# lucagem29/mcmc_clv_model

Hardware: AMD Instinct MI355X
Metric: MCMC sweeps/sec x N_customers (customer-sweeps/s) (higher is better)
Workload: dtype f64

## Files before the change

include/clvmcmc.h:

```cpp
#ifndef CLVMCMC_H
#define CLVMCMC_H

#include <stdint.h>

#ifdef __cplusplus
extern "C" {
#endif

#define CLV_ABI_VERSION 2

#define CLV_BLOCK 256
#define CLV_MAX_K 9
#define CLV_MAX_D 3

enum { CLV_OK = 0, CLV_EINVAL = -1, CLV_EHIP = -2, CLV_ESTATE = -3, CLV_ENOMEM = -4 };
enum { CLV_RNG_PHILOX = 0, CLV_RNG_REPLAY = 1 };
enum { CLV_SINK_FULL = 0, CLV_SINK_SUMMARY = 1, CLV_SINK_NONE = 2, CLV_SINK_SUMMARY_PCT = 3 };

#define CLV_SUMMARY_MU_CAP 0.05
enum {
  CLV_SUM_LAMBDA = 0, CLV_SUM_MU, CLV_SUM_Z, CLV_SUM_LOG_LAMBDA, CLV_SUM_LOG_MU,
  CLV_SUM_LAMBDA2, CLV_SUM_MU2, CLV_SUM_ETA, CLV_SUM_LOG_ETA, CLV_SUM_MU_CAPPED, CLV_SUM_TAU,
  CLV_N_SUM_STATS
};

typedef struct clv_config {
  int32_t abi_version;
  int32_t D;
  int32_t K;
  int32_t n_mh_steps;
  int32_t burnin, mcmc, thin;
  int32_t n_chains;
  int32_t chain_first;
  int32_t rng_mode;
  int32_t draw_sink;
  int32_t device;
  uint64_t seed;
  int64_t n_global;
  int64_t shard_begin;
  int32_t world_size;
  int32_t rank;
  int32_t blocks_per_rank;
  int32_t blocks_per_unit;
  uint64_t stream;
} clv_config;

typedef struct clv_data {
  int64_t n;
  const int32_t* x;
  const double* t_x;
  const double* T_cal;
  const double* covariates;
  const double* log_s;
} clv_data;

typedef struct clv_prior {
  double lam_init;
  double V[CLV_MAX_K * CLV_MAX_K];
  double chol_V[CLV_MAX_K * CLV_MAX_K];
  double A0B0[CLV_MAX_K * CLV_MAX_D];
  double S0_B0A0B0[CLV_MAX_D * CLV_MAX_D];
  double nu_n;
  double beta_init[CLV_MAX_K * CLV_MAX_D];
  double sigma_init[CLV_MAX_D * CLV_MAX_D];
  double omega2;
} clv_prior;

typedef struct clv_sampler clv_sampler;

int32_t clv_abi_version(void);
int32_t clv_default_blocks_per_unit(int64_t n_global);
int64_t clv_sizeof(int32_t which);
const char* clv_last_error(void);
int clv_device_count(int32_t* count);

int clv_create(const clv_config* cfg, const clv_data* data, const clv_prior* prior,
               clv_sampler** out);
void clv_destroy(clv_sampler* s);

int clv_set_replay_tape(clv_sampler* s, const double* tape, int64_t n_sweeps);
int64_t clv_replay_sweep_stride(const clv_sampler* s);

int clv_run(clv_sampler* s, int64_t n_sweeps);
int clv_rollback(clv_sampler* s);

int clv_sweep(clv_sampler* s);
int clv_hyper(clv_sampler* s, const double* gathered_device_ptr);
int clv_partials(clv_sampler* s, double** device_ptr, int64_t* n_doubles, int32_t* stride);
int clv_copy_partials(clv_sampler* s, void* dst_device_ptr);
int clv_synchronize(clv_sampler* s);
int64_t clv_sweeps_done(const clv_sampler* s);

int clv_clock_ghz(clv_sampler* s, double* ghz);
int clv_clock_probe(clv_sampler* s, double us, double* ghz);
int clv_launch_info(const clv_sampler* s, int64_t* out);
int clv_split_relay_steps(const clv_sampler* s, int32_t* out);
#define CLV_IPC_HANDLE_BYTES 64
int clv_p2p_info(const clv_sampler* s, int64_t* out);
int clv_p2p_export(clv_sampler* s, void* handle);
int clv_p2p_connect(clv_sampler* s, const void* handles, const uint64_t* ptrs);
int clv_p2p_disconnect(clv_sampler* s);
int clv_p2p_set_persistent(clv_sampler* s, int32_t on);
int clv_set_wait_timeout(clv_sampler* s, double ms);
int clv_set_stream(clv_sampler* s, uint64_t stream);
int clv_note_sweeps(clv_sampler* s, int64_t n);

int clv_read_draws(clv_sampler* s, double* level1, double* level2, double* loglik);
int clv_stream_draws(clv_sampler* s, double* level1);
int clv_read_summary(clv_sampler* s, double* sums, int64_t* n_stored);

int clv_get_state(clv_sampler* s, double* lambdas, double* mus, double* hyper);
int clv_set_state(clv_sampler* s, const double* lambdas, const double* mus, const double* hyper,
                  int64_t sweeps_done);

int clv_set_timing(clv_sampler* s, int32_t enable);
int clv_kernel_time(clv_sampler* s, double* sweep_kernel_ms_total, int64_t* sweep_launches,
                    double* hyper_kernel_ms_total, int64_t* hyper_launches);

int clv_debug_host_times(const clv_sampler* s, int64_t* out);
int clv_debug_philox(uint32_t k0, uint32_t k1, const uint32_t* ctr, int64_t n, uint32_t* out);
int clv_debug_variates(uint64_t seed, int32_t chain, uint32_t sweep, int64_t n, int32_t n_steps,
                       float* t_l, float* t_m, float* u_acc, double* u_z, double* u_tau,
                       double* e_alive, double* eta_z, float* log2_u_acc);
int clv_debug_log2u_scan(uint64_t w_begin, uint64_t w_end, double* out);
int clv_debug_t3(const uint32_t* words, int64_t n, int32_t packed, float* t_l, float* t_m);
int clv_debug_level2(int32_t D, int32_t K, const clv_prior* prior, const double* xty,
                     const double* yty, const double* iw_normal, const double* iw_chi2,
                     const double* z, double* beta, double* sigma);
int clv_debug_stamps(clv_sampler* s, uint64_t* out);
int clv_debug_wg_stamps(clv_sampler* s, uint64_t* out);
int clv_debug_hyper_variates(uint64_t seed, int32_t chain, uint32_t sweep, double df, int64_t n,
                             double* chi2, double* normals);
int clv_debug_exp(const double* x, int64_t n, double* out);
int clv_debug_log(const double* x, int64_t n, double* out);
int clv_debug_mh_step(int64_t n, const int32_t* x, const uint8_t* z, const double* T_cal, const double* tau,
                      const double* mean, const double* prec3, const double* cur_pt, const float* t3,
                      const double* scale2, const float* log_u, double* out);
int clv_debug_wg_map(int32_t n_chains, int32_t nb, int32_t n_cu, int32_t* out);
int clv_debug_persist_fits(int64_t grid_wgs, int32_t blocks_per_cu, int32_t n_cu);
int clv_debug_persist_choice(int32_t D, int32_t K, int32_t n_chains, int64_t grid_wgs, int32_t blocks_per_cu,
                             int32_t n_cu);
int clv_debug_split_fits(int32_t n_chains, int32_t nb, int32_t blocks_per_cu, int32_t n_cu);
int clv_debug_split_choice(int32_t n_chains, int32_t nb, int32_t blocks_per_cu, int32_t n_cu);
int clv_debug_split_layout(int32_t n_chains, int32_t nb, int32_t* out);
int clv_debug_split_relay_plan(int32_t S, int32_t R, int32_t* out);
int clv_debug_split_draw_plan(int32_t R, int32_t share, int32_t* out);
int clv_debug_split_stamps(clv_sampler* s, uint64_t* out);
int clv_debug_sweep_plan(const int64_t* in, int32_t* out);

enum { CLV_EXCHANGE_AUTO = 0, CLV_EXCHANGE_P2P = 1, CLV_EXCHANGE_COPY = 2 };
typedef struct clv_group clv_group;
int clv_group_create(clv_sampler* const* shards, int32_t n, int32_t exchange, clv_group** out);
int clv_group_run(clv_group* g, int64_t n_sweeps);
int32_t clv_group_exchange(const clv_group* g);
void clv_group_destroy(clv_group* g);

enum {
  CLV_L1_MEAN_LAMBDA = 0, CLV_L1_LAMBDA_P025, CLV_L1_LAMBDA_P975, CLV_L1_MEAN_MU, CLV_L1_MEAN_MU_CAPPED,
  CLV_L1_MU_P025, CLV_L1_MU_P975, CLV_L1_MEAN_Z, CLV_L1_MEAN_TAU, CLV_L1_MEAN_ETA, CLV_N_L1_STATS
};
int clv_predict(int32_t device, const double* level1, int64_t n_draws, int64_t n, int32_t width,
                const double* T_cal, double T_star, uint64_t seed, int32_t simulate_spend, double sigma_s,
                int64_t* x_future, double* spend_future);
int clv_predict_sampler(clv_sampler* s, double T_star, uint64_t seed, int32_t simulate_spend,
                        double sigma_s, int64_t* x_future, double* spend_future);
int clv_track(int32_t device, const double* level1, int64_t n_draws, int64_t n, int32_t width,
              const double* birth_week, const double* times, int32_t n_times, uint64_t seed,
              double* inc_weekly);
int clv_track_sampler(clv_sampler* s, const double* birth_week, const double* times, int32_t n_times,
                      uint64_t seed, double* inc_weekly);
int clv_level1_summary(int32_t device, const double* level1, int64_t n_draws, int64_t n, int32_t width,
                       double mu_cap, double* out);
int clv_level1_summary_sampler(clv_sampler* s, double mu_cap, double* out);
int clv_chain_total_loglik(int32_t device, const double* level1, int64_t n_draws, int64_t n, int32_t width,
                           const int32_t* x, const double* T_cal, double* mean_total);
int clv_chain_total_loglik_sampler(clv_sampler* s, double* mean_total);

enum {
  CLV_LTV_VALUE_MEAN = 0, CLV_LTV_VALUE_SD, CLV_LTV_VALUE_P025, CLV_LTV_VALUE_P50, CLV_LTV_VALUE_P975,
  CLV_LTV_RESIDUAL_MEAN, CLV_LTV_RESIDUAL_SD, CLV_LTV_RESIDUAL_P025, CLV_LTV_RESIDUAL_P50, CLV_LTV_RESIDUAL_P975,
  CLV_LTV_P_ALIVE, CLV_LTV_LIFETIME_YRS, CLV_LTV_SURVIVAL_1YR, CLV_N_LTV_STATS
};
enum {
  CLV_LTV_DRAW_EQUITY = 0, CLV_LTV_DRAW_VALUE_TOTAL, CLV_LTV_DRAW_N_ALIVE, CLV_LTV_DRAW_MU_SHARE,
  CLV_N_LTV_DRAW_STATS
};
int clv_lifetime_value(int32_t device, const double* level1, int64_t n_draws, int64_t n, int32_t width,
                       const double* monetary , double delta, double horizon ,
                       double value_scale, double periods_per_year, double* out_customers, double* out_draws);
int clv_lifetime_value_sampler(clv_sampler* s, const double* monetary, double delta, double horizon,
                               double value_scale, double periods_per_year, double* out_customers,
                               double* out_draws);
int clv_ltv_info(int64_t* out);

enum {
  CLV_IC_LPPD = 0, CLV_IC_P_WAIC, CLV_IC_ELPD_WAIC, CLV_IC_ELPD_LOO, CLV_IC_P_LOO, CLV_IC_PARETO_K,
  CLV_IC_TAIL_LEN, CLV_N_IC_STATS
};
int clv_pointwise_loglik(int32_t device, const double* level1, int64_t n_draws, int64_t n, int32_t width,
                         const int32_t* x, const double* t_x, const double* T_cal,
                         const double* log_s , double omega2, double* out);
int clv_psis_loo(int32_t device, const double* loglik, int64_t n_draws, int64_t n, double reff, double* out);
int clv_information_criteria(int32_t device, const double* level1, int64_t n_draws, int64_t n, int32_t width,
                             const int32_t* x, const double* t_x, const double* T_cal, const double* log_s,
                             double omega2, double reff, double* out);
int clv_information_criteria_sampler(clv_sampler* s, int32_t spend, double omega2, double reff, double* out);
int clv_ic_info(int64_t* out);
int clv_debug_information_criteria(int32_t device, const double* level1, int64_t n_draws, int64_t n, int32_t width,
                                   const int32_t* x, const double* t_x, const double* T_cal, const double* log_s,
                                   double omega2, double reff, int64_t batch_keys, int32_t grid, double* out);

int clv_score_customers(int32_t device, int32_t D, int32_t K, int32_t n_chains, int64_t n_draws,
                        const double* level2, int64_t n, const int32_t* x, const double* t_x,
                        const double* T_cal, const double* cov, const double* log_s, double omega2,
                        int32_t n_mh_steps, int32_t warmup, int32_t inner_sweeps, uint64_t seed,
                        int32_t chain_first, int64_t customer_offset, int64_t sweep_first,
                        const double* init_lam, const double* init_mu, int32_t sink, double* level1_out,
                        double* sums_out, double* state_lam_out, double* state_mu_out);
int clv_score_customers_sampler(clv_sampler* s, int64_t n, const int32_t* x, const double* t_x,
                                const double* T_cal, const double* cov, const double* log_s,
                                int32_t n_mh_steps, int32_t warmup, int32_t inner_sweeps, uint64_t seed,
                                int64_t customer_offset, int64_t sweep_first, const double* init_lam,
                                const double* init_mu, int32_t sink, double* level1_out, double* sums_out,
                                double* state_lam_out, double* state_mu_out);
int clv_score_info(int64_t* out);
int clv_debug_score_hyper(int32_t device, int32_t D, int32_t K, int64_t n_rec, const double* level2,
                          double omega2, double* out);

enum {
  CLV_FC_XSTAR_MEAN = 0, CLV_FC_P_ALIVE, CLV_FC_P_ZERO, CLV_FC_Q05, CLV_FC_Q50, CLV_FC_Q95, CLV_FC_TAIL_MASS,
  CLV_FC_LOG_SCORE, CLV_FC_PIT_LO, CLV_FC_PIT_HI, CLV_FC_RPS, CLV_N_FC_STATS
// ... 150 lines not shown
```

mcmc_clv_model_amd/_lib.py:

```python
from __future__ import annotations

import ctypes
import os
from ctypes import c_uint8, POINTER, c_char_p, c_double, c_float, c_int32, c_int64, c_uint32, c_uint64, c_void_p

try:
    import torch
except Exception:
    torch = None

LIB_NAME = "libclvmcmc.so"
LIB_PATH = os.environ.get("CLV_LIB_PATH") or os.path.join(os.path.dirname(os.path.abspath(__file__)), LIB_NAME)

ABI_VERSION = 2
BLOCK = 256
MAX_K = 9
MAX_D = 3
RNG_PHILOX, RNG_REPLAY = 0, 1
SINK_FULL, SINK_SUMMARY, SINK_NONE, SINK_SUMMARY_PCT = 0, 1, 2, 3
EXCHANGE_AUTO, EXCHANGE_P2P, EXCHANGE_COPY = 0, 1, 2
SUM_STATS = ("lambda", "mu", "z", "log_lambda", "log_mu", "lambda2", "mu2", "eta", "log_eta", "mu_capped", "tau")
SUMMARY_MU_CAP = 0.05
N_SUM_STATS = len(SUM_STATS)
TAPE_HYPER = 40


class ClvConfig(ctypes.Structure):
    _fields_ = [
        ("abi_version", c_int32), ("D", c_int32), ("K", c_int32), ("n_mh_steps", c_int32),
        ("burnin", c_int32), ("mcmc", c_int32), ("thin", c_int32), ("n_chains", c_int32),
        ("chain_first", c_int32), ("rng_mode", c_int32), ("draw_sink", c_int32), ("device", c_int32),
        ("seed", c_uint64), ("n_global", c_int64), ("shard_begin", c_int64),
        ("world_size", c_int32), ("rank", c_int32), ("blocks_per_rank", c_int32),
        ("blocks_per_unit", c_int32), ("stream", c_uint64),
    ]


class ClvData(ctypes.Structure):
    _fields_ = [
        ("n", c_int64), ("x", c_void_p), ("t_x", c_void_p), ("T_cal", c_void_p),
        ("covariates", c_void_p), ("log_s", c_void_p),
    ]


class ClvPrior(ctypes.Structure):
    _fields_ = [
        ("lam_init", c_double), ("V", c_double * 81), ("chol_V", c_double * 81), ("A0B0", c_double * 27),
        ("S0_B0A0B0", c_double * 9), ("nu_n", c_double), ("beta_init", c_double * 27),
        ("sigma_init", c_double * 9), ("omega2", c_double),
    ]


class ClvBatchItem(ctypes.Structure):
    _fields_ = [
        ("n", c_int64), ("seed", c_uint64), ("x", c_void_p), ("t_x", c_void_p), ("T_cal", c_void_p),
        ("covariates", c_void_p), ("log_s", c_void_p), ("prior", POINTER(ClvPrior)),
        ("level1", c_void_p), ("level2", c_void_p), ("loglik", c_void_p), ("sums", c_void_p),
        ("state_lam", c_void_p), ("state_mu", c_void_p),
    ]


_lib = None


class ClvError(RuntimeError):
    pass


def lib() -> ctypes.CDLL:
    global _lib
    if _lib is not None:
        return _lib
    if not os.path.exists(LIB_PATH):
        raise ClvError(
            f"{LIB_NAME} is not built ({LIB_PATH}); run `make -C mcmc_clv_model_amd/csrc` "
            "or `python -c 'import __graft_entry__ as g; g.build()'`")
    L = ctypes.CDLL(LIB_PATH, mode=ctypes.RTLD_GLOBAL)
    sp = c_void_p
    dp = POINTER(c_double)
    sigs = {
        "clv_abi_version": (c_int32, []),
        "clv_default_blocks_per_unit": (c_int32, [c_int64]),
        "clv_sizeof": (c_int64, [c_int32]),
        "clv_last_error": (c_char_p, []),
        "clv_device_count": (c_int32, [POINTER(c_int32)]),
        "clv_create": (c_int32, [POINTER(ClvConfig), POINTER(ClvData), POINTER(ClvPrior), POINTER(sp)]),
        "clv_destroy": (None, [sp]),
        "clv_set_replay_tape": (c_int32, [sp, dp, c_int64]),
        "clv_replay_sweep_stride": (c_int64, [sp]),
        "clv_run": (c_int32, [sp, c_int64]),
        "clv_rollback": (c_int32, [sp]),
        "clv_sweep": (c_int32, [sp]),
        "clv_hyper": (c_int32, [sp, c_void_p]),
        "clv_partials": (c_int32, [sp, POINTER(c_void_p), POINTER(c_int64), POINTER(c_int32)]),
        "clv_copy_partials": (c_int32, [sp, c_void_p]),
        "clv_synchronize": (c_int32, [sp]),
        "clv_sweeps_done": (c_int64, [sp]),
        "clv_clock_ghz": (c_int32, [sp, POINTER(c_double)]),
        "clv_clock_probe": (c_int32, [sp, c_double, POINTER(c_double)]),
        "clv_launch_info": (c_int32, [sp, POINTER(c_int64)]),
        "clv_split_relay_steps": (c_int32, [sp, POINTER(c_int32)]),
        "clv_p2p_info": (c_int32, [sp, POINTER(c_int64)]),
        "clv_p2p_export": (c_int32, [sp, c_void_p]),
        "clv_p2p_connect": (c_int32, [sp, c_void_p, POINTER(c_uint64)]),
        "clv_p2p_disconnect": (c_int32, [sp]),
        "clv_p2p_set_persistent": (c_int32, [sp, c_int32]),
        "clv_set_wait_timeout": (c_int32, [sp, c_double]),
        "clv_set_stream": (c_int32, [sp, c_uint64]),
        "clv_note_sweeps": (c_int32, [sp, c_int64]),
        "clv_read_draws": (c_int32, [sp, dp, dp, dp]),
        "clv_stream_draws": (c_int32, [sp, dp]),
        "clv_read_summary": (c_int32, [sp, dp, POINTER(c_int64)]),
        "clv_get_state": (c_int32, [sp, dp, dp, dp]),
        "clv_set_state": (c_int32, [sp, dp, dp, dp, c_int64]),
        "clv_set_timing": (c_int32, [sp, c_int32]),
        "clv_kernel_time": (c_int32, [sp, dp, POINTER(c_int64), dp, POINTER(c_int64)]),
        "clv_debug_philox": (c_int32, [c_uint32, c_uint32, POINTER(c_uint32), c_int64, POINTER(c_uint32)]),
        "clv_debug_variates": (c_int32, [c_uint64, c_int32, c_uint32, c_int64, c_int32, POINTER(c_float),
                                         POINTER(c_float), POINTER(c_float), dp, dp, dp, dp, POINTER(c_float)]),
        "clv_debug_log2u_scan": (c_int32, [c_uint64, c_uint64, dp]),
        "clv_debug_host_times": (c_int32, [sp, POINTER(c_int64)]),
        "clv_debug_t3": (c_int32, [POINTER(c_uint32), c_int64, c_int32, POINTER(c_float), POINTER(c_float)]),
        "clv_debug_level2": (c_int32, [c_int32, c_int32, POINTER(ClvPrior), dp, dp, dp, dp, dp, dp, dp]),
        "clv_debug_hyper_variates": (c_int32, [c_uint64, c_int32, c_uint32, c_double, c_int64, dp, dp]),
        "clv_debug_stamps": (c_int32, [sp, POINTER(c_uint64)]),
        "clv_debug_wg_stamps": (c_int32, [sp, POINTER(c_uint64)]),
        "clv_debug_split_stamps": (c_int32, [sp, POINTER(c_uint64)]),
        "clv_debug_split_relay_plan": (c_int32, [c_int32, c_int32, POINTER(c_int32)]),
        "clv_debug_split_draw_plan": (c_int32, [c_int32, c_int32, POINTER(c_int32)]),
        "clv_debug_exp": (c_int32, [dp, c_int64, dp]),
        "clv_debug_log": (c_int32, [dp, c_int64, dp]),
        "clv_debug_mh_step": (c_int32, [c_int64, POINTER(c_int32), POINTER(c_uint8), dp, dp, dp, dp, dp,
                                        POINTER(c_float), dp, POINTER(c_float), dp]),
        "clv_debug_wg_map": (c_int32, [c_int32, c_int32, c_int32, POINTER(c_int32)]),
        "clv_debug_sweep_plan": (c_int32, [POINTER(c_int64), POINTER(c_int32)]),
        "clv_debug_persist_choice": (c_int32, [c_int32, c_int32, c_int32, c_int64, c_int32, c_int32]),
        "clv_debug_persist_fits": (c_int32, [c_int64, c_int32, c_int32]),
        "clv_group_create": (c_int32, [POINTER(sp), c_int32, c_int32, POINTER(sp)]),
        "clv_group_run": (c_int32, [sp, c_int64]),
        "clv_group_exchange": (c_int32, [sp]),
        "clv_group_destroy": (None, [sp]),
        "clv_predict": (c_int32, [c_int32, dp, c_int64, c_int64, c_int32, dp, c_double, c_uint64, c_int32, c_double,
                                  POINTER(c_int64), dp]),
        "clv_predict_sampler": (c_int32, [sp, c_double, c_uint64, c_int32, c_double, POINTER(c_int64), dp]),
        "clv_track": (c_int32, [c_int32, dp, c_int64, c_int64, c_int32, dp, dp, c_int32, c_uint64, dp]),
        "clv_track_sampler": (c_int32, [sp, dp, dp, c_int32, c_uint64, dp]),
        "clv_level1_summary": (c_int32, [c_int32, dp, c_int64, c_int64, c_int32, c_double, dp]),
        "clv_level1_summary_sampler": (c_int32, [sp, c_double, dp]),
        "clv_chain_total_loglik": (c_int32, [c_int32, dp, c_int64, c_int64, c_int32, POINTER(c_int32), dp, dp]),
        "clv_chain_total_loglik_sampler": (c_int32, [sp, dp]),
        "clv_lifetime_value": (c_int32, [c_int32, dp, c_int64, c_int64, c_int32, dp, c_double, c_double, c_double,
                                         c_double, dp, dp]),
        "clv_lifetime_value_sampler": (c_int32, [sp, dp, c_double, c_double, c_double, c_double, dp, dp]),
        "clv_ltv_info": (c_int32, [POINTER(c_int64)]),
        "clv_pointwise_loglik": (c_int32, [c_int32, dp, c_int64, c_int64, c_int32, POINTER(c_int32), dp, dp, dp,
                                           c_double, dp]),
        "clv_psis_loo": (c_int32, [c_int32, dp, c_int64, c_int64, c_double, dp]),
        "clv_information_criteria": (c_int32, [c_int32, dp, c_int64, c_int64, c_int32, POINTER(c_int32), dp, dp, dp,
                                               c_double, c_double, dp]),
        "clv_information_criteria_sampler": (c_int32, [sp, c_int32, c_double, c_double, dp]),
        "clv_ic_info": (c_int32, [POINTER(c_int64)]),
        "clv_debug_information_criteria": (c_int32, [c_int32, dp, c_int64, c_int64, c_int32, POINTER(c_int32), dp,
                                                     dp, dp, c_double, c_double, c_int64, c_int32, dp]),
        "clv_score_customers": (c_int32, [c_int32, c_int32, c_int32, c_int32, c_int64, dp, c_int64, POINTER(c_int32), dp,
                                          dp, dp, dp, c_double, c_int32, c_int32, c_int32, c_uint64, c_int32, c_int64,
                                          c_int64, dp, dp, c_int32, dp, dp, dp, dp]),
        "clv_score_customers_sampler": (c_int32, [sp, c_int64, POINTER(c_int32), dp, dp, dp, dp, c_int32, c_int32,
                                                  c_int32, c_uint64, c_int64, c_int64, dp, dp, c_int32, dp, dp, dp, dp]),
        "clv_score_info": (c_int32, [POINTER(c_int64)]),
        "clv_debug_score_hyper": (c_int32, [c_int32, c_int32, c_int32, c_int64, dp, c_double, dp]),
        "clv_forecast": (c_int32, [c_int32, dp, c_int64, c_int64, c_int32, POINTER(c_int32), dp, dp, c_double, c_int32,
                                   POINTER(c_int32), dp, dp]),
        "clv_forecast_sampler": (c_int32, [sp, c_double, c_int32, POINTER(c_int32), dp, dp]),
        "clv_forecast_info": (c_int32, [POINTER(c_int64)]),
        "clv_debug_forecast": (c_int32, [c_int32, dp, c_int64, c_int64, c_int32, POINTER(c_int32), dp, dp, c_double,
                                         c_int32, POINTER(c_int32), c_int64, c_int32, dp, dp]),
        "clv_ppc": (c_int32, [c_int32, c_int32, dp, c_int32, dp, c_int32, c_int32, dp, c_int64, c_int64,
                              POINTER(c_int32), dp, dp, c_int32, c_uint64, c_int64, dp, POINTER(c_int64), dp,
                              POINTER(c_int64), dp]),
        "clv_ppc_sampler": (c_int32, [sp, c_int32, c_int32, c_uint64, dp, POINTER(c_int64), dp, POINTER(c_int64), dp]),
        "clv_ppc_info": (c_int32, [POINTER(c_int64)]),
        "clv_debug_ppc": (c_int32, [c_int32, c_int32, dp, c_int32, dp, c_int32, c_int32, dp, c_int64, c_int64,
                                    POINTER(c_int32), dp, dp, c_int32, c_uint64, c_int64, dp, POINTER(c_int64), dp,
                                    POINTER(c_int64), dp, c_int64, c_int32]),
        "clv_marginal_loglik": (c_int32, [c_int32, dp, c_int32, c_int32, dp, c_int64, c_int64, POINTER(c_int32), dp,
                                          dp, dp, c_double, c_int32, dp]),
        "clv_marginal_information_criteria": (c_int32, [c_int32, dp, c_int32, c_int32, dp, c_int64, c_int64,
                                                        POINTER(c_int32), dp, dp, dp, c_double, c_int32, c_double, dp]),
        "clv_marginal_information_criteria_sampler": (c_int32, [sp, c_int32, c_double, c_double, c_int32, dp]),
        "clv_marginal_info": (c_int32, [POINTER(c_int64)]),
        "clv_debug_marginal_loglik": (c_int32, [c_int32, dp, c_int32, c_int32, dp, c_int64, c_int64, POINTER(c_int32),
                                                dp, dp, dp, c_double, c_int32, c_int64, c_int32, dp, dp]),
        "clv_mml_create": (c_int32, [c_int32, c_int64, POINTER(c_int32), dp, dp, dp, c_int32, dp, POINTER(sp)]),
        "clv_mml_destroy": (None, [sp]),
        "clv_mml_eval": (c_int32, [sp, dp, c_int32, dp, POINTER(c_int64)]),
        "clv_mml_customers": (c_int32, [sp, dp, c_int32, c_double, dp]),
        "clv_debug_mml_eval": (c_int32, [sp, dp, c_int32, c_int32, dp, POINTER(c_int64)]),
        "clv_mml_info": (c_int32, [POINTER(c_int64)]),
        "clv_diagnostics": (c_int32, [c_int32, dp, c_int32, c_int64, c_int64, c_int32, c_uint32, dp]),
        "clv_diagnostics_sampler": (c_int32, [sp, c_uint32, dp, dp]),
        "clv_autocorr": (c_int32, [c_int32, dp, c_int32, c_int64, c_int64, c_int32, dp]),
        "clv_rank_diagnostics": (c_int32, [c_int32, dp, c_int32, c_int64, c_int64, c_int32, c_uint32, c_double, dp]),
        "clv_rank_diagnostics_sampler": (c_int32, [sp, c_uint32, c_double, dp, dp]),
        "clv_debug_zscale": (c_int32, [c_int32, dp, c_int32, c_int64, c_int64, c_int32, dp, dp]),
        "clv_elog2cbs": (c_int32, [c_int32, c_int64, POINTER(c_int64), POINTER(c_int64), dp, c_int64, c_int64, c_int64,
                                   POINTER(c_int64), POINTER(c_int64), POINTER(c_int64), dp, dp, dp, dp,
                                   POINTER(c_int64), dp, dp, POINTER(c_int64), dp]),
        "clv_generate_pareto_abe": (c_int32, [c_int32, c_int64, c_int32, dp, dp, dp, dp, c_int32, dp, c_uint64,
                                              POINTER(c_int64), dp, dp, dp, dp, POINTER(c_uint8), POINTER(c_int64), dp,
                                              POINTER(c_int64), POINTER(c_int64), c_int64, POINTER(c_int64), dp]),
        "clv_pnbd_create": (c_int32, [c_int32, c_int64, POINTER(c_int32), dp, dp, dp, POINTER(sp)]),
        "clv_pnbd_destroy": (None, [sp]),
        "clv_pnbd_eval": (c_int32, [sp, dp, dp, POINTER(c_int64)]),
        "clv_pnbd_customers": (c_int32, [sp, dp, c_double, dp]),
        "clv_pnbd_track": (c_int32, [c_int32, c_int64, dp, dp, c_int32, dp, dp]),
        "clv_pnbd_set_covariates": (c_int32, [sp, c_int32, dp, c_int32, dp]),
        "clv_pnbd_eval_cov": (c_int32, [sp, dp, dp, POINTER(c_int64)]),
        "clv_pnbd_customers_cov": (c_int32, [sp, dp, c_double, dp]),
# ... 153 lines not shown
```

mcmc_clv_model_amd/csrc/capi.hip:

```cpp
#include <hip/hip_runtime.h>

#include <algorithm>
#include <chrono>
#include <cstdlib>
#include <cstdio>
#include <cstring>
#include <string>
#include <vector>

#include "internal.h"
#include "kernels.h"
#include "philox.h"

using namespace clv;

namespace {

thread_local std::string g_err;

constexpr int PRIOR_V = 0, PRIOR_CHOLV = 81, PRIOR_A0B0 = 162, PRIOR_S0B = 189, PRIOR_DOUBLES = 198;
constexpr int GRAPH_CHUNK = 64;
constexpr int TIMING_EVENTS = 256;

}
// ... 214 lines not shown
  if ((d[1] == WAIT_P2P_MAIL || d[1] == WAIT_FX_MAIL) && g.units_per_rank > 0 && unit >= 0)
    m += "unit " + std::to_string(unit) + " (rank " + std::to_string(unit / g.units_per_rank) + ", local unit " +
         std::to_string(unit % g.units_per_rank) + ")";
  else
    m += (d[1] == WAIT_HYPER ? "of block " : "") + std::to_string(unit);
  if (d[1] == WAIT_RELAY) m += " (statistic: the wave row, bits: the flag's tag)";
  char bits[32];
  std::snprintf(bits, sizeof(bits), "%016llx", d[7]);
  m += " statistic " + std::to_string((long long)d[6]) + " still empty (bits " + bits + ") after " +
       std::to_string(d[8]) + " polls, " + std::to_string(d[9] / 100000.0) + " ms; " + std::to_string(d[10]) +
       " lanes of the wave missing";
  if (d[1] == WAIT_P2P_MAIL || d[1] == WAIT_FX_MAIL) {
    m += "; progress (sweep each rank's level-2 side last polled for):";
    for (int q = 0; q < std::min(g.world_size, 5); ++q)
      m += " " + std::to_string(q) + ":" + (d[11 + q] == ~0ull ? std::string("none") : std::to_string((long long)d[11 + q]));
  }
  return m + "]";
}

bool parse_wait_ms(const char* txt, double* ms) {
  for (const char* c = txt; *c; ++c)
    if (*c == 'x' || *c == 'X' || *c == 'n' || *c == 'N' || *c == 'i' || *c == 'I') return false;
  char* end = nullptr;
  const double v = std::strtod(txt, &end);
  if (end == txt) return false;
  while (*end == ' ' || *end == '\t' || *end == '\n') ++end;
  if (*end || !(v == v) || v > 1e300 || v < -1e300) return false;
  *ms = std::min(3.6e6, std::max(1.0, v));
  return true;
}

}

extern "C" {

int32_t clv_abi_version(void) { return CLV_ABI_VERSION; }

int32_t clv_default_blocks_per_unit(int64_t n_global) {
  const int64_t nb = (n_global + BLOCK - 1) / BLOCK;
  int32_t g = 1;
  while ((nb + g - 1) / g > 512) g *= 2;
  return g;
}

const char* clv_last_error(void) { return g_err.c_str(); }

int64_t clv_sizeof(int32_t which) {
  switch (which) {
    case 0: return (int64_t)sizeof(clv_config);
    case 1: return (int64_t)sizeof(clv_data);
    case 2: return (int64_t)sizeof(clv_prior);
    default: return -1;
  }
}

int clv_device_count(int32_t* count) {
  int n = 0;
  CLV_HIP(hipGetDeviceCount(&n));
  *count = n;
  return CLV_OK;
}

int64_t clv_replay_sweep_stride(const clv_sampler* s) {
  const int64_t n = s->g.n;
  return n * (2 + 3 * (int64_t)s->g.S + (s->g.D == 3 ? 1 : 0)) + TAPE_HYPER;
}

}

bool clv::persist_grid_fits(int64_t grid_wgs, int blocks_per_cu, int n_cu) {
  constexpr int SGPR_MAX = 102;
  const int sgpr_term = 800 / (((SGPR_MAX + 15) / 16) * 16 + 16);
  const int64_t per_cu = std::min({blocks_per_cu, 8, sgpr_term});
  const int64_t slots = per_cu * n_cu;
  const int64_t margin = std::max(1, n_cu / 32);
  return grid_wgs > 0 && slots > 0 && grid_wgs <= slots - margin;
}

constexpr size_t PERSIST_SCRATCH_MAX = 64;
#ifndef CLV_SPLIT_RELAY_DEFAULT
#define CLV_SPLIT_RELAY_DEFAULT 1
#endif
constexpr bool SPLIT_RELAY_DEFAULT = CLV_SPLIT_RELAY_DEFAULT != 0;

namespace {

bool persist_worth(int D, int K, int n_chains, int64_t grid_wgs, int n_cu) {
  (void)D, (void)K, (void)n_chains;
  return n_cu > 0 && grid_wgs > 0;
}

bool persist_split_fits(int n_chains, int nb, int blocks_per_cu, int n_cu) {
  if (n_chains < 1 || nb < 1 || nb > SPLIT_MAX_NB || blocks_per_cu < 1 || n_cu < 1) return false;
  const int64_t grid = (int64_t)n_chains * (split_wgs(nb) + 1);
  const int64_t margin = std::max(1, n_cu / 64);
  return grid <= n_cu - margin;
}

bool persist_split_pays(int n_chains, int nb, int n_cu) { return (int64_t)n_chains * (nb + 1) > n_cu; }

std::vector<int32_t> persist_split_layout(int n_chains, int nb) {
  const int per = split_wgs(nb) + 1;
  std::vector<int32_t> map((size_t)n_chains * per);
  for (int c = 0; c < n_chains; ++c)
    for (int p = 0; p < per; ++p) map[(size_t)c * per + p] = (c << 16) | p;
  return map;
}

#ifndef CLV_L2_ALONE_MIN_NB
#define CLV_L2_ALONE_MIN_NB 256
#endif
std::vector<int32_t> persist_wg_map(int C, int nb, int n_cu) {
  const int per = nb + 1;
  const int T = C * per;
  std::vector<int32_t> map(T);
  for (int c = 0; c < C; ++c)
    for (int b = 0; b < per; ++b) map[c * per + b] = (c << 16) | b;
  const int P = T - n_cu;
  if (P <= 0 || T > 2 * n_cu) return map;
  std::vector<std::vector<int>> todo(C);
  for (int c = 0; c < C; ++c)
    for (int b = nb - 1; b >= 0; --b) todo[c].push_back(b);
  std::vector<int32_t> first, second, single;
  int p = 0;
  const bool l2_alone = nb >= CLV_L2_ALONE_MIN_NB;
  for (int c = 0; !l2_alone && c < C && p < P; ++c, ++p) {
    first.push_back((c << 16) | nb);
    if (todo[c].empty()) return map;
    second.push_back((c << 16) | todo[c].back());
    todo[c].pop_back();
  }
  const int n_l2_paired = (int)first.size();
  const bool l2_paired = n_l2_paired == C;
  for (int c = 0; p < P; c = (c + 1) % C) {
    bool any = false;
    for (int k = 0; k < C && !any; ++k) any = todo[(c + k) % C].size() >= 2;
    if (!any) return map;
    if (todo[c].size() < 2) continue;
    first.push_back((c << 16) | todo[c].back());
    todo[c].pop_back();
    second.push_back((c << 16) | todo[c].back());
    todo[c].pop_back();
    ++p;
  }
  for (int c = 0; c < C; ++c) {
    if (!l2_paired && c >= n_l2_paired) single.push_back((c << 16) | nb);
    while (!todo[c].empty()) {
      single.push_back((c << 16) | todo[c].back());
      todo[c].pop_back();
    }
  }
  std::vector<int32_t> sorted_single;
  for (size_t k = 0; sorted_single.size() < single.size(); ++k)
    for (int c = 0; c < C; ++c) {
      size_t seen = 0;
      for (int32_t v : single)
        if ((v >> 16) == c && seen++ == k) sorted_single.push_back(v);
    }
  if ((int)first.size() != P || (int)sorted_single.size() != n_cu - P) return map;
  for (int i = 0; i < P; ++i) {
    map[i] = first[i];
    map[n_cu + i] = second[i];
  }
  for (int i = 0; i < n_cu - P; ++i) map[P + i] = sorted_single[i];
  return map;
}


struct SweepEnv {
  int persistent = -1;
  int layout = 0;
  int relay = -1;
  bool defer = true;
  int mail_first = 0;
  double wait_ms = 0.0;
};

SweepEnv read_sweep_env() {
  const auto is = [](const char* v, const char* text) { return v && !std::strcmp(v, text); };
  SweepEnv e;
  const char* v = std::getenv("CLV_PERSISTENT");
  e.persistent = is(v, "0") ? 0 : is(v, "1") ? 1 : -1;
  v = std::getenv("CLV_PERSIST_LAYOUT");
  e.layout = !v ? 0 : is(v, "block") ? LAYOUT_BLOCK : is(v, "split") ? LAYOUT_SPLIT : -1;
  v = std::getenv("CLV_SPLIT_RELAY");
  e.relay = !v ? -1 : is(v, "0") ? 0 : is(v, "1") ? 1 : 2;
  e.defer = !is(std::getenv("CLV_DEFER"), "0");
  v = std::getenv("CLV_MAIL_ALLOC");
  e.mail_first = is(v, "fine") ? 1 : is(v, "default") ? 2 : 0;
  v = std::getenv("CLV_WAIT_TIMEOUT_MS");
  if (v && !parse_wait_ms(v, &e.wait_ms)) e.wait_ms = -1.0;
  return e;
}

constexpr int64_t NOT_QUERIED = -2, QUERY_FAILED = -1;
struct Instance { int bpc = 0; int64_t scratch = NOT_QUERIED; };
struct SweepResources {
  int n_cu = 0;
  Instance block, split, relay;
};
struct SweepPlan {
  bool persistent = false, split = false, p2p_capable = false, p2p_persist_fits = false, fx_capable = false, defer = false;
  int relay_steps = 0;
  bool need_split = false, need_relay = false;
  const char* error = nullptr;
};

bool persist_shape(const Geometry& g, bool replay) {
  if (replay || g.nb_local <= 0 || g.nb_local > 2 * BLOCK) return false;
  if (g.world_size == 1) return g.blocks_per_unit == 1;
  const int bpu = g.blocks_per_unit;
  return g.world_size <= MAX_WORLD && g.n_units_global <= 2 * BLOCK && bpu <= 64 &&
         (int64_t)g.stride * ((g.nb_local + bpu - 1) / bpu) <= UMAIL;
}

bool persist_grid_chosen(int D, int K, int n_chains, int64_t grid_wgs, int blocks_per_cu, int n_cu, bool force) {
  return persist_grid_fits(grid_wgs, blocks_per_cu, n_cu) && (force || persist_worth(D, K, n_chains, grid_wgs, n_cu));
}
bool split_chosen(int n_chains, int nb, int blocks_per_cu, int n_cu, bool force) {
  return persist_split_fits(n_chains, nb, blocks_per_cu, n_cu) && (force || persist_split_pays(n_chains, nb, n_cu));
}

SweepPlan plan_sweep(const Geometry& g, bool replay, const SweepResources& r, const SweepEnv& e) {
  SweepPlan p;
  const int C = g.n_chains, nb = g.nb_local;
  const bool force = e.persistent == 1;
  const bool resident = persist_shape(g, replay) && e.persistent != 0 &&
                        (force || (r.block.scratch >= 0 && r.block.scratch <= (int64_t)PERSIST_SCRATCH_MAX)) &&
                        persist_grid_chosen(g.D, g.K, C, (int64_t)(nb + 1) * C, r.block.bpc, r.n_cu, force);
  if (g.world_size == 1) p.persistent = resident;
  else p.p2p_capable = p.p2p_persist_fits = resident;
  p.fx_capable = !replay && g.world_size > 1 && g.world_size <= MAX_WORLD && g.n_units_global <= 2 * BLOCK;
  p.defer = p.persistent && e.defer;
  if (!(p.persistent && g.D == 2 && g.S <= PRE_STEPS && nb <= SPLIT_MAX_NB)) return p;
  if (e.layout < 0) p.error = "CLV_PERSIST_LAYOUT must be block or split";
  else if (e.relay > 1) p.error = "CLV_SPLIT_RELAY must be 0 or 1";
  if (p.error || e.layout == LAYOUT_BLOCK) return p;
  if (r.split.scratch == NOT_QUERIED) {
    p.need_split = true;
    return p;
  }
  p.split = r.split.scratch == 0 && split_chosen(C, nb, r.split.bpc, r.n_cu, e.layout == LAYOUT_SPLIT);
  if (p.split && SPLIT_RELAY_STEPS > 0 && g.S > SPLIT_RELAY_STEPS && (e.relay < 0 ? SPLIT_RELAY_DEFAULT : e.relay == 1)) {
    if (r.relay.scratch == NOT_QUERIED) p.need_relay = true;
    else if (r.relay.scratch == 0 && persist_split_fits(C, nb, r.relay.bpc, r.n_cu)) p.relay_steps = SPLIT_RELAY_STEPS;
  }
  return p;
}


int validate_and_derive(const clv_config* cfg, const clv_data* data, const clv_prior* prior, clv_sampler** out) {
  if (cfg->abi_version != CLV_ABI_VERSION) return fail(CLV_EINVAL, "ABI version mismatch");
  if (cfg->D != 2 && cfg->D != 3) return fail(CLV_EINVAL, "D must be 2 or 3");
  if (cfg->K < 1 || cfg->K > CLV_MAX_K) return fail(CLV_EINVAL, "K must be in 1..9");
  if (cfg->n_mh_steps < 0) return fail(CLV_EINVAL, "n_mh_steps must be >= 0");
  if (cfg->thin < 1) return fail(CLV_EINVAL, "thin must be >= 1");
  if (cfg->burnin < 0 || cfg->mcmc < 0) return fail(CLV_EINVAL, "burnin/mcmc must be >= 0");
  if (cfg->n_chains < 1) return fail(CLV_EINVAL, "n_chains must be >= 1");
  if (cfg->rng_mode != CLV_RNG_PHILOX && cfg->rng_mode != CLV_RNG_REPLAY) return fail(CLV_EINVAL, "bad rng_mode");
  if (cfg->draw_sink < CLV_SINK_FULL || cfg->draw_sink > CLV_SINK_SUMMARY_PCT) return fail(CLV_EINVAL, "bad draw_sink");
  if (data->n < 0) return fail(CLV_EINVAL, "n must be >= 0");
  if (cfg->n_global > 0xffffffffLL) return fail(CLV_EINVAL, "n_global must fit the 32-bit Philox customer counter");
  if (cfg->n_global < data->n || cfg->n_global < 1) return fail(CLV_EINVAL, "n_global must be >= n >= 0 and > 0");
  if (cfg->world_size < 1 || cfg->rank < 0 || cfg->rank >= cfg->world_size) return fail(CLV_EINVAL, "bad rank/world_size");
  if (cfg->D == 3 && data->n > 0 && !data->log_s) return fail(CLV_EINVAL, "D == 3 needs log_s");
  if (cfg->K > 1 && data->n > 0 && !data->covariates) return fail(CLV_EINVAL, "K > 1 needs covariates");
  if (data->n > 0 && (!data->x || !data->t_x || !data->T_cal)) return fail(CLV_EINVAL, "missing CBS column");
  if (cfg->rng_mode == CLV_RNG_REPLAY && cfg->world_size != 1) return fail(CLV_EINVAL, "replay needs world_size 1");

  const int32_t bpu = cfg->blocks_per_unit ? cfg->blocks_per_unit : clv_default_blocks_per_unit(cfg->n_global);
  if (!is_pow2(bpu)) return fail(CLV_EINVAL, "blocks_per_unit must be a power of two");
  const int nb_local = (int)((data->n + BLOCK - 1) / BLOCK);
  int32_t bpr = cfg->blocks_per_rank;
  if (bpr == 0) {
    if (cfg->world_size != 1) return fail(CLV_EINVAL, "blocks_per_rank required when sharded");
    bpr = ((std::max(nb_local, 1) + bpu - 1) / bpu) * bpu;
  }
  if (bpr % bpu) return fail(CLV_EINVAL, "blocks_per_rank must be a multiple of blocks_per_unit");
  if (nb_local > bpr) return fail(CLV_EINVAL, "shard larger than blocks_per_rank * CLV_BLOCK");
  if (cfg->shard_begin != (int64_t)cfg->rank * bpr * BLOCK) return fail(CLV_EINVAL, "shard_begin != rank * blocks_per_rank * CLV_BLOCK");
  const int64_t nb_global = (cfg->n_global + BLOCK - 1) / BLOCK;
  if ((int64_t)bpr * cfg->world_size < nb_global) return fail(CLV_EINVAL, "shards do not cover n_global");

  auto* s = new clv_sampler();
  s->cfg = *cfg;
  s->cfg.blocks_per_rank = bpr;
  s->cfg.blocks_per_unit = bpu;
  s->prior = *prior;
  s->replay = cfg->rng_mode == CLV_RNG_REPLAY;

  Geometry& g = s->g;
  g.D = cfg->D;
  g.K = cfg->K;
  g.S = cfg->n_mh_steps;
  g.n_chains = cfg->n_chains;
  g.n = data->n;
  g.n_global = cfg->n_global;
  g.shard_begin = cfg->shard_begin;
  g.nb_local = nb_local;
  g.blocks_per_rank = bpr;
  g.blocks_per_unit = bpu;
  g.units_per_rank = bpr / bpu;
  g.n_units_global = (nb_global + bpu - 1) / bpu;
  g.world_size = cfg->world_size;
  g.stride = cfg->K * cfg->D + cfg->D * (cfg->D + 1) / 2 + 1;
  g.burnin = cfg->burnin;
  g.mcmc = cfg->mcmc;
  g.thin = cfg->thin;
  g.n_draws = cfg->mcmc >= 1 ? (cfg->mcmc - 1) / cfg->thin + 1 : 0;
  g.l2w = cfg->D * cfg->K + cfg->D * (cfg->D + 1) / 2;
  *out = s;
  return CLV_OK;
}

int open_device_and_stream(clv_sampler* s) {
  if (s->cfg.device >= 0) CLV_HIP(hipSetDevice(s->cfg.device));
  CLV_HIP(hipGetDevice(&s->device));
  if (s->cfg.stream) {
    s->stream = (hipStream_t)(uintptr_t)s->cfg.stream;
  } else {
    CLV_HIP(hipStreamCreateWithFlags(&s->own, hipStreamNonBlocking));
    s->stream = s->own;
  }
  return CLV_OK;
}

Instance query_split_instance(const Geometry& g, bool relay) {
  Instance in;
  size_t scratch = 0;
  const bool ok = persist_split_resources(g.D, g.K, &in.bpc, &scratch, relay) == hipSuccess;
  if (!ok) (void)hipGetLastError();
  in.scratch = ok ? (int64_t)scratch : QUERY_FAILED;
  return in;
}

int decide_sweep_path(clv_sampler* s, const SweepEnv& env) {
  const Geometry& g = s->g;
  SweepResources r;
  if (persist_shape(g, s->replay)) {
    hipDeviceProp_t prop{};
    size_t scratch = 0;
    r.block.scratch = QUERY_FAILED;
    if (persist_occupancy(g.D, g.K, g.world_size > 1, &r.block.bpc) == hipSuccess &&
        persist_scratch_bytes(g.D, g.K, g.world_size > 1, &scratch) == hipSuccess &&
        hipGetDeviceProperties(&prop, s->device) == hipSuccess) {
      r.block.scratch = (int64_t)scratch;
      r.n_cu = prop.multiProcessorCount;
    }
    s->persist_bpc = r.block.bpc;
    s->n_cu = r.n_cu;
  }
  SweepPlan p = plan_sweep(g, s->replay, r, env);
  if (p.need_split) {
    r.split = query_split_instance(g, false);
    p = plan_sweep(g, s->replay, r, env);
  }
  if (p.need_relay) {
    r.relay = query_split_instance(g, true);
    p = plan_sweep(g, s->replay, r, env);
  }
  if (p.error) return fail(CLV_EINVAL, p.error);
  s->persistent = p.persistent;
  s->split = p.split;
  s->relay_steps = p.relay_steps;
  s->p2p_capable = p.p2p_capable;
  s->p2p_persist_fits = p.p2p_persist_fits;
  s->fx_capable = p.fx_capable;
  s->defer = p.defer;
  if (s->persistent || s->p2p_capable || s->fx_capable) {
    if (env.wait_ms < 0) return fail(CLV_EINVAL, "CLV_WAIT_TIMEOUT_MS must be a finite decimal number of ms");
    const double ms = env.wait_ms > 0 ? env.wait_ms : g.world_size > 1 ? 10000.0 : 2000.0;
    s->wait_ticks = (uint64_t)(ms * 1e5);
  }
  return CLV_OK;
}

void forget_peers(clv_sampler* s) {
  s->p2p_ready = false;
  for (void* p : s->ipc_opened) (void)hipIpcCloseMemHandle(p);
  s->ipc_opened.clear();
}

hipError_t fill_mail(clv_sampler* s) {
  return hipMemsetAsync(s->d_mail, 0xFF, sizeof(double) * mail_count(s->g), s->stream);
}

int allocate_and_clear(clv_sampler* s, const SweepEnv& env) {
  const Geometry& g = s->g;
  const hipStream_t st = s->stream;
  const size_t C = g.n_chains, n1 = std::max<int64_t>(g.n, 1);
  const bool summary = (s->cfg.draw_sink == CLV_SINK_SUMMARY || s->cfg.draw_sink == CLV_SINK_SUMMARY_PCT) && g.n > 0;
  CLV_HIP(s->d_x.alloc(n1));
  for (auto* b : {&s->d_tx, &s->d_T}) CLV_HIP(b->alloc(n1));
  if (g.K > 1) CLV_HIP(s->d_cov.alloc((g.K - 1) * n1));
  if (g.D == 3) CLV_HIP(s->d_logs.alloc(n1));
  CLV_HIP(s->d_clk.alloc(2 * CLK_RING, 0, st));
  for (auto* b : {&s->d_lam, &s->d_mu}) CLV_HIP(b->alloc(state_count(g)));
  CLV_HIP(s->d_hyper.alloc(hyper_count(g), 0, st));
  CLV_HIP(s->d_block.alloc(C * g.blocks_per_rank * g.stride, 0, st));
  if (g.blocks_per_unit > 1) CLV_HIP(s->d_unit_own.alloc(unit_count(g), 0, st));
  s->d_unit = g.blocks_per_unit > 1 ? s->d_unit_own : s->d_block;
  CLV_HIP(s->d_prior.alloc(PRIOR_DOUBLES));
  CLV_HIP(s->d_ctrl.alloc(1, 0, st));
  CLV_HIP(s->d_arrive.alloc(arrive_count(g), 0, st));
  CLV_HIP(s->d_hvar.alloc(2 * C * HV, 0, st));
  CLV_HIP(s->d_hyp2.alloc(handoff_count(g)));
  if (s->p2p_capable || s->fx_capable) {
    const unsigned flags[3] = {hipDeviceMallocUncached, hipDeviceMallocFinegrained, hipDeviceMallocDefault};
    for (int k = env.mail_first; k < 3 && !s->d_mail; ++k) {
      void* p = nullptr;
      if (hipExtMallocWithFlags(&p, sizeof(double) * mail_count(g), flags[k]) == hipSuccess && p) {
        s->d_mail.reset((double*)p);
        s->mail_kind = k;
      } else {
        (void)hipGetLastError();
      }
    }
    if (!s->d_mail) return fail(CLV_ENOMEM, "peer mail buffer");
    CLV_HIP(fill_mail(s));
    CLV_HIP(s->d_peers.alloc(g.world_size));
  }
  if (s->persistent || s->p2p_capable || s->fx_capable) {
    CLV_HIP(s->d_pblock.alloc(pblock_count(g)));
    if (s->defer) CLV_HIP(s->d_pend.alloc(2 * C * g.stride));
    for (auto* b : {&s->d_lam_alt, &s->d_mu_alt}) CLV_HIP(b->alloc(state_count(g)));
    CLV_HIP(s->d_hyper_alt.alloc(hyper_count(g)));
    if (summary) CLV_HIP(s->d_sums_prev.alloc(sums_count(g)));
    CLV_HIP(s->d_diag.alloc(DIAG_WORDS, 0, st));
    CLV_HIP(hipHostMalloc((void**)&s->h_abort, sizeof(uint32_t), hipHostMallocMapped));
    *s->h_abort = 0;
    CLV_HIP(hipHostGetDevicePointer((void**)&s->d_h_abort, s->h_abort, 0));
  }
  if ((s->persistent || s->p2p_capable) && s->n_cu > 0) {
    const std::vector<int32_t> map = persist_wg_map((int)C, g.nb_local, s->n_cu);
    CLV_HIP(s->d_wgmap.upload(map.data(), map.size()));
    if (s->split) {
      const std::vector<int32_t> smap = persist_split_layout((int)C, g.nb_local);
      CLV_HIP(s->d_wgmap_split.upload(smap.data(), smap.size()));
    }
  }
#ifdef CLV_STAMPS
  {
    std::vector<unsigned long long> stamps(1024 * 8 + (12 + 16) * C * (std::max(g.nb_local, 1) + 1), 0ull);
    for (int i = 0; i < 1024; ++i) stamps[i * 8 + 0] = stamps[i * 8 + 4] = ~0ull;
    CLV_HIP(s->d_stamps.upload(stamps.data(), stamps.size()));
  }
#endif
// ... 132 lines not shown
  if (s->pending_init_hyper) return fail(CLV_ESTATE, "bivariate: call clv_hyper once before the first sweep");
  CLV_HIP(hipSetDevice(s->device));
  int rc = persist_flush(s);
  if (rc) return rc;
  rc = check_replay_range(s, 1);
  if (rc) return rc;
  hipEvent_t e0 = nullptr, e1 = nullptr;
  if (s->timing) {
    rc = ensure_events(s);
    if (rc) return rc;
    e0 = s->ev[4 * s->ev_used];
    e1 = s->ev[4 * s->ev_used + 1];
  }
  rc = enqueue_sweep(s, e0, e1);
  if (rc) return rc;
  if (s->timing && ++s->ev_used == TIMING_EVENTS) {
    rc = harvest_timing(s);
    if (rc) return rc;
  }
  s->sweeps_done++;
  return CLV_OK;
}

int clv_partials(clv_sampler* s, double** ptr, int64_t* n_doubles, int32_t* stride) {
  if (!s) return fail(CLV_EINVAL, "null sampler");
  if (ptr) *ptr = s->d_unit;
  if (n_doubles) *n_doubles = (int64_t)unit_count(s->g);
  if (stride) *stride = s->g.stride;
  return CLV_OK;
}

int clv_copy_partials(clv_sampler* s, void* dst) {
  if (!s || !dst) return fail(CLV_EINVAL, "null argument");
  CLV_HIP(hipSetDevice(s->device));
  CLV_HIP(hipMemcpyAsync(dst, s->d_unit, sizeof(double) * unit_count(s->g), hipMemcpyDeviceToDevice, s->stream));
  return CLV_OK;
}

int clv_synchronize(clv_sampler* s) {
  if (!s) return fail(CLV_EINVAL, "null sampler");
  CLV_HIP(hipSetDevice(s->device));
  CLV_HIP(hipStreamSynchronize(s->stream));
  return CLV_OK;
}

int64_t clv_sweeps_done(const clv_sampler* s) { return s ? s->sweeps_done : -1; }

int clv_clock_ghz(clv_sampler* s, double* ghz) {
  if (!s || !ghz) return fail(CLV_EINVAL, "null argument");
  *ghz = 0.0;
  const int64_t end = s->sweeps_done - 1;
  const int64_t first = std::max<int64_t>(s->clk_first, end - (CLK_RING - 1));
  if (!s->d_clk || s->clk_first < 1 || end < first) return CLV_OK;
  CLV_HIP(hipSetDevice(s->device));
  CLV_HIP(hipStreamSynchronize(s->stream));
  std::vector<unsigned long long> ring(2 * CLK_RING);
  CLV_HIP(hipMemcpy(ring.data(), s->d_clk, sizeof(unsigned long long) * ring.size(), hipMemcpyDeviceToHost));
  double dm = 0.0, dr = 0.0;
  for (int64_t q = first; q <= end; ++q) {
    dm += (double)ring[2 * (q % CLK_RING)];
    dr += (double)ring[2 * (q % CLK_RING) + 1];
  }
  if (dr > 0.0) *ghz = 0.1 * dm / dr;
  return CLV_OK;
}

int clv_launch_info(const clv_sampler* s, int64_t* out) {
  if (!s || !out) return fail(CLV_EINVAL, "null argument");
  out[0] = s->persistent ? 1 : 0;
  out[1] = s->persist_bpc;
  out[2] = s->n_cu;
  out[3] = (int64_t)(s->g.nb_local + (s->persistent ? 1 : 0)) * s->g.n_chains;
  out[4] = s->split ? (int64_t)(split_wgs(s->g.nb_local) + 1) * s->g.n_chains : out[3];
  out[5] = !s->persistent ? LAYOUT_NONE : s->split ? LAYOUT_SPLIT : s->split_reverted ? -LAYOUT_BLOCK : LAYOUT_BLOCK;
  return CLV_OK;
}

int clv_split_relay_steps(const clv_sampler* s, int32_t* out) {
  if (!s || !out) return fail(CLV_EINVAL, "null argument");
  *out = s->split ? s->relay_steps : 0;
  return CLV_OK;
}

int clv_p2p_info(const clv_sampler* s, int64_t* out) {
  if (!s || !out) return fail(CLV_EINVAL, "null argument");
  out[0] = (s->p2p_capable || s->fx_capable) ? 1 : 0;
  out[4] = s->p2p_capable ? 1 : 0;
  out[1] = s->p2p_ready ? 1 : 0;
  out[2] = s->d_mail ? (int64_t)sizeof(double) * 2 * s->g.world_size * s->g.n_chains * s->g.stride * s->g.units_per_rank : 0;
  out[3] = (int64_t)(uintptr_t)s->d_mail.p;
  out[5] = s->d_mail ? s->mail_kind : -1;
  return CLV_OK;
}

int clv_p2p_export(clv_sampler* s, void* handle) {
  if (!s || !handle) return fail(CLV_EINVAL, "null argument");
  if (!s->p2p_capable && !s->fx_capable) return fail(CLV_ESTATE, "no peer exchange for this sampler (world size 1 or replay mode)");
  CLV_HIP(hipSetDevice(s->device));
  hipIpcMemHandle_t h;
  CLV_HIP(hipIpcGetMemHandle(&h, s->d_mail));
  std::memcpy(handle, &h, sizeof(h));
  return CLV_OK;
}

int clv_p2p_connect(clv_sampler* s, const void* handles, const uint64_t* ptrs) {
  if (!s || (!handles && !ptrs)) return fail(CLV_EINVAL, "null argument");
  if (!s->p2p_capable && !s->fx_capable) return fail(CLV_ESTATE, "no peer exchange for this sampler (world size 1 or replay mode)");
  CLV_HIP(hipSetDevice(s->device));
  CLV_HIP(hipStreamSynchronize(s->stream));
  forget_peers(s);
  CLV_HIP(fill_mail(s));
  const int W = s->g.world_size, r = s->cfg.rank;
  std::vector<double*> peers(W, nullptr);
  for (int q = 0; q < W; ++q) {
    if (q == r) {
      peers[q] = s->d_mail;
    } else if (handles) {
      hipIpcMemHandle_t h;
      std::memcpy(&h, (const char*)handles + (size_t)q * sizeof(h), sizeof(h));
      void* p = nullptr;
      CLV_HIP(hipIpcOpenMemHandle(&p, h, hipIpcMemLazyEnablePeerAccess));
      s->ipc_opened.push_back(p);
      peers[q] = (double*)p;
    } else {
      peers[q] = (double*)(uintptr_t)ptrs[q];
    }
    if (!peers[q]) return fail(CLV_EINVAL, "null peer mail pointer");
  }
  CLV_HIP(hipMemcpy(s->d_peers, peers.data(), sizeof(double*) * W, hipMemcpyHostToDevice));
  CLV_HIP(hipStreamSynchronize(s->stream));
  s->p2p_ready = true;
  return CLV_OK;
}

int clv_p2p_set_persistent(clv_sampler* s, int32_t on) {
  if (!s) return fail(CLV_EINVAL, "null sampler");
  if (on && !s->p2p_persist_fits) return fail(CLV_ESTATE, "the persistent peer exchange does not fit this shard's grid");
  if (!on && !s->fx_capable) return fail(CLV_ESTATE, "no fused peer exchange for this sampler");
  CLV_HIP(hipSetDevice(s->device));
  CLV_HIP(hipStreamSynchronize(s->stream));
  s->p2p_capable = on != 0;
  s->last_persist_n = 0;
  return CLV_OK;
}

int clv_p2p_disconnect(clv_sampler* s) {
  if (!s) return fail(CLV_EINVAL, "null sampler");
  CLV_HIP(hipSetDevice(s->device));
  CLV_HIP(hipStreamSynchronize(s->stream));
  forget_peers(s);
  if (s->d_peers) CLV_HIP(hipMemset(s->d_peers, 0, sizeof(double*) * s->g.world_size));
  return CLV_OK;
}

int clv_set_wait_timeout(clv_sampler* s, double ms) {
  if (!s || !(ms >= 1.0) || ms > 3.6e6) return fail(CLV_EINVAL, "wait timeout must be in [1 ms, 1 h]");
  s->wait_ticks = (uint64_t)(ms * 1e5);
  return drop_graph(s);
}

int clv_set_stream(clv_sampler* s, uint64_t stream) {
  if (!s || !stream) return fail(CLV_EINVAL, "bad arguments");
  if (int rc = drop_graph(s)) return rc;
  s->stream = (hipStream_t)(uintptr_t)stream;
  return CLV_OK;
}

int clv_note_sweeps(clv_sampler* s, int64_t n) {
  if (!s || s->sweeps_done + n < 0) return fail(CLV_EINVAL, "bad arguments");
  s->sweeps_done += n;
  s->last_persist_n = 0;
  return CLV_OK;
}

}

static int rewind_ctrl_and_sums(clv_sampler* s) {
  Ctrl c{};
  c.cur = s->sweeps_done;
  CLV_HIP(hipMemcpy(s->d_ctrl, &c, sizeof(Ctrl), hipMemcpyHostToDevice));
  if (s->d_sums_prev)
    CLV_HIP(hipMemcpy(s->d_sums, s->d_sums_prev, sizeof(double) * sums_count(s->g), hipMemcpyDeviceToDevice));
  return CLV_OK;
}

static inline int64_t host_now_ns() {
  return std::chrono::duration_cast<std::chrono::nanoseconds>(std::chrono::steady_clock::now().time_since_epoch())
      .count();
}

int clv::persist_launch(clv_sampler* s, int64_t n_sweeps) {
  const Geometry& g = s->g;
  s->last_persist_n = 0;
  s->inflight_n = 0;
  if (n_sweeps == 0) return CLV_OK;
  if (s->slots_dirty) {
    CLV_HIP(hipMemsetAsync(s->d_hyp2, 0xFF, sizeof(double) * handoff_count(g), s->stream));
    CLV_HIP(hipMemsetAsync(s->d_pblock, 0xFF, sizeof(double) * pblock_count(g), s->stream));
    s->slots_dirty = false;
  }
  if (s->d_sums_prev)
    CLV_HIP(hipMemcpyAsync(s->d_sums_prev, s->d_sums, sizeof(double) * sums_count(g), hipMemcpyDeviceToDevice, s->stream));
  SweepArgs a = sweep_args(s, 0, 1);
  const int64_t stride_c = (int64_t)g.n_chains * g.stride;
  a.pend_in = s->pend ? s->d_pend + s->pend_buf * stride_c : nullptr;
  a.pend_out = s->defer ? s->d_pend + (s->pend_buf ^ 1) * stride_c : nullptr;
  hipEvent_t e0 = nullptr, e1 = nullptr;
  if (s->timing) {
    int rc = ensure_events(s);
    if (rc) return rc;
    e0 = s->ev[4 * s->ev_used];
    e1 = s->ev[4 * s->ev_used + 1];
    if (s->ev_sweeps.size() < TIMING_EVENTS) s->ev_sweeps.assign(TIMING_EVENTS, 1);
    s->ev_sweeps[s->ev_used] = n_sweeps;
  }
  if (e0) CLV_HIP(hipEventRecord(e0, s->stream));
  s->host_ns[2] = host_now_ns();
  if (s->split) {
    a.wg_map = s->d_wgmap_split;
    CLV_HIP(launch_persist_split(a, s->sweeps_done + 1, n_sweeps, s->stream, s->relay_steps > 0));
  } else {
    CLV_HIP(launch_persist(a, s->sweeps_done + 1, n_sweeps, s->stream, nullptr, nullptr));
  }
  s->host_ns[3] = host_now_ns();
  if (e1) CLV_HIP(hipEventRecord(e1, s->stream));
  s->inflight_done = e1;
  if (s->timing) {
    if (++s->ev_used == TIMING_EVENTS) {
      int rc = harvest_timing(s);
      if (rc) return rc;
    }
  } else {
    if (!s->done_ev) CLV_HIP(hipEventCreateWithFlags(&s->done_ev, hipEventDisableTiming));
    CLV_HIP(hipEventRecord(s->done_ev, s->stream));
    s->inflight_done = s->done_ev;
  }
  s->inflight_n = n_sweeps;
  s->host_ns[4] = host_now_ns();
  return CLV_OK;
}

int clv::persist_wait(clv_sampler* s) {
  const int64_t n_sweeps = s->inflight_n;
  if (n_sweeps == 0) return CLV_OK;
  s->inflight_n = 0;
  const Geometry& g = s->g;
  const hipEvent_t done = s->inflight_done;
  if (!done) {
    CLV_HIP(hipStreamSynchronize(s->stream));
  } else {
    hipError_t q;
    while ((q = hipEventQuery(done)) == hipErrorNotReady) {
    }
    CLV_HIP(q);
  }
  s->host_ns[5] = host_now_ns();
  if (__atomic_load_n(s->h_abort, __ATOMIC_ACQUIRE)) {
    *s->h_abort = 0;
    if (int rc = rewind_ctrl_and_sums(s)) return rc;
    s->slots_dirty = true;
    if (g.world_size > 1) s->p2p_ready = false;
    std::string diag = take_wait_diag(s);
    if (s->split) {
      s->split = false;
      s->relay_steps = 0;
      s->split_reverted = true;
      diag += "; the split layout's launch aborted: this handle uses the block layout from now on";
    }
    return fail(CLV_EHIP, std::string(g.world_size > 1
                                          ? "persistent sweep kernel: a wait timed out (a peer rank not running, or not all "
                                            "resident?); state unchanged"
                                          : "persistent sweep kernel: a workgroup timed out waiting for its chain (not all "
                                            "resident?); state unchanged") + diag);
  }
  s->d_lam.swap(s->d_lam_alt);
  s->d_mu.swap(s->d_mu_alt);
  s->rb_pend = s->pend;
  s->rb_pend_buf = s->pend_buf;
  s->rb_hyper_swaps = 0;
  if (s->defer) {
    s->pend = true;
    s->pend_buf ^= 1;
  } else {
    s->d_hyper.swap(s->d_hyper_alt);
    s->rb_hyper_swaps = 1;
    s->pend = false;
  }
  if (int rc = drop_graph(s)) return rc;
  s->sweeps_done += n_sweeps;
  s->last_persist_n = n_sweeps;
  return CLV_OK;
}

int clv::persist_flush(clv_sampler* s) {
  if (!s->pend) return CLV_OK;
  CLV_HIP(hipSetDevice(s->device));
  SweepArgs a = sweep_args(s, 0, 1);
  a.pend_in = s->d_pend + s->pend_buf * (int64_t)s->g.n_chains * s->g.stride;
  a.pend_out = nullptr;
  CLV_HIP(launch_persist_flush(a, s->sweeps_done + 1, s->stream));
  CLV_HIP(hipStreamSynchronize(s->stream));
  s->d_hyper.swap(s->d_hyper_alt);
  s->rb_hyper_swaps++;
  s->pend = false;
  return drop_graph(s);
}

namespace {
int run_persistent(clv_sampler* s, int64_t n_sweeps) {
  int rc = persist_launch(s, n_sweeps);
  if (rc) return rc;
  return persist_wait(s);
}

int enqueue_fused_sweeps(clv_sampler* s, int64_t n_sweeps) {
  int rc = CLV_OK;
  int64_t left = n_sweeps;
  if (s->timing) {
    rc = ensure_events(s);
    if (rc) return rc;
    while (left > 0) {
      const int k = s->ev_used;
      rc = enqueue_fused(s, s->ev[4 * k], s->ev[4 * k + 1]);
      if (rc) return rc;
      s->ev_used++;
      s->sweeps_done++;
      left--;
      if (s->ev_used == TIMING_EVENTS) {
        rc = harvest_timing(s);
        if (rc) return rc;
      }
    }
    return harvest_timing(s);
  }
  if (left >= GRAPH_CHUNK) {
    rc = build_graph(s, GRAPH_CHUNK);
    if (rc) return rc;
    while (left >= GRAPH_CHUNK) {
      CLV_HIP(hipGraphLaunch(s->graph_exec, s->stream));
      s->sweeps_done += GRAPH_CHUNK;
      left -= GRAPH_CHUNK;
    }
  }
  while (left > 0) {
    rc = enqueue_fused(s, nullptr, nullptr);
    if (rc) return rc;
    s->sweeps_done++;
    left--;
// ... 337 lines not shown
  CLV_HIP(dres.alloc(r.size()));
  CLV_HIP(launch_debug_log2u_scan(w_begin, w_end, NB, dres, nullptr));
  CLV_HIP(dres.download(r.data(), r.size()));
  double mu = 0.0, ma = 0.0, wu = 0.0, mu_far = 0.0;
  for (int b = 0; b < NB; ++b) {
    if (r[4 * b] > mu) {
      mu = r[4 * b];
      wu = r[4 * b + 2];
    }
    ma = std::max(ma, r[4 * b + 1]);
    mu_far = std::max(mu_far, r[4 * b + 3]);
  }
  out[0] = mu;
  out[1] = ma;
  out[2] = wu;
  out[3] = mu_far;
  return CLV_OK;
}

int clv_debug_t3(const uint32_t* words, int64_t n, int32_t packed, float* tl, float* tm) {
  if (!words || !tl || !tm || n < 1 || (packed != 0 && packed != 1)) return fail(CLV_EINVAL, "bad arguments");
  DevPtr<uint32_t> dw;
  DevPtr<float> dl, dm;
  CLV_HIP(dw.upload(words, 3 * n));
  CLV_HIP(dl.alloc(n));
  CLV_HIP(dm.alloc(n));
  CLV_HIP(launch_debug_t3(dw, n, packed, dl, dm, nullptr));
  CLV_HIP(dl.download(tl, n));
  CLV_HIP(dm.download(tm, n));
  return CLV_OK;
}

int clv_debug_level2(int32_t D, int32_t K, const clv_prior* prior, const double* xty, const double* yty,
                     const double* iwn, const double* chi2, const double* z, double* beta, double* sigma) {
  if ((D != 2 && D != 3) || K < 1 || K > CLV_MAX_K || !prior) return fail(CLV_EINVAL, "bad arguments");
  const std::vector<double> pr = pack_prior(prior, D, K);
  std::vector<double> in(K * D + D * D + 6 + D * K, 0.0);
  for (int i = 0; i < K * D; ++i) in[i] = xty[i];
  for (int i = 0; i < D * D; ++i) in[K * D + i] = yty[i];
  for (int i = 0; i < D * (D - 1) / 2; ++i) in[K * D + D * D + i] = iwn[i];
  for (int i = 0; i < D; ++i) in[K * D + D * D + 3 + i] = chi2[i];
  for (int i = 0; i < D * K; ++i) in[K * D + D * D + 6 + i] = z[i];
  std::vector<double> o(K * D + D * D);
  DevPtr<double> dpr, din, dout;
  CLV_HIP(dpr.upload(pr.data(), pr.size()));
  CLV_HIP(din.upload(in.data(), in.size()));
  CLV_HIP(dout.alloc(o.size()));
  CLV_HIP(launch_debug_level2(D, K, dpr, din, dout, nullptr));
  CLV_HIP(dout.download(o.data(), o.size()));
  for (int i = 0; i < K * D; ++i) beta[i] = o[i];
  for (int i = 0; i < D * D; ++i) sigma[i] = o[K * D + i];
  return CLV_OK;
}

int clv_debug_hyper_variates(uint64_t seed, int32_t chain, uint32_t sweep, double df, int64_t n, double* chi2,
                             double* normals) {
  if (n < 1 || df < 2.0) return fail(CLV_EINVAL, "bad arguments");
  DevPtr<double> dc, dn;
  CLV_HIP(dc.alloc(n));
  CLV_HIP(dn.alloc(n));
  CLV_HIP(launch_debug_hyper_variates(seed, chain, sweep, df, n, dc, dn, nullptr));
  CLV_HIP(dc.download(chi2, n));
  CLV_HIP(dn.download(normals, n));
  return CLV_OK;
}

int clv_debug_persist_choice(int32_t D, int32_t K, int32_t n_chains, int64_t grid_wgs, int32_t blocks_per_cu,
                             int32_t n_cu) {
  return persist_grid_chosen(D, K, n_chains, grid_wgs, blocks_per_cu, n_cu, false) ? 1 : 0;
}

int clv_debug_persist_fits(int64_t grid_wgs, int32_t blocks_per_cu, int32_t n_cu) {
  return persist_grid_fits(grid_wgs, blocks_per_cu, n_cu) ? 1 : 0;
}

int clv_debug_split_fits(int32_t n_chains, int32_t nb, int32_t blocks_per_cu, int32_t n_cu) {
  return persist_split_fits(n_chains, nb, blocks_per_cu, n_cu) ? 1 : 0;
}

int clv_debug_split_choice(int32_t n_chains, int32_t nb, int32_t blocks_per_cu, int32_t n_cu) {
  return split_chosen(n_chains, nb, blocks_per_cu, n_cu, false) ? 1 : 0;
}

int clv_debug_sweep_plan(const int64_t* in, int32_t* out) {
  if (!in || !out) return fail(CLV_EINVAL, "null argument");
  Geometry g{};
  g.D = (int)in[0];
  g.K = (int)in[1];
  g.S = (int)in[2];
  g.n_chains = (int)in[3];
  g.nb_local = (int)in[4];
  g.blocks_per_unit = (int)in[5];
  g.n_units_global = in[6];
  g.world_size = (int)in[7];
  g.stride = g.K * g.D + g.D * (g.D + 1) / 2 + 1;
  SweepResources r;
  r.n_cu = (int)in[9];
  r.block = Instance{(int)in[10], in[11]};
  r.split = Instance{(int)in[12], in[13]};
  r.relay = Instance{(int)in[14], in[15]};
  SweepEnv e;
  e.persistent = (int)in[16];
  e.layout = (int)in[17];
  e.relay = (int)in[18];
  e.defer = in[19] != 0;
  const SweepPlan p = plan_sweep(g, in[8] != 0, r, e);
  const int32_t o[8] = {p.persistent, p.split, p.relay_steps, p.p2p_capable, p.p2p_persist_fits, p.fx_capable,
                        p.defer, (p.need_split ? 1 : 0) | (p.need_relay ? 2 : 0)};
  std::copy(o, o + 8, out);
  return p.error ? fail(CLV_EINVAL, p.error) : CLV_OK;
}

int clv_debug_split_relay_plan(int32_t S, int32_t R, int32_t* out) {
  if (!out || S < 0 || S > PRE_STEPS || !(R == 0 || R == 8 || R == 12)) return fail(CLV_EINVAL, "bad arguments");
  const SplitRelayPlan pl = split_relay_plan(S, R);
  const int32_t o[8] = {pl.own_begin, pl.own_end, pl.relay_begin, pl.relay_end,
                        pl.own_begin, pl.own_end, pl.relay_begin, pl.relay_end};
  std::copy(o, o + 8, out);
  return CLV_OK;
}

int clv_debug_split_draw_plan(int32_t R, int32_t share, int32_t* out) {
  if (!out || !(R == 8 || R == 12) || share < -1 || share >= SPLIT_DRAW_SHARES) return fail(CLV_EINVAL, "bad arguments");
  if (share < 0) {
    out[0] = SPLIT_RELAY_DRAW;
    return CLV_OK;
  }
  constexpr int NQ = PRE_STEPS / 4;
  for (int row = 0; row < SPLIT_CW; ++row) {
    for (int q = 0; q < NQ; ++q) {
      const SplitDrawSlot d = split_draw_plan(R, share, row, q);
      const int32_t o[4] = {d.wave, d.slot, d.staged, d.reader};
      std::copy(o, o + 4, out + (row * NQ + q) * 4);
    }
  }
  return CLV_OK;
}

int clv_debug_split_layout(int32_t n_chains, int32_t nb, int32_t* out) {
  if (!out || n_chains < 1 || nb < 1 || nb > SPLIT_MAX_NB || n_chains >= (1 << 15)) return fail(CLV_EINVAL, "bad arguments");
  const std::vector<int32_t> m = persist_split_layout(n_chains, nb);
  const int nwg = split_wgs(nb);
  for (size_t i = 0; i < m.size(); ++i) {
    int32_t* o = out + 8 * i;
    const int p = m[i] & 0xFFFF;
    o[0] = m[i] >> 16;
    for (int k = 1; k < 8; ++k) o[k] = -1;
    if (p == nwg) continue;
    const int r0 = SPLIT_CW * p;
    o[1] = r0;
    o[2] = std::min(SPLIT_CW, 4 * nb - r0);
    const int b0 = (p & 1) ? (r0 - 2) / 4 : r0 / 4, b1 = (p & 1) ? (r0 + 2) / 4 : r0 / 4 + 1;
    o[3] = (p & 1) ? 3 : 1;
    o[4] = b0;
    if (b1 < nb) {
      o[5] = (p & 1) ? 1 : 2;
      o[6] = b1;
    }
    o[7] = (p & 1) ? nb + 2 * (b0 / 3) : -1;
  }
  return CLV_OK;
}

int clv_debug_wg_map(int32_t n_chains, int32_t nb, int32_t n_cu, int32_t* out) {
  if (!out || n_chains < 1 || nb < 0 || n_cu < 1 || n_chains >= (1 << 15) || nb >= (1 << 16))
    return fail(CLV_EINVAL, "bad arguments");
  const std::vector<int32_t> m = persist_wg_map(n_chains, nb, n_cu);
  std::copy(m.begin(), m.end(), out);
  return CLV_OK;
}

int clv_debug_mh_step(int64_t n, const int32_t* x, const uint8_t* z, const double* T_cal, const double* tau,
                      const double* mean, const double* prec3, const double* cur_pt, const float* t3,
                      const double* scale2, const float* log_u, double* out) {
  if (!x || !z || !T_cal || !tau || !mean || !prec3 || !cur_pt || !t3 || !scale2 || !log_u || !out || n < 1)
    return fail(CLV_EINVAL, "bad arguments");
  DevPtr<int32_t> dx;
  DevPtr<uint8_t> dz;
  DevPtr<double> dT, dtau, dm, dp, dc, ds, dout;
  DevPtr<float> dt3, dlu;
  CLV_HIP(dx.upload(x, n));
  CLV_HIP(dz.upload(z, n));
  CLV_HIP(dT.upload(T_cal, n));
  CLV_HIP(dtau.upload(tau, n));
  CLV_HIP(dm.upload(mean, 2 * n));
  CLV_HIP(dp.upload(prec3, 3));
  CLV_HIP(dc.upload(cur_pt, 2 * n));
  CLV_HIP(ds.upload(scale2, 2));
  CLV_HIP(dt3.upload(t3, 2 * n));
  CLV_HIP(dlu.upload(log_u, n));
  CLV_HIP(dout.alloc(7 * n));
  CLV_HIP(launch_debug_mh(dx, dz, dT, dtau, dm, dp, dc, dt3, ds, dlu, n, dout, nullptr));
  CLV_HIP(dout.download(out, 7 * n));
// ... 20 lines not shown
```

mcmc_clv_model_amd/csrc/internal.h:

```cpp
#pragma once
#include <hip/hip_runtime.h>

#include <algorithm>
#include <atomic>
#include <condition_variable>
#include <mutex>
#include <string>
#include <vector>

#include "kernels.h"

namespace clv {

int fail(int code, const std::string& msg);

int persist_launch(clv_sampler* s, int64_t n_sweeps);
int persist_wait(clv_sampler* s);
int persist_flush(clv_sampler* s);
bool persist_grid_fits(int64_t grid_wgs, int blocks_per_cu, int n_cu);

struct DrawStreamState {
  std::mutex m;
  std::condition_variable cv;
  int64_t pending = 0;
// ... 40 lines not shown
    const hipError_t e = alloc(count);
    return e != hipSuccess || !count ? e : hipMemsetAsync(p, byte, count * sizeof(T), st);
  }
  hipError_t upload(const T* host, size_t count) {
    const hipError_t e = alloc(count);
    return e != hipSuccess || !count ? e : hipMemcpy(p, host, count * sizeof(T), hipMemcpyHostToDevice);
  }
  hipError_t download(T* host, size_t count) const { return hipMemcpy(host, p, count * sizeof(T), hipMemcpyDeviceToHost); }
};
using DevBuf = DevPtr<void>;

struct DeviceScope {
  int prev = -1;
  explicit DeviceScope(int dev) {
    (void)hipGetDevice(&prev);
    if (dev >= 0) (void)hipSetDevice(dev);
  }
  ~DeviceScope() {
    if (prev >= 0) (void)hipSetDevice(prev);
  }
};

}

#define CLV_HIP(expr)                                                                           \
  do {                                                                                          \
    hipError_t e_ = (expr);                                                                     \
    if (e_ != hipSuccess)                                                                       \
      return ::clv::fail(CLV_EHIP, std::string(#expr) + ": " + hipGetErrorString(e_));          \
  } while (0)

namespace clv {

template <class T>
int upload(DevBuf& buf, const T* host, size_t count, hipStream_t st) {
  if (!host) return CLV_OK;
  CLV_HIP(hipMalloc(&buf.p, sizeof(T) * count));
  CLV_HIP(hipMemcpyAsync(buf.p, host, sizeof(T) * count, hipMemcpyHostToDevice, st));
  return CLV_OK;
}

}

struct clv_sampler {
  clv_config cfg{};
  clv_prior prior{};
  clv::Geometry g{};
  bool replay = false;
  int device = 0;
  hipStream_t stream = nullptr;
  hipStream_t own = nullptr;

  clv::DevPtr<int32_t> d_x;
  clv::DevPtr<double> d_tx, d_T, d_cov, d_logs;
  clv::DevPtr<double> d_lam, d_mu, d_hyper;
  clv::DevPtr<double> d_block, d_unit_own;
  double* d_unit = nullptr;
  clv::DevPtr<double> d_prior;
  clv::DevPtr<clv::Ctrl> d_ctrl;
  clv::DevPtr<uint32_t> d_arrive;
  clv::DevPtr<double> d_hyp2;
  clv::DevPtr<double> d_pblock;
  clv::DevPtr<double> d_lam_alt, d_mu_alt, d_hyper_alt;
  clv::DevPtr<double> d_sums_prev;
  uint32_t* h_abort = nullptr;
  uint32_t* d_h_abort = nullptr;
  clv::DevPtr<unsigned long long> d_diag;
  clv::DevPtr<unsigned long long> d_clk;
  int64_t clk_first = 0;
  uint64_t wait_ticks = 0;
  bool slots_dirty = true;
  int64_t last_persist_n = 0;
  bool defer = false;
  bool pend = false;
  int pend_buf = 0;
  clv::DevPtr<double> d_pend;
  bool rb_pend = false;
  int rb_pend_buf = 0;
  int rb_hyper_swaps = 0;
  bool persistent = false;
  int persist_bpc = 0, n_cu = 0;
  bool split = false;
  int relay_steps = 0;
  bool split_reverted = false;
  clv::DevPtr<int32_t> d_wgmap_split;
  bool p2p_capable = false;
  bool p2p_persist_fits = false;
  bool fx_capable = false;
  bool p2p_ready = false;
  clv::DevPtr<double> d_mail;
  int mail_kind = -1;
  clv::DevPtr<double*> d_peers;
  clv::DevPtr<int32_t> d_wgmap;
  std::vector<void*> ipc_opened;
  clv::DevPtr<double> d_hvar;
  clv::DevPtr<unsigned long long> d_stamps;
  clv::DevPtr<double> d_level1, d_level2, d_loglik, d_sums;
  clv::DevPtr<float2> d_qstore;
  clv::DevPtr<double> d_tape;
  clv::DevPtr<double> d_bs;
  int64_t tape_sweeps = 0;

  bool pending_init_hyper = false;
  int64_t sweeps_done = 0;

  hipGraphExec_t graph_exec = nullptr;
  int graph_sweeps = 0;

  hipEvent_t done_ev = nullptr;
  int64_t inflight_n = 0;
  hipEvent_t inflight_done = nullptr;

  int64_t host_ns[8] = {0, 0, 0, 0, 0, 0, 0, 0};

  clv::DrawStreamState* ds = nullptr;
  double* ds_dest = nullptr;
  int64_t ds_next = 0;

  bool timing = false;
  std::vector<hipEvent_t> ev;
  std::vector<int64_t> ev_sweeps;
  int ev_used = 0;
  double t_sweep_ms = 0.0, t_hyper_ms = 0.0;
  int64_t n_sweep_timed = 0, n_hyper_timed = 0;
};

namespace clv {

inline size_t state_count(const Geometry& g) { return (size_t)g.n_chains * std::max<int64_t>(g.n, 1); }
inline size_t hyper_count(const Geometry& g) { return (size_t)g.n_chains * HS; }
inline size_t sums_count(const Geometry& g) { return (size_t)g.n_chains * CLV_N_SUM_STATS * g.n; }
inline size_t arrive_count(const Geometry& g) { return (size_t)g.n_chains * (1 + g.units_per_rank); }
inline size_t handoff_count(const Geometry& g) { return 2 * hyper_count(g); }
inline size_t pblock_count(const Geometry& g) { return (size_t)g.n_chains * split_records(std::max(g.nb_local, 1)) * g.stride; }
inline size_t unit_count(const Geometry& g) { return (size_t)g.n_chains * g.units_per_rank * g.stride; }
inline size_t mail_count(const Geometry& g) { return mail_slots(g.world_size, g.n_chains, g.stride, g.units_per_rank) + MAIL_TAIL; }
inline size_t loglik_count(const Geometry& g) { return (size_t)g.n_chains * g.n_draws; }
inline size_t level1_count(const Geometry& g) { return loglik_count(g) * g.n * (g.D + 2); }

inline int64_t stored_draws(const clv_sampler* s) {
  if (s->sweeps_done <= s->g.burnin) return 0;
  const int64_t k = (s->sweeps_done - 1 - s->g.burnin) / s->g.thin + 1;
  return k < s->g.n_draws ? k : (int64_t)s->g.n_draws;
}

}
```

mcmc_clv_model_amd/csrc/kernels.h:

```cpp
#pragma once
#include <hip/hip_runtime.h>
#include <stdint.h>

#include "../../include/clvmcmc.h"

namespace clv {

constexpr int BLOCK = CLV_BLOCK;
constexpr int HS = 64;
constexpr int H_TAG = 63;
constexpr int TAPE_HYPER = 40;
constexpr int MAX_WORLD = 64;
constexpr int UMAIL = 2048;
constexpr int HV = 40;
constexpr int MAIL_TAIL = MAX_WORLD;
constexpr int CLK_RING = 1024;
constexpr int DIAG_WORDS = 16;
constexpr int PRE_STEPS = 20;
constexpr int SPLIT_CW = 6;
constexpr int SPLIT_NT = 512;
constexpr int SPLIT_MAX_NB = 256;
enum : int { LAYOUT_NONE = 0, LAYOUT_BLOCK = 1, LAYOUT_SPLIT = 2 };
__host__ __device__ inline int split_wgs(int nb) { return (2 * nb + 2) / 3; }
__host__ __device__ inline int split_records(int nb) { return nb + 2 * ((nb + 1) / 3); }
enum : int { WAIT_HYPER = 1, WAIT_BLOCKS = 2, WAIT_P2P_MAIL = 3, WAIT_FX_MAIL = 4, WAIT_RELAY = 5 };
#ifndef CLV_SPLIT_RELAY_STEPS
#define CLV_SPLIT_RELAY_STEPS 8
#endif
constexpr int SPLIT_RELAY_STEPS = CLV_SPLIT_RELAY_STEPS;
static_assert(SPLIT_RELAY_STEPS == 0 || SPLIT_RELAY_STEPS == 8 || SPLIT_RELAY_STEPS == 12, "relay point: 8 or 12 steps");
struct SplitRelayPlan {
  int own_begin, own_end, relay_begin, relay_end;
};
__host__ __device__ constexpr SplitRelayPlan split_relay_plan(int S, int R) {
  return SplitRelayPlan{0, (R > 0 && S > R) ? R : S, (R > 0 && S > R) ? R : S, S};
}
#ifndef CLV_SPLIT_RELAY_DRAW
#define CLV_SPLIT_RELAY_DRAW 4
#endif
#ifndef CLV_SPLIT_RELAY_GAP2_CHUNKS
#define CLV_SPLIT_RELAY_GAP2_CHUNKS 3
#endif
#ifndef CLV_SPLIT_RELAY_GAP2_STOP
#define CLV_SPLIT_RELAY_GAP2_STOP 6
#endif
constexpr int SPLIT_RELAY_DRAW = CLV_SPLIT_RELAY_DRAW;
constexpr int SPLIT_RELAY_GAP2_CHUNKS = CLV_SPLIT_RELAY_GAP2_CHUNKS;
constexpr int SPLIT_RELAY_GAP2_STOP = CLV_SPLIT_RELAY_GAP2_STOP;
constexpr int SPLIT_DRAW_SHARES = 6;
static_assert(SPLIT_RELAY_DRAW >= 0 && SPLIT_RELAY_DRAW < SPLIT_DRAW_SHARES, "draw share: 0..5");
static_assert(SPLIT_RELAY_GAP2_CHUNKS >= 1 && SPLIT_RELAY_GAP2_STOP >= 1 && SPLIT_RELAY_GAP2_STOP <= SPLIT_CW, "gap 2 limits");
enum : int { DRAW_WINDOW = 0, DRAW_GAP1 = 1, DRAW_GAP2 = 2 };
struct SplitDrawSlot {
  int wave;
  int slot;
  int staged;
  int reader;
};
__host__ __device__ constexpr int split_draw_gap1_chunks(int share) { return share >= 4 ? share - 3 : share >= 2 ? share - 1 : 0; }
__host__ __device__ constexpr SplitDrawSlot split_draw_plan(int R, int share, int row, int chunk) {
  const int qr = R / 4;
  const int reader = (row >= 4 && chunk >= qr) ? row + 2 : row;
  if (share >= 1 && share <= 3 && row >= 4 && chunk >= qr && chunk < qr + SPLIT_RELAY_GAP2_CHUNKS)
    return SplitDrawSlot{row + 2, DRAW_GAP2, 0, reader};
  if ((row & 3) < 2 && chunk < split_draw_gap1_chunks(share) && chunk < qr)
    return SplitDrawSlot{6 + (row & 1), DRAW_GAP1, 1, reader};
  return SplitDrawSlot{reader, DRAW_WINDOW, 0, reader};
}

__host__ __device__ inline int64_t mail_slots(int world, int chains, int stride, int units_per_rank) {
  return 2LL * world * chains * stride * units_per_rank;
}

enum : int {
  H_BETA = 0,
  H_SIGMA = 27,
  H_P00 = 36, H_P01 = 37, H_P11 = 38,
  H_S00 = 39, H_S11 = 40,
  H_S22 = 41, H_POSTVAR = 42, H_SQRT_POSTVAR = 43, H_OMEGA2 = 44,
  H_INV_OMEGA2 = 45, H_INV_S22 = 46,
};

struct Ctrl {
  int64_t cur;
  uint32_t arrive;
  uint32_t abort;
};

struct Geometry {
  int D, K, S;
  int n_chains;
  int64_t n;
  int64_t n_global;
  int64_t shard_begin;
  int nb_local;
  int blocks_per_rank;
  int blocks_per_unit;
  int units_per_rank;
  int64_t n_units_global;
  int world_size;
  int stride;
  int burnin, mcmc, thin, n_draws;
  int l2w;
};

struct Rng {
  uint64_t seed;
// ... 11 lines not shown
  Ctrl* ctrl;
  double* level2;
  double* loglik;
  const double* V;
  const double* cholV;
  const double* A0B0;
  const double* S0B;
  double nu_n;
  double omega2;
  int mode;
  const double* hvar;
  unsigned long long* stamps;
};

struct SweepArgs {
  Geometry g;
  Rng r;
  const int32_t* x;
  const double* tx;
  const double* T;
  const double* cov;
  const double* log_s;
  double* lam;
  double* mu;
  const double* hyper;
  double* blockpart;
  double* pblock;
  const Ctrl* ctrl;
  Ctrl* ctrl_rw;
  double* hyp2;
  double* level1;
  double* sums;
  float2* qstore;
  int64_t* n_stored;
  double lam_init;
  int init;
  int fuse;
  uint32_t* chain_arrive;
  uint32_t* unit_arrive;
  double* unitpart;
  double* hvar_out;
  double* mail;
  double* const* peers;
  int rank;
  const int32_t* wg_map;
  double* lam_out;
  double* mu_out;
  double* hyper_out;
  const double* pend_in;
  double* pend_out;
  uint64_t wait_ticks;
  uint32_t* abort_host;
  unsigned long long* diag;
  unsigned long long* clk;
  HyperArgs h;
  unsigned long long* stamps;
};

struct ScoreArgs {
  const double* hyper;
  int64_t n_draws;
  int64_t s_first;
  int warmup;
  int inner;
  double* level1;
  double* sums;
  double* lam_out;
  double* mu_out;
};

struct GroupArgs {
  Geometry g;
  const double* blockpart;
  double* unitpart;
};


hipError_t launch_sweep(const SweepArgs& a, bool replay, hipStream_t st, hipEvent_t e0 = nullptr,
                        hipEvent_t e1 = nullptr);
hipError_t launch_group(const GroupArgs& a, hipStream_t st);
hipError_t launch_persist(const SweepArgs& a, int64_t s_first, int64_t n_sweeps, hipStream_t st,
                          hipEvent_t e0 = nullptr, hipEvent_t e1 = nullptr);
hipError_t launch_persist_split(const SweepArgs& a, int64_t s_first, int64_t n_sweeps, hipStream_t st,
                                bool relay = false);
hipError_t persist_split_resources(int D, int K, int* blocks_per_cu, size_t* scratch_bytes, bool relay = false);
hipError_t persist_occupancy(int D, int K, bool p2p, int* blocks_per_cu);
hipError_t persist_scratch_bytes(int D, int K, bool p2p, size_t* bytes);
hipError_t launch_persist_flush(const SweepArgs& a, int64_t s_first, hipStream_t st);
hipError_t launch_hyper(const HyperArgs& a, bool replay, hipStream_t st);
hipError_t launch_set_hyper(int D, int K, int n_chains, double* hyper, const double* beta_sigma,
                            double omega2, bool replay, hipStream_t st);
hipError_t launch_debug_philox(uint32_t k0, uint32_t k1, const uint32_t* ctr, int64_t n, uint32_t* out,
                               hipStream_t st);
hipError_t launch_debug_variates(uint64_t seed, int chain, uint32_t sweep, int64_t n, int S, float* tl,
                                 float* tm, float* ua, float* l2u, double* uz, double* ut, double* ea, double* ez,
                                 hipStream_t st);
hipError_t launch_debug_log2u_scan(uint64_t w_begin, uint64_t w_end, int n_blocks, double* out, hipStream_t st);
hipError_t launch_debug_t3(const uint32_t* w, int64_t n, int packed, float* tl, float* tm, hipStream_t st);
hipError_t launch_debug_level2(int D, int K, const double* prior_dev, const double* in, double* out,
                               hipStream_t st);
hipError_t launch_debug_hyper_variates(uint64_t seed, int chain, uint32_t sweep, double df, int64_t n,
                                       double* chi2, double* normals, hipStream_t st);
hipError_t launch_debug_exp(const double* x, int64_t n, double* out, hipStream_t st, bool log_fn = false);
hipError_t launch_debug_mh(const int32_t* x, const uint8_t* z, const double* T, const double* tau, const double* m,
                           const double* prec, const double* cur_pt, const float* t3, const double* scale,
                           const float* log_u, int64_t n, double* out, hipStream_t st);

}
```

mcmc_clv_model_amd/csrc/kernels.hip:

```cpp
#include <hip/hip_ext.h>

#include "fastmath.h"
#include "internal.h"
#include "kernels.h"
#include "philox.h"

#ifndef SWEEP_MH_PIPELINE
#define SWEEP_MH_PIPELINE 1
#endif
#ifndef CLV_OPAQUE_GI
#define CLV_OPAQUE_GI(D) ((D) == 3)
#endif
#ifndef CLV_L2_OPAQUE
#define CLV_L2_OPAQUE(P) (P)
#endif
#ifndef CLV_L2_LANE0_MAX
#define CLV_L2_LANE0_MAX 6
#endif
#ifndef PERSIST_REDUCE_GEN
#define PERSIST_REDUCE_GEN 1
#endif
#ifndef SWEEP_REDUCE_CHUNK
#define SWEEP_REDUCE_CHUNK 8
#endif
// ... 1816 lines not shown
          const uint64_t t0 = __builtin_amdgcn_s_memrealtime();
          for (uint32_t poll = 0; !timed_out; ++poll) {
            bool ok = true;
#pragma unroll
            for (int q = 0; q < FXC; ++q) {
              if (j0 + q < NS) {
                v0[q] = ld_sys(q0 + j0 + q);
                v1[q] = ld_sys(q1 + j0 + q);
                ok = ok & (!h0 | slot_full(v0[q])) & (!h1 | slot_full(v1[q]));
              }
            }
            if (__all(ok)) break;
            const int ws = wait_state(a, t0, poll, a.wait_ticks);
            if (ws == WAIT_OBSERVED) {
              timed_out = true;
            } else if (ws == WAIT_EXPIRED) {
              timed_out = true;
              int64_t mu_ = -1;
              int mj = -1;
              uint64_t mb = 0;
#pragma unroll
              for (int q = FXC - 1; q >= 0; --q) {
                if (j0 + q < NS) {
                  if (h1 && !slot_full(v1[q])) { mu_ = u1; mj = j0 + q; mb = dbits(v1[q]); }
                  if (h0 && !slot_full(v0[q])) { mu_ = u0; mj = j0 + q; mb = dbits(v0[q]); }
                }
              }
              report_wait(a, WAIT_FX_MAIL, s, c, ok, mu_, mj, mb, poll, t0);
              raise_abort(a);
            } else {
              __builtin_amdgcn_s_sleep(1);
            }
          }
#pragma unroll
          for (int q = 0; q < FXC; ++q) {
            if (j0 + q < NS) {
              acc[j0 + q] = 0.0;
              if (h0) acc[j0 + q] += v0[q];
              if (h1) acc[j0 + q] += v1[q];
            }
          }
        }
        if (timed_out) s_fx_abort = 1;
        __syncthreads();
        if (!s_fx_abort) {
          const int nrun = g.units_per_rank * NS;
          hyper_finish<D, K, REPLAY, NS, NT>(a.h, c, s, 0, acc, red, tot, var_iw, var_chi, var_noise, &l2, [&] {
            for (int e = (int)threadIdx.x - 64; e >= 0 && e < g.world_size * nrun; e += NT - 64) {
              const int q = e / nrun;
              st_sys((double*)mb + (int64_t)q * mail_rank + (e - q * nrun), slot_empty());
            }
          });
        }
      }
      if (threadIdx.x == 0) CLV_STAMP(a.stamps, s, 3, false);
    }
  }
}


template <int D, int K, bool REPLAY, bool FX>
__global__ __launch_bounds__(BLOCK) void sweep_kernel(SweepArgs a) {
  sweep_body<D, K, REPLAY, FX>(a);
}
template <int D, int K, bool REPLAY, bool FX>
__global__ __launch_bounds__(BLOCK, 4) void sweep_kernel_occ4(SweepArgs a) {
  sweep_body<D, K, REPLAY, FX>(a);
}

template <int D, int K, bool REPLAY, bool FX>
hipError_t launch_sweep_t(const SweepArgs& a, hipStream_t st, hipEvent_t e0, hipEvent_t e1) {
  const dim3 grid(a.g.nb_local, a.g.n_chains);
  const dim3 block(BLOCK);
  if constexpr (SweepOcc<D, K>::value >= 4) {
    if (e0) hipExtLaunchKernelGGL((sweep_kernel_occ4<D, K, REPLAY, FX>), grid, block, 0, st, e0, e1, 0, a);
    else hipLaunchKernelGGL((sweep_kernel_occ4<D, K, REPLAY, FX>), grid, block, 0, st, a);
  } else {
    if (e0) hipExtLaunchKernelGGL((sweep_kernel<D, K, REPLAY, FX>), grid, block, 0, st, e0, e1, 0, a);
    else hipLaunchKernelGGL((sweep_kernel<D, K, REPLAY, FX>), grid, block, 0, st, a);
  }
  return hipGetLastError();
}

template <int D, int K, bool P2P, bool SPLIT = false>
__device__ __forceinline__ void persist_level2(const SweepArgs& a, int64_t s_first, int64_t n_sweeps, int c, uint32_t k0,
                                            uint32_t k1, int64_t wgi, int64_t it_stamp, double* pool) {
  constexpr int NT = BLOCK;
  constexpr int NXY = K * D;
  constexpr int NYY = D * (D + 1) / 2;
  constexpr int NS = NXY + NYY + 1;
  constexpr int NTRIL = D * (D - 1) / 2;
  (void)NXY;
  __shared__ double red[BLOCK / 64][NS];
  __shared__ double tot[NS];
  __shared__ double Hs[HS];
  __shared__ uint32_t s_abort;
  __shared__ double var_iw[4], var_chi[4], var_noise[32];
  __shared__ L2Scratch l2;
  __shared__ double* s_peers[P2P ? MAX_WORLD : 1];
  const Geometry& g = a.g;
  const int tid0 = threadIdx.x;
  (void)wgi;
  static_assert(!(SPLIT && P2P), "the split layout is world size 1 only");
  double* parts0 = a.pblock + (int64_t)c * (SPLIT ? split_records(g.nb_local) : g.nb_local) * NS;
  if (tid0 == 0) s_abort = 0;
  if constexpr (P2P) {
    if (tid0 < g.world_size) s_peers[tid0] = a.peers[tid0];
  }
  __syncthreads();
  __builtin_amdgcn_s_setprio(3);
  stage_prior(a.h.V, &l2);
  const double* pin = P2P ? nullptr : a.pend_in;
  double* pout = P2P ? nullptr : a.pend_out;
  ClockMark clk_prev = CLV_CLOCK_RECORD && a.clk && c == 0 ? ClockMark::now() : ClockMark{0, 0};
  for (int64_t it = pin ? -1 : 0; it < n_sweeps; ++it) {
    int tid = tid0;
    double* parts = parts0;
    if constexpr (CLV_L2_OPAQUE(P2P)) {
      asm volatile("" : "+v"(tid));
      asm volatile("" : "+s"(parts));
    }
    const int64_t s = s_first + it;
    const bool stp = tid == 0 && it == it_stamp;
    (void)stp;
    const int64_t hs = (D == 2) ? s + 1 : s;
    const bool from_pend = it < 0;
    const bool defer_now = pout && it == n_sweeps - 1;
    CLV_P_STAMP(a.stamps, wgi, 0, stp);
    if (!defer_now) {
      if (tid < NTRIL) var_iw[tid] = hyper_normal(k0, k1, HSLOT_NORMAL0 + tid, (uint32_t)hs);
      if (tid >= 32 && tid < 32 + D * K) var_noise[tid - 32] = hyper_normal(k0, k1, HSLOT_BETA_NORMAL0 + (tid - 32), (uint32_t)hs);
      if (tid >= 64 && tid < 64 + D) var_chi[tid - 64] = chi2_draw(k0, k1, (uint32_t)hs, tid - 64, a.h.nu_n - D + 1 + (tid - 64));
    }
    if (from_pend && tid < NS) tot[tid] = pin[(int64_t)c * NS + tid];
    __syncthreads();
    if (!defer_now && tid == 0) bartlett_inverse<D>(var_iw, var_chi, l2.Ai);
    CLV_P_STAMP(a.stamps, wgi, 1, stp);
    if (!from_pend) {
    double v0[NS], v1[NS];
    int eb = -1, er = 0, src = tid & 63;
    if constexpr (SPLIT) {
      const int bm = tid - 1, bp = tid + 1;
      if (tid % 3 == 1 && tid < g.nb_local) {
        eb = tid;
        src = (tid & 63) != 63 ? src + 1 : src - 1;
      } else if (bm >= 0 && bm % 3 == 1 && (bm & 63) != 63 && bm < g.nb_local) {
        eb = bm;
        er = 1;
      } else if (bp % 3 == 1 && (bp & 63) == 63 && bp < g.nb_local) {
        eb = bp;
        er = 1;
      }
    }
    const bool own_split = SPLIT && eb == tid;
    const int b0 = tid, b1 = SPLIT ? eb : tid + NT;
    const bool hb0 = b0 < g.nb_local, hb1 = SPLIT ? eb >= 0 : b1 < g.nb_local;
    double* pb0 = parts + (int64_t)b0 * NS;
    double* pb1 = parts + (int64_t)(SPLIT ? g.nb_local + 2 * (eb / 3) + er : b1) * NS;
    const double* qb0 = hb0 ? pb0 : parts;
    const double* qb1 = hb1 ? pb1 : parts;
    const int64_t per_rank = (int64_t)g.n_chains * NS * g.units_per_rank;
    const double* mb = a.mail + (int64_t)(s & 1) * g.world_size * per_rank + (int64_t)c * NS * g.units_per_rank;
    const int64_t u0 = tid, u1 = tid + NT;
    const int r0 = (int)(u0 / g.units_per_rank), r1 = (int)(u1 / g.units_per_rank);
    const int l0 = (int)(u0 % g.units_per_rank), l1 = (int)(u1 % g.units_per_rank);
    const double* p0 = mb + r0 * per_rank + (int64_t)l0 * NS;
    const double* p1 = mb + r1 * per_rank + (int64_t)l1 * NS;
    const bool h0 = u0 < g.n_units_global, h1 = u1 < g.n_units_global;
    const bool m0 = P2P && h0 && r0 != a.rank, m1 = P2P && h1 && r1 != a.rank;
    const double* q0 = m0 ? p0 : mb;
    const double* q1 = m1 ? p1 : mb;
    double w0[NS], w1[NS];
    bool mdone = !(m0 || m1);
    if constexpr (P2P) {
      if (tid == 0) post_progress(a, s_peers, s);
    }
    const uint64_t t0 = __builtin_amdgcn_s_memrealtime();
    {
      bool done = false;
      for (uint32_t poll = 0;; ++poll) {
        if (!done) {
          bool ok = true;
#pragma unroll
          for (int j = 0; j < NS; ++j) {
            v0[j] = ld_wt(qb0 + j);
            v1[j] = ld_wt(qb1 + j);
          }
#pragma unroll
          for (int j = 0; j < NS; ++j) ok = ok & (!hb0 | slot_full(v0[j])) & (!hb1 | slot_full(v1[j]));
          done = ok;
        }
        if constexpr (P2P) {
          if (!mdone) {
            bool ok = true;
#pragma unroll
            for (int j = 0; j < NS; ++j) {
              w0[j] = ld_sys(q0 + j);
              w1[j] = ld_sys(q1 + j);
            }
#pragma unroll
            for (int j = 0; j < NS; ++j) ok = ok & (!m0 | slot_full(w0[j])) & (!m1 | slot_full(w1[j]));
            mdone = ok;
          }
        }
        if (__all(done)) break;
        const int ws = wait_state(a, t0, poll, a.wait_ticks);
        if (ws == WAIT_OBSERVED) {
          s_abort = 1;
          break;
        }
        if (ws == WAIT_EXPIRED) {
          int64_t mb_ = -1;
          int mj = -1;
          uint64_t mbits = 0;
#pragma unroll
          for (int j = NS - 1; j >= 0; --j) {
            if (hb1 && !slot_full(v1[j])) { mb_ = b1; mj = j; mbits = dbits(v1[j]); }
            if (hb0 && !slot_full(v0[j])) { mb_ = b0; mj = j; mbits = dbits(v0[j]); }
          }
          report_wait(a, WAIT_BLOCKS, s, c, done, mb_, mj, mbits, poll, t0);
          raise_abort(a);
// ... 41 lines not shown
          for (int j = 0; j < NS; ++j) t[j] = v[j];
        } else {
#pragma unroll
          for (int j = 0; j < NS; ++j) t[j] = 0.0 + v[j];
          for (int k = 1; k < bpu; ++k) {
#pragma unroll
            for (int j = 0; j < NS; ++j) t[j] += __shfl(v[j], lane + k, 64);
          }
        }
        if (tid % bpu == 0 && ub < ul) {
#pragma unroll
          for (int j = 0; j < NS; ++j) umail[ub * NS + j] = t[j];
        }
      }
      lds_barrier();
      CLV_P_STAMP(a.stamps, wgi, 10, stp);
      const int64_t dst = ((int64_t)(s & 1) * g.world_size + a.rank) * per_rank + (int64_t)c * NS * g.units_per_rank;
      for (int e = tid; e < NS * ul; e += NT) {
        const double v = umail[e];
        for (int q = 0; q < g.world_size; ++q)
          if (q != a.rank) st_sys(s_peers[q] + dst + e, v);
      }
      const uint64_t tw = t0;
      for (uint32_t poll = 0; !__all(mdone); ++poll) {
        if (!mdone) {
          bool ok = true;
#pragma unroll
          for (int j = 0; j < NS; ++j) {
            w0[j] = ld_sys(q0 + j);
            w1[j] = ld_sys(q1 + j);
          }
#pragma unroll
          for (int j = 0; j < NS; ++j) ok = ok & (!m0 | slot_full(w0[j])) & (!m1 | slot_full(w1[j]));
          mdone = ok;
        }
        if (__all(mdone)) break;
        const int ws = wait_state(a, tw, poll, a.wait_ticks);
        if (ws == WAIT_OBSERVED) {
          s_abort = 1;
          break;
        }
        if (ws == WAIT_EXPIRED) {
          int64_t mu_ = -1;
          int mj = -1;
          uint64_t mbits = 0;
#pragma unroll
          for (int j = NS - 1; j >= 0; --j) {
            if (m1 && !slot_full(w1[j])) { mu_ = u1; mj = j; mbits = dbits(w1[j]); }
            if (m0 && !slot_full(w0[j])) { mu_ = u0; mj = j; mbits = dbits(w0[j]); }
          }
          report_wait(a, WAIT_P2P_MAIL, s, c, mdone, mu_, mj, mbits, poll, tw);
          raise_abort(a);
          s_abort = 1;
          break;
        }
        __builtin_amdgcn_s_sleep(1);
      }
      CLV_P_STAMP(a.stamps, wgi, 11, stp);
      lds_barrier();
      if (s_abort) return;
#pragma unroll
      for (int j = 0; j < NS; ++j) {
        const double x0 = m0 ? w0[j] : (h0 ? umail[l0 * NS + j] : 0.0);
        const double x1 = m1 ? w1[j] : (h1 ? umail[l1 * NS + j] : 0.0);
        acc[j] = 0.0;
        if (h0) acc[j] += x0;
        if (h1) acc[j] += x1;
      }
    }
    block_reduce<NS, NT, P2P>(acc, red, tot);
    CLV_P_STAMP(a.stamps, wgi, 6, stp);
    const int rt = tid - 64;
    if (rt >= 0) {
      const int nrec = (SPLIT ? split_records(g.nb_local) : g.nb_local) * NS;
      for (int e = rt; e < nrec; e += NT - 64) st_wt(parts + e, slot_empty());
      if ((it > 0 || pin) && rt < HS) st_wt(a.hyp2 + ((int64_t)(s & 1) * g.n_chains + c) * HS + rt, slot_empty());
    }
    if constexpr (P2P) {
      const int nrun = g.units_per_rank * NS;
      for (int e = rt; rt >= 0 && e < g.world_size * nrun; e += NT - 64) {
        const int q = e / nrun;
        if (q != a.rank) st_sys((double*)mb + (int64_t)q * per_rank + (e - q * nrun), slot_empty());
      }
    }
    }
    if (defer_now) {
      if (tid < NS) pout[(int64_t)c * NS + tid] = tot[tid];
      if (tid == 0) {
        if (is_stored(s, g)) a.h.loglik[(int64_t)c * g.n_draws + draw_index(s, g)] = tot[NS - 1] / (double)g.n_global;
        a.ctrl_rw->cur = s;
      }
      return;
    }
    if (tid < HS) Hs[tid] = 0.0;
    level2_draw<D, K, P2P ? 6 : CLV_L2_LANE0_MAX>(tot, var_iw, var_chi, var_noise, false, &l2, l2.Ai);
    CLV_P_STAMP(a.stamps, wgi, 7, stp);
    if (tid == 0) {
      double Sig[D][D];
#pragma unroll
      for (int p = 0; p < D; ++p)
#pragma unroll
        for (int q = 0; q < D; ++q) Sig[p][q] = l2.Sig[p * D + q];
      finalize_hyper<D, K, true, CLV_L2_NR != 0>(l2.beta, Sig, a.h.omega2, Hs);
    }
    CLV_P_STAMP(a.stamps, wgi, 3, stp);
    asm volatile("s_waitcnt vmcnt(0)" ::: "memory");
    __syncthreads();
    const bool last = it == n_sweeps - 1;
    if (tid < HS) {
      if (last) a.hyper_out[(int64_t)c * HS + tid] = Hs[tid];
      else st_wt(a.hyp2 + ((int64_t)((s + 1) & 1) * g.n_chains + c) * HS + tid, Hs[tid]);
    }
    CLV_P_STAMP(a.stamps, wgi, 4, stp);
    CLV_P_STAMP(a.stamps, wgi, 5, tid == 0 && it + 1 == it_stamp);
    if (CLV_CLOCK_RECORD && a.clk && c == 0 && tid == 0) clk_prev = clock_mark(a.clk, s, clk_prev);
#ifdef CLV_STAMPS
    if (tid == 0 && a.stamps && c < 8 && it % 4 == 0 && it / 4 < 1024)
      a.stamps[(it / 4) * 8 + c] = __builtin_amdgcn_s_memrealtime();
#endif
    const bool store_l2 = hs >= 1 && is_stored(hs, g);
    double* o = store_l2 ? a.h.level2 + ((int64_t)c * g.n_draws + draw_index(hs, g)) * g.l2w : nullptr;
    if (tid < K * D && store_l2) o[(tid % D) * K + tid / D] = l2.beta[tid];
    if (tid == 0) {
      if (store_l2) {
        int q = K * D;
#pragma unroll
        for (int p = 0; p < D; ++p)
#pragma unroll
          for (int r = p; r < D; ++r) o[q++] = l2.Sig[p * D + r];
      }
      if (!from_pend && is_stored(s, g)) a.h.loglik[(int64_t)c * g.n_draws + draw_index(s, g)] = tot[NS - 1] / (double)g.n_global;
      if (last) a.ctrl_rw->cur = s;
    }
    __syncthreads();
  }
  return;
}

__device__ __forceinline__ const SweepArgs& kernargs_fresh() {
  auto p4 = (const __attribute__((address_space(4))) SweepArgs*)__builtin_amdgcn_kernarg_segment_ptr();
  asm volatile("" : "+s"(p4));
  return *(const SweepArgs*)p4;
}

#ifndef CLV_PERSIST_FRESH_ARGS
#define CLV_PERSIST_FRESH_ARGS 1
#endif
template <bool FRESH>
__device__ __forceinline__ const SweepArgs& loop_args(const SweepArgs& a) {
  if constexpr (FRESH) return kernargs_fresh();
  else return a;
}

template <int D, int K, bool P2P>
__global__ __launch_bounds__(BLOCK, 2) void persist_kernel(SweepArgs a, int64_t s_first, int64_t n_sweeps) {
  constexpr int NXY = K * D;
  constexpr int NYY = D * (D + 1) / 2;
  constexpr int NS = NXY + NYY + 1;
  __shared__ double red[BLOCK / 64][NS];
  __shared__ double tot[NS];
  __shared__ __attribute__((aligned(16))) double exp_tab[D == 3 ? FAST_TAB_N3 : FAST_TAB_N];
  __shared__ double Hs[HS];
  __shared__ uint32_t s_abort;
  __shared__ __attribute__((aligned(16))) char pool[PRE_LDS_BYTES];
  static_assert(UMAIL * sizeof(double) <= PRE_LDS_BYTES, "the level-2 unit partials share the variates' LDS");
  __shared__ double zeta_lds[D == 3 ? BLOCK : 1];
// ... 58 lines not shown
          if (__all(slot_full(v))) {
            Hs[tid] = v;
            break;
          }
          const int ws = wait_state(a, t0, poll, hyper_wait_ticks(a));
          if (ws != WAIT_GOING) {
            if (ws == WAIT_EXPIRED) {
              report_wait(a, WAIT_HYPER, s, c, slot_full(v), b, tid, dbits(v), poll, t0);
              raise_abort(a);
            }
            if (tid == 0) s_abort = 1;
            break;
          }
          __builtin_amdgcn_s_sleep(1);
        }
      }
      __syncthreads();
      if (s_abort) return;
    }
    CLV_P_STAMP(a.stamps, wgi, 1, stp);
    StatGen<D, K> st{};
    CustOut<D> out{};
    __builtin_amdgcn_s_setprio(2);
    if (cu.active) {
      cust_coeffs<D, K, false>(cu, Hs, exp_tab);
      CLV_P_STAMP(a.stamps, wgi, 2, stp);
      const double s00 = Hs[H_S00];
      const double s11 = Hs[H_S11];
      if (pre) mh_run_pre(cu, pv, s00, s11, g.S, exp_tab);
      else mh_run(cu, SlotPhilox(k0, k1, cu.gi, (uint32_t)s), s00, s11, g.S, exp_tab);
      CLV_P_STAMP(a.stamps, wgi, 3, stp);
      if constexpr (D == 3) {
        if (!pre) zeta_lds[tid] = eta_normal(k0, k1, cu.gi, s, exp_tab);
      }
      out = cust_finish<D, K, false>(cu, a, s, stored, Hs, k0, k1, nullptr, exp_tab, st,
                                     D == 3 ? &zeta_lds[tid] : nullptr);
    }
    CLV_P_STAMP(a.stamps, wgi, 4, stp);
#if PERSIST_REDUCE_GEN
    block_reduce_gen<NS, SWEEP_REDUCE_CHUNK>(st, red, tot);
#else
    {
      double acc[NS];
#pragma unroll
      for (int j = 0; j < NS; ++j) acc[j] = st(j);
      block_reduce<NS>(acc, red, tot);
    }
#endif
    if (tid < NS) st_wt(parts + (int64_t)b * NS + tid, tot[tid]);
    __builtin_amdgcn_s_setprio(0);
    CLV_P_STAMP(a.stamps, wgi, 5, stp);
    CLV_P_STAMP(a.stamps, wgi, 8, stp);
    CLV_P_STAMP(a.stamps, wgi, 9, stp);
#ifdef CLV_STAMPS
    if (stp && a.stamps) a.stamps[1024 * 8 + wgi * 12 + 11] = blockIdx.y * gridDim.x + blockIdx.x;
#endif
    if (cu.active) {
      cust_store<D, K>(cu, out, a, c, s, stored, false);
      if (it + 1 < n_sweeps) {
        cust_ztau<D, K, false>(cu, a, s + 1, k0, k1, nullptr, exp_tab);
        if (pre) mh_pre_variates(SlotPhilox(k0, k1, cu.gi, (uint32_t)(s + 1)), g.S, pv);
        if constexpr (D == 3) {
          if (pre) zeta_lds[tid] = eta_normal(k0, k1, cu.gi, s + 1, exp_tab);
        }
      }
    }
    CLV_P_STAMP(a.stamps, wgi, 6, stp);
  }
  if (cu.active) {
    const int64_t ci = (int64_t)c * g.n + cu.i;
    a.lam_out[ci] = cu.lam;
    a.mu_out[ci] = cu.mu;
  }
}

#ifndef CLV_SPLIT_HELP_CHUNKS
#define CLV_SPLIT_HELP_CHUNKS 2
#endif
constexpr int SPLIT_NC = SPLIT_CW * 64;
constexpr int SPLIT_PRE_LDS_BYTES = PRE_STEPS * SPLIT_NC * 12;

constexpr int RELAY_REC = 11;

template <int D, int K, int R>
__device__ __forceinline__ void split_relay_sweeps(const SweepArgs& a_launch, int64_t s_first, int64_t n_sweeps, int c,
                                                   int p, uint32_t k0, uint32_t k1, int64_t wgi, int64_t it_stamp,
                                                   double* parts, char* pool, double (*red)[K * D + D * (D + 1) / 2 + 1],
                                                   const double* exp_tab, double* Hs, uint32_t* s_abort) {
  constexpr int NS = K * D + D * (D + 1) / 2 + 1;
  constexpr int MC = MH_CHUNK_STEPS;
  constexpr int NQ = PRE_STEPS / MC;
  static_assert(R > 0 && R % MC == 0 && R < PRE_STEPS, "relay point: whole chunks, inside the pool");
  constexpr SplitRelayPlan PLAN = split_relay_plan(PRE_STEPS, R);
  static_assert(PLAN.own_begin == 0 && PLAN.own_end == PLAN.relay_begin && PLAN.own_end % MC == 0 && PLAN.relay_end == PRE_STEPS,
                "the relay plan cuts between chunks");
  static_assert(split_relay_plan(R + 1, R).own_end == PLAN.own_end, "one cut for every relayed S");
  constexpr int QR = PLAN.relay_begin / MC;
  __shared__ double relay_rec[RELAY_REC][128];
  __shared__ double relay_ret[4][128];
  __shared__ uint32_t relay_flag[2];
  __shared__ uint32_t relay_abort;
  (void)wgi;
  (void)it_stamp;
  const int tid = threadIdx.x;
  const int wave = __builtin_amdgcn_readfirstlane(tid >> 6);
  const bool first_wait = a_launch.pend_in != nullptr;
  if (tid < 2) relay_flag[tid] = 0;
  if (tid == 2) relay_abort = 0;
  constexpr int DRAW = SPLIT_RELAY_DRAW;
  constexpr int HC1 = split_draw_gap1_chunks(DRAW);
  constexpr bool GAP2 = split_draw_plan(R, DRAW, 4, QR).slot == DRAW_GAP2;
  static_assert(HC1 <= QR, "gap 1 draws owner chunks only");
  static_assert(HC1 == 0 || (split_draw_plan(R, DRAW, 0, HC1 - 1).wave == SPLIT_CW && split_draw_plan(R, DRAW, 4, HC1 - 1).wave == SPLIT_CW &&
                             split_draw_plan(R, DRAW, 1, HC1 - 1).wave == SPLIT_CW + 1 && split_draw_plan(R, DRAW, 5, HC1 - 1).wave == SPLIT_CW + 1 &&
                             split_draw_plan(R, DRAW, 0, HC1).slot == DRAW_WINDOW && split_draw_plan(R, DRAW, 2, 0).slot == DRAW_WINDOW),
                "gap 1: the first HC1 chunks of rows 0 and 4 by wavefront 6, of rows 1 and 5 by wavefront 7");
  static_assert(GAP2 == (split_draw_plan(R, DRAW, 5, QR).slot == DRAW_GAP2) && split_draw_plan(R, DRAW, 4, QR - 1).slot != DRAW_GAP2,
                "gap 2: the relay wavefront's own chunks, the same of rows 4 and 5");
  constexpr int STAGE_STEPS = (HC1 > 0 ? HC1 : 1) * MC;
  float2* stage_t = nullptr;
  float* stage_u = nullptr;
  uint32_t* relay_drawn = nullptr;
  uint32_t* relay_arrive = nullptr;
  if constexpr (HC1 > 0) {
    __shared__ __attribute__((aligned(16))) char stage[4 * STAGE_STEPS * 64 * 12];
    __shared__ uint32_t drawn[4];
    stage_t = (float2*)stage;
    stage_u = (float*)(stage + 4 * STAGE_STEPS * 64 * 8);
    relay_drawn = drawn;
  }
  if constexpr (GAP2) {
    __shared__ uint32_t arrive;
    relay_arrive = &arrive;
    if (tid == 3) arrive = 0;
  }

  if (wave >= SPLIT_CW) {
    const int rw = wave - SPLIT_CW;
    const int rl = tid - SPLIT_CW * 64;
    const PreVariates pv{(float2*)pool, (float*)(pool + PRE_STEPS * SPLIT_NC * 8), tid - 128};
    Cust<D, K> cu;
    {
      const Geometry& g = a_launch.g;
      const int64_t i = (int64_t)p * SPLIT_NC + (tid - 128);
      cu.active = i < g.n;
      cu.i = cu.active ? i : (g.n > 0 ? g.n - 1 : 0);
      cu.xr_[0] = 1.0;
#pragma unroll
      for (int k = 1; k < K; ++k) cu.xr_[k] = a_launch.cov[(int64_t)(k - 1) * g.n + cu.i];
      cu.gi = (uint32_t)(g.shard_begin + cu.i);
      cu.xm = 0.0;
      cu.lc.omz = 0.0;
      if (cu.active) mh_pre_variates_range<QR, NQ, SPLIT_NC>(SlotPhilox(k0, k1, cu.gi, (uint32_t)s_first), g.S, pv);
    }
    __syncthreads();
    for (int64_t it = 0; it < n_sweeps; ++it) {
      const SweepArgs& a = loop_args<CLV_PERSIST_FRESH_ARGS != 0>(a_launch);
      const Geometry& g = a.g;
      if (it > 0 || first_wait) {
        __syncthreads();
        if (*s_abort) return;
      }
      const int64_t s = uniform64(s_first + it);
      const bool stored = is_stored(s, g);
      const uint32_t tag = (uint32_t)it + 1u;
      const bool ahead = it + 1 < n_sweeps;
      if constexpr (HC1 > 0) {
        if (ahead) {
          const int S = opaque_uniform(g.S);
          uint32_t have[2] = {0u, 0u};
          bool go = true;
#pragma unroll
          for (int q = 0; q < HC1; ++q) {
#pragma unroll
            for (int t = 0; t < 2; ++t) {
              if (q * MC < S) {
                if (go)
                  go = (uint32_t)__builtin_amdgcn_readfirstlane(
                           (int)__hip_atomic_load(&relay_flag[rw], __ATOMIC_RELAXED, __HIP_MEMORY_SCOPE_WORKGROUP)) != tag;
                if (go) {
                  const int64_t i = (int64_t)p * SPLIT_NC + (rw + 4 * t) * 64 + (tid & 63);
                  if (i < g.n) {
                    const SlotPhilox ph(k0, k1, (uint32_t)(g.shard_begin + i), (uint32_t)(s + 1));
                    float tl[MC], tm[MC], lu[MC];
                    mh_chunk_variates(ph, (uint32_t)q, tl, tm, lu);
                    const int col = ((2 * t + rw) * STAGE_STEPS + q * MC) * 64 + (tid & 63);
#pragma unroll
                    for (int st = 0; st < MC; ++st) {
                      stage_t[col + st * 64] = make_float2(tl[st], tm[st]);
                      stage_u[col + st * 64] = q * MC + st < S ? lu[st] : __builtin_inff();
                    }
                  }
                  have[t] |= 1u << q;
                }
              }
            }
          }
          if ((tid & 63) == 0) {
            relay_drawn[rw] = have[0];
            relay_drawn[2 + rw] = have[1];
          }
        }
        CLV_R_STAMP(a, wgi, 12 + rw, it == it_stamp);
      }
      bool seen = true;
      {
        const uint64_t t0 = __builtin_amdgcn_s_memrealtime();
        for (uint32_t poll = 0;; ++poll) {
          const uint32_t f = (uint32_t)__builtin_amdgcn_readfirstlane(
              (int)__hip_atomic_load(&relay_flag[rw], __ATOMIC_RELAXED, __HIP_MEMORY_SCOPE_WORKGROUP));
          if (f == tag) break;
          const int ws = wait_state(a, t0, poll, a.wait_ticks);
          if (ws != WAIT_GOING) {
            if (ws == WAIT_EXPIRED) {
              report_wait(a, WAIT_RELAY, s, c, false, p, 4 + rw, f, poll, t0);
              raise_abort(a);
            }
            if ((tid & 63) == 0) relay_abort = 1;
            seen = false;
            break;
          }
          __builtin_amdgcn_s_sleep(1);
        }
      }
      __builtin_amdgcn_fence(__ATOMIC_ACQUIRE, "workgroup", "local");
      CLV_R_STAMP(a, wgi, 2 * rw, it == it_stamp);
      StatGen<D, K> st{};
      __builtin_amdgcn_s_setprio(3);
      if (seen && cu.active) {
        cu.fc.A = relay_rec[0][rl];
        cu.fc.B = relay_rec[1][rl];
        cu.fc.C = relay_rec[2][rl];
        cu.fc.Dl = relay_rec[3][rl];
        cu.fc.El = relay_rec[4][rl];
        cu.fc.w = relay_rec[5][rl];
        cu.ll = relay_rec[6][rl];
        cu.lm = relay_rec[7][rl];
        cu.cur = relay_rec[8][rl];
        cu.lc.w = cu.fc.w;
        if (stored) {
          cu.xm = relay_rec[9][rl];
          cu.lc.omz = relay_rec[10][rl];
        }
        mh_run_pre_range<QR, NQ, SPLIT_NC>(cu, pv, Hs[H_S00], Hs[H_S11], g.S, exp_tab);
        const CustOut<D> out = cust_finish<D, K, false>(cu, a, s, stored, Hs, k0, k1, nullptr, exp_tab, st, nullptr);
        relay_ret[0][rl] = out.lam;
        relay_ret[1][rl] = out.mu;
        relay_ret[2][rl] = cu.ll;
        relay_ret[3][rl] = cu.lm;
      }
      wave_reduce_gen_row<NS, SWEEP_REDUCE_CHUNK>(st, red[4 + rw]);
      CLV_R_STAMP(a, wgi, 2 * rw + 1, it == it_stamp);
      if constexpr (GAP2) {
        uint32_t have = 0u;
        if (ahead) {
          __builtin_amdgcn_s_setprio(0);
          const int S = opaque_uniform(g.S);
          const SlotPhilox ph(k0, k1, cu.gi, (uint32_t)(s + 1));
          bool go = true;
#pragma unroll
          for (int q = QR; q < NQ; ++q) {
            if (split_draw_plan(R, DRAW, 4, q).slot == DRAW_GAP2 && q * MC < S) {
              if (go)
                go = (int32_t)((uint32_t)__builtin_amdgcn_readfirstlane(
                                   (int)__hip_atomic_load(relay_arrive, __ATOMIC_RELAXED, __HIP_MEMORY_SCOPE_WORKGROUP)) -
                               ((tag - 1u) * (uint32_t)SPLIT_CW + (uint32_t)SPLIT_RELAY_GAP2_STOP)) < 0;
              if (go) {
                if (cu.active) {
                  float tl[MC], tm[MC], lu[MC];
                  mh_chunk_variates(ph, (uint32_t)q, tl, tm, lu);
#pragma unroll
                  for (int st = 0; st < MC; ++st) {
                    const int k = q * MC + st;
                    pv.t[k * SPLIT_NC + pv.lane] = make_float2(tl[st], tm[st]);
                    pv.u[k * SPLIT_NC + pv.lane] = k < S ? lu[st] : __builtin_inff();
                  }
                }
                have |= 1u << q;
              }
            }
          }
        }
        CLV_R_STAMP(a, wgi, 14 + rw, it == it_stamp);
        __syncthreads();
        __builtin_amdgcn_s_setprio(0);
        if (relay_abort) return;
        if (cu.active && ahead)
          mh_pre_variates_window<QR, NQ, SPLIT_NC, SPLIT_NC, false>(SlotPhilox(k0, k1, cu.gi, (uint32_t)(s + 1)), g.S, pv, pv, have);
      } else {
        __syncthreads();
        __builtin_amdgcn_s_setprio(0);
        if (relay_abort) return;
        if (cu.active && ahead)
          mh_pre_variates_range<QR, NQ, SPLIT_NC>(SlotPhilox(k0, k1, cu.gi, (uint32_t)(s + 1)), g.S, pv);
      }
    }
    return;
  }

  const bool relayed = wave >= 4;
  const int rl = tid - 4 * 64;
  const PreVariates pv{(float2*)pool, (float*)(pool + PRE_STEPS * SPLIT_NC * 8), tid};
  CLV_P_STAMP(a_launch.stamps, wgi, 7, tid == 0);
  Cust<D, K> cu;
  {
    const int64_t i = (int64_t)p * SPLIT_NC + tid;
    cu.active = i < a_launch.g.n;
    cu.i = cu.active ? i : (a_launch.g.n > 0 ? a_launch.g.n - 1 : 0);
  }
  cust_load(cu, a_launch, c);
  __syncthreads();
  if (cu.active) {
    cust_ztau<D, K, false>(cu, a_launch, s_first, k0, k1, nullptr, exp_tab);
    const SlotPhilox ph(k0, k1, cu.gi, (uint32_t)s_first);
    mh_pre_variates_range<0, QR, SPLIT_NC>(ph, a_launch.g.S, pv);
    if (!relayed) mh_pre_variates_range<QR, NQ, SPLIT_NC>(ph, a_launch.g.S, pv);
  }
  CLV_P_STAMP(a_launch.stamps, wgi, 10, tid == 0);
  for (int64_t it = 0; it < n_sweeps; ++it) {
    const SweepArgs& a = loop_args<CLV_PERSIST_FRESH_ARGS != 0>(a_launch);
    const Geometry& g = a.g;
    const double* hyp_c = a.hyp2 + (int64_t)c * HS;
    const int64_t s = uniform64(s_first + it);
    const bool stored = is_stored(s, g);
    const bool stp = tid == 0 && it == it_stamp;
    (void)stp;
    CLV_P_STAMP(a.stamps, wgi, 0, stp);
    if (it > 0 || first_wait) {
      if (tid < 64) {
        const double* src = hyp_c + (int64_t)(s & 1) * g.n_chains * HS;
        const uint64_t t0 = __builtin_amdgcn_s_memrealtime();
        for (uint32_t poll = 0;; ++poll) {
          const double v = ld_wt(src + tid);
          if (__all(slot_full(v))) {
            Hs[tid] = v;
            break;
          }
          const int ws = wait_state(a, t0, poll, hyper_wait_ticks(a));
          if (ws != WAIT_GOING) {
            if (ws == WAIT_EXPIRED) {
              report_wait(a, WAIT_HYPER, s, c, slot_full(v), p, tid, dbits(v), poll, t0);
              raise_abort(a);
            }
            if (tid == 0) *s_abort = 1;
            break;
          }
          __builtin_amdgcn_s_sleep(1);
        }
      }
      __syncthreads();
      if (*s_abort) return;
    }
    CLV_P_STAMP(a.stamps, wgi, 1, stp);
    StatGen<D, K> st{};
    CustOut<D> out{};
    if (relayed) {
      __builtin_amdgcn_s_setprio(3);
      if (cu.active) {
        cust_coeffs<D, K, false>(cu, Hs, exp_tab);
        mh_run_pre_range<0, QR, SPLIT_NC>(cu, pv, Hs[H_S00], Hs[H_S11], g.S, exp_tab);
        relay_rec[0][rl] = cu.fc.A;
        relay_rec[1][rl] = cu.fc.B;
        relay_rec[2][rl] = cu.fc.C;
        relay_rec[3][rl] = cu.fc.Dl;
        relay_rec[4][rl] = cu.fc.El;
        relay_rec[5][rl] = cu.fc.w;
        relay_rec[6][rl] = cu.ll;
        relay_rec[7][rl] = cu.lm;
        relay_rec[8][rl] = cu.cur;
        if (stored) {
          relay_rec[9][rl] = cu.xm;
          relay_rec[10][rl] = cu.lc.omz;
        }
      }
      __builtin_amdgcn_fence(__ATOMIC_RELEASE, "workgroup", "local");
      if ((tid & 63) == 0)
        __hip_atomic_store(&relay_flag[wave - 4], (uint32_t)it + 1u, __ATOMIC_RELAXED, __HIP_MEMORY_SCOPE_WORKGROUP);
    } else {
      __builtin_amdgcn_s_setprio(2);
      if (cu.active) {
        cust_coeffs<D, K, false>(cu, Hs, exp_tab);
        CLV_P_STAMP(a.stamps, wgi, 2, stp);
        mh_run_pre_range<0, QR, SPLIT_NC>(cu, pv, Hs[H_S00], Hs[H_S11], g.S, exp_tab);
        mh_run_pre_range<QR, NQ, SPLIT_NC>(cu, pv, Hs[H_S00], Hs[H_S11], g.S, exp_tab);
        CLV_P_STAMP(a.stamps, wgi, 3, stp);
        out = cust_finish<D, K, false>(cu, a, s, stored, Hs, k0, k1, nullptr, exp_tab, st, nullptr);
      }
      CLV_P_STAMP(a.stamps, wgi, 4, stp);
      wave_reduce_gen<NS, SWEEP_REDUCE_CHUNK>(st, red);
    }
    if constexpr (GAP2) {
      if ((tid & 63) == 0) __hip_atomic_fetch_add(relay_arrive, 1u, __ATOMIC_RELAXED, __HIP_MEMORY_SCOPE_WORKGROUP);
    }
    __syncthreads();
    if (relay_abort) return;
    {
      const int j = tid & 63;
      const int r0 = SPLIT_CW * p;
      if (j < NS && tid < 128) {
        if ((p & 1) == 0) {
          if (tid < 64) {
            st_wt(parts + (int64_t)(r0 / 4) * NS + j, ((red[0][j] + red[1][j]) + red[2][j]) + red[3][j]);
          } else {
            const int b = r0 / 4 + 1;
            if (b < g.nb_local) st_wt(parts + (int64_t)b * NS + j, red[4][j] + red[5][j]);
          }
        } else {
          if (tid < 64) {
            const int b = (r0 - 2) / 4;
            double* ext = parts + (int64_t)(g.nb_local + 2 * (b / 3)) * NS;
            st_wt(ext + j, red[0][j]);
            st_wt(ext + NS + j, red[1][j]);
          } else {
            const int b = (r0 + 2) / 4;
            if (b < g.nb_local) st_wt(parts + (int64_t)b * NS + j, ((red[2][j] + red[3][j]) + red[4][j]) + red[5][j]);
          }
        }
      }
    }
    __builtin_amdgcn_s_setprio(0);
    CLV_P_STAMP(a.stamps, wgi, 5, stp);
    CLV_P_STAMP(a.stamps, wgi, 8, stp);
    CLV_P_STAMP(a.stamps, wgi, 9, stp);
#ifdef CLV_STAMPS
    if (stp && a.stamps) a.stamps[1024 * 8 + wgi * 12 + 11] = blockIdx.y * gridDim.x + blockIdx.x;
#endif
    if (cu.active) {
      if (relayed) {
        cu.lam = relay_ret[0][rl];
        cu.mu = relay_ret[1][rl];
        out = CustOut<D>{cu.lam, cu.mu, 1.0, relay_ret[2][rl], relay_ret[3][rl], 0.0};
      }
      cust_store<D, K>(cu, out, a, c, s, stored, false);
      if (it + 1 < n_sweeps) {
        cust_ztau<D, K, false>(cu, a, s + 1, k0, k1, nullptr, exp_tab);
        const SlotPhilox ph(k0, k1, cu.gi, (uint32_t)(s + 1));
        if constexpr (HC1 > 0) {
          const int w = __builtin_amdgcn_readfirstlane(tid >> 6);
          const int sr = 2 * (w >> 2) + (w & 1);
          const uint32_t have = (w & 3) < 2 ? relay_drawn[sr] : 0u;
          const PreVariates sv{stage_t + sr * STAGE_STEPS * 64, stage_u + sr * STAGE_STEPS * 64, tid & 63};
          mh_pre_variates_window<0, HC1, SPLIT_NC, 64, true>(ph, g.S, pv, sv, have);
          mh_pre_variates_range<HC1, QR, SPLIT_NC>(ph, g.S, pv);
        } else {
          mh_pre_variates_range<0, QR, SPLIT_NC>(ph, g.S, pv);
        }
        if (!relayed) mh_pre_variates_range<QR, NQ, SPLIT_NC>(ph, g.S, pv);
      }
    }
    CLV_P_STAMP(a.stamps, wgi, 6, stp);
  }
  if (cu.active) {
    const int64_t ci = (int64_t)c * a_launch.g.n + cu.i;
    a_launch.lam_out[ci] = cu.lam;
    a_launch.mu_out[ci] = cu.mu;
  }
}

template <int D, int K, int HC, int R = 0>
__global__ __launch_bounds__(SPLIT_NT, 1) void persist_kernel_split(SweepArgs a, int64_t s_first, int64_t n_sweeps) {
  static_assert(D == 2, "the split layout is bivariate");
  constexpr int NXY = K * D;
  constexpr int NYY = D * (D + 1) / 2;
  constexpr int NS = NXY + NYY + 1;
  constexpr int MC = MH_CHUNK_STEPS;
  constexpr int NQ = PRE_STEPS / MC;
  static_assert(HC >= 0 && HC <= NQ, "helper share");
  __shared__ double red[SPLIT_CW][NS];
  __shared__ __attribute__((aligned(16))) double exp_tab[FAST_TAB_N];
  __shared__ double Hs[HS];
  __shared__ uint32_t s_abort;
  __shared__ __attribute__((aligned(16))) char pool[SPLIT_PRE_LDS_BYTES];
  const Geometry& g = a.g;
  const int nwg = split_wgs(g.nb_local);
  int c = blockIdx.y, p = blockIdx.x;
  if (a.wg_map) {
    const int32_t m = a.wg_map[blockIdx.y * gridDim.x + blockIdx.x];
    c = m >> 16;
    p = m & 0xFFFF;
  }
  const int tid = threadIdx.x;
  const int wave = __builtin_amdgcn_readfirstlane(tid >> 6);
  const int64_t wgi = (int64_t)c * (nwg + 1) + p;
  const int64_t it_stamp = n_sweeps >= 2 ? n_sweeps - 2 : 0;
  (void)wgi;
  (void)it_stamp;
  uint32_t k0, k1;
  chain_key(a.r.seed, (int64_t)a.r.chain_first + c, &k0, &k1);
  double* parts = a.pblock + (int64_t)c * split_records(g.nb_local) * NS;
  if (tid == 0) s_abort = 0;

  if (p == nwg) {
    if (tid >= BLOCK) return;
    persist_level2<D, K, false, true>(a, s_first, n_sweeps, c, k0, k1, wgi, it_stamp, (double*)pool);
    return;
  }

  const PreVariates pv{(float2*)pool, (float*)(pool + PRE_STEPS * SPLIT_NC * 8), tid};
  fast_tab_fill(exp_tab, tid, SPLIT_NT, false);
  if (tid < HS) Hs[tid] = a.hyper[(int64_t)c * HS + tid];
  const bool first_wait = a.pend_in != nullptr;
  CLV_R_STAMP(a, wgi, 4 + wave, true);
  if constexpr (R > 0) {
    split_relay_sweeps<D, K, R>(a, s_first, n_sweeps, c, p, k0, k1, wgi, it_stamp, parts, pool, red, exp_tab, Hs, &s_abort);
    return;
  }

  if (wave >= SPLIT_CW) {
    const int h = wave - SPLIT_CW;
    uint32_t gi[2];
    bool on[2];
    int col[2];
#pragma unroll
    for (int t = 0; t < 2; ++t) {
      col[t] = (h + 4 * t) * 64 + (tid & 63);
      const int64_t i = (int64_t)p * SPLIT_NC + col[t];
      on[t] = i < g.n;
      gi[t] = (uint32_t)(g.shard_begin + i);
    }
    __syncthreads();
    for (int64_t it = 0; it < n_sweeps; ++it) {
      if (it > 0 || first_wait) {
        __syncthreads();
        if (s_abort) return;
      }
      const bool ahead = HC > 0 && it + 1 < n_sweeps;
      const int S = opaque_uniform(loop_args<CLV_PERSIST_FRESH_ARGS != 0>(a).g.S);
      float tl[2][HC > 0 ? HC : 1][MC], tm[2][HC > 0 ? HC : 1][MC], lu[2][HC > 0 ? HC : 1][MC];
      if (ahead) {
#pragma unroll
        for (int t = 0; t < 2; ++t) {
          if (on[t]) {
            const SlotPhilox ph(k0, k1, gi[t], (uint32_t)(s_first + it + 1));
#pragma unroll
            for (int q = 0; q < HC; ++q)
              if (q * MC < S) mh_chunk_variates(ph, (uint32_t)q, tl[t][q], tm[t][q], lu[t][q]);
          }
        }
      }
      __syncthreads();
      if (ahead) {
#pragma unroll
        for (int t = 0; t < 2; ++t) {
          if (on[t]) {
#pragma unroll
            for (int q = 0; q < HC; ++q) {
              if (q * MC < S) {
#pragma unroll
                for (int st = 0; st < MC; ++st) {
                  const int k = q * MC + st;
                  pv.t[k * SPLIT_NC + col[t]] = make_float2(tl[t][q][st], tm[t][q][st]);
                  pv.u[k * SPLIT_NC + col[t]] = k < S ? lu[t][q][st] : __builtin_inff();
                }
              }
            }
          }
        }
      }
    }
    return;
  }

  CLV_P_STAMP(a.stamps, wgi, 7, tid == 0);
  Cust<D, K> cu;
  {
    const int64_t i = (int64_t)p * SPLIT_NC + tid;
    cu.active = i < g.n;
    cu.i = cu.active ? i : (g.n > 0 ? g.n - 1 : 0);
  }
  cust_load(cu, a, c);
  __syncthreads();
  if (cu.active) {
    cust_ztau<D, K, false>(cu, a, s_first, k0, k1, nullptr, exp_tab);
    mh_pre_variates<NQ, SPLIT_NC>(SlotPhilox(k0, k1, cu.gi, (uint32_t)s_first), g.S, pv);
  }
  CLV_P_STAMP(a.stamps, wgi, 10, tid == 0);
  const SweepArgs& a_launch = a;
  for (int64_t it = 0; it < n_sweeps; ++it) {
    const SweepArgs& a = loop_args<CLV_PERSIST_FRESH_ARGS != 0>(a_launch);
    const Geometry& g = a.g;
    const double* hyp_c = a.hyp2 + (int64_t)c * HS;
    const int64_t s = uniform64(s_first + it);
    const bool stored = is_stored(s, g);
    const bool stp = tid == 0 && it == it_stamp;
    (void)stp;
    CLV_P_STAMP(a.stamps, wgi, 0, stp);
    if (it > 0 || first_wait) {
// ... 457 lines not shown
  H[H_P00] = prec[0];
  H[H_P01] = prec[1];
  H[H_P11] = prec[2];
  Cust<2, 1> u;
  u.xr_[0] = 1.0;
  u.xm = (double)x[i];
  u.z = z[i] != 0;
  u.lc.xm = u.xm;
  u.lc.omz = u.z ? 0.0 : 1.0;
  u.lc.w = u.z ? T[i] : tau[i];
  u.ll = cur_pt[2 * i];
  u.lm = cur_pt[2 * i + 1];
  cust_coeffs<2, 1, false>(u, H, tab);
  const double cur0 = u.cur;
  const double pl = clip70_fma(scale[0], (double)t3[2 * i], u.ll);
  const double pm = prop_lm(scale[1], (double)t3[2 * i + 1], u.lm);
  const double plp = log_post_fast(u.fc, pl, pm, tab);
  mh_step(u, scale[0], scale[1], t3[2 * i], t3[2 * i + 1], log_u[i], tab);
  double* o = out + 7 * i;
  o[0] = cur0;
  o[1] = plp;
  o[2] = pl;
  o[3] = pm;
  o[4] = u.ll;
  o[5] = u.lm;
  o[6] = u.cur;
}

#ifdef CLV_ONLY_K
#define CLV_FOR_K(M, D, R) M(D, CLV_ONLY_K, R)
#else
#define CLV_FOR_K(M, D, R) \
  M(D, 1, R) M(D, 2, R) M(D, 3, R) M(D, 4, R) M(D, 5, R) M(D, 6, R) M(D, 7, R) M(D, 8, R) M(D, 9, R)
#endif

hipError_t launch_sweep(const SweepArgs& a, bool replay, hipStream_t st, hipEvent_t e0, hipEvent_t e1) {
  const bool fx = a.fuse && a.g.world_size > 1;
#define CLV_CASE(DD, KK, RR)                                                      \
  if (a.g.D == DD && a.g.K == KK && replay == RR) {                               \
    if constexpr (!RR) {                                                          \
      if (fx) return launch_sweep_t<DD, KK, RR, true>(a, st, e0, e1);             \
    }                                                                             \
    return launch_sweep_t<DD, KK, RR, false>(a, st, e0, e1);                      \
  }
  CLV_FOR_K(CLV_CASE, 2, false)
  CLV_FOR_K(CLV_CASE, 3, false)
  CLV_FOR_K(CLV_CASE, 2, true)
  CLV_FOR_K(CLV_CASE, 3, true)
#undef CLV_CASE
  return hipErrorInvalidValue;
}

hipError_t launch_persist_flush(const SweepArgs& a, int64_t s_first, hipStream_t st) {
  const dim3 grid(1, a.g.n_chains);
#define CLV_CASE(DD, KK, PP)                                                                     \
  if (a.g.D == DD && a.g.K == KK) {                                                              \
    hipLaunchKernelGGL((persist_flush_kernel<DD, KK>), grid, dim3(BLOCK), 0, st, a, s_first);  \
    return hipGetLastError();                                                                  \
  }
  CLV_FOR_K(CLV_CASE, 2, false)
  CLV_FOR_K(CLV_CASE, 3, false)
#undef CLV_CASE
  return hipErrorInvalidValue;
}

hipError_t launch_persist(const SweepArgs& a, int64_t s_first, int64_t n_sweeps, hipStream_t st, hipEvent_t e0,
                          hipEvent_t e1) {
  const dim3 grid(a.g.nb_local + 1, a.g.n_chains);
  const dim3 block(BLOCK);
#define CLV_CASE(DD, KK, PP)                                                                                         \
  if (a.g.D == DD && a.g.K == KK && (a.g.world_size > 1) == PP) {                                                \
    if (e0) hipExtLaunchKernelGGL((persist_kernel<DD, KK, PP>), grid, block, 0, st, e0, e1, 0, a, s_first, n_sweeps); \
    else hipLaunchKernelGGL((persist_kernel<DD, KK, PP>), grid, block, 0, st, a, s_first, n_sweeps);                  \
    return hipGetLastError();                                                                                      \
  }
  CLV_FOR_K(CLV_CASE, 2, false)
  CLV_FOR_K(CLV_CASE, 3, false)
  CLV_FOR_K(CLV_CASE, 2, true)
  CLV_FOR_K(CLV_CASE, 3, true)
#undef CLV_CASE
  return hipErrorInvalidValue;
}

hipError_t launch_persist_split(const SweepArgs& a, int64_t s_first, int64_t n_sweeps, hipStream_t st, bool relay) {
  const dim3 grid(split_wgs(a.g.nb_local) + 1, a.g.n_chains);
  if (relay && !(SPLIT_RELAY_STEPS > 0 && a.g.S > SPLIT_RELAY_STEPS)) return hipErrorInvalidValue;
#define CLV_CASE(DD, KK, PP)                                                                                        \
  if (a.g.D == DD && a.g.K == KK && relay) {                                                                      \
    hipLaunchKernelGGL((persist_kernel_split<DD, KK, CLV_SPLIT_HELP_CHUNKS, SPLIT_RELAY_STEPS>), grid, dim3(SPLIT_NT), 0, st, a, s_first, n_sweeps); \
    return hipGetLastError();                                                                                     \
  }                                                                                                               \
  if (a.g.D == DD && a.g.K == KK) {                                                                               \
    hipLaunchKernelGGL((persist_kernel_split<DD, KK, CLV_SPLIT_HELP_CHUNKS>), grid, dim3(SPLIT_NT), 0, st, a, s_first, n_sweeps); \
    return hipGetLastError();                                                                                     \
  }
  CLV_FOR_K(CLV_CASE, 2, false)
#undef CLV_CASE
  return hipErrorInvalidValue;
}

hipError_t persist_split_resources(int D, int K, int* blocks_per_cu, size_t* scratch_bytes, bool relay) {
  hipFuncAttributes fa{};
  if (relay && SPLIT_RELAY_STEPS <= 0) return hipErrorInvalidValue;
#define CLV_CASE(DD, KK, PP)                                                                                      \
  if (D == DD && K == KK && relay) {                                                                              \
    hipError_t e = hipOccupancyMaxActiveBlocksPerMultiprocessor(blocks_per_cu, persist_kernel_split<DD, KK, CLV_SPLIT_HELP_CHUNKS, SPLIT_RELAY_STEPS>, SPLIT_NT, 0); \
    if (e != hipSuccess) return e;                                                                                \
    e = hipFuncGetAttributes(&fa, reinterpret_cast<const void*>(&persist_kernel_split<DD, KK, CLV_SPLIT_HELP_CHUNKS, SPLIT_RELAY_STEPS>)); \
    *scratch_bytes = fa.localSizeBytes;                                                                           \
    return e;                                                                                                     \
  }                                                                                                               \
  if (D == DD && K == KK) {                                                                                       \
    hipError_t e = hipOccupancyMaxActiveBlocksPerMultiprocessor(blocks_per_cu, persist_kernel_split<DD, KK, CLV_SPLIT_HELP_CHUNKS>, SPLIT_NT, 0); \
    if (e != hipSuccess) return e;                                                                                \
    e = hipFuncGetAttributes(&fa, reinterpret_cast<const void*>(&persist_kernel_split<DD, KK, CLV_SPLIT_HELP_CHUNKS>)); \
    *scratch_bytes = fa.localSizeBytes;                                                                           \
    return e;                                                                                                     \
  }
  CLV_FOR_K(CLV_CASE, 2, false)
#undef CLV_CASE
  return hipErrorInvalidValue;
}

hipError_t persist_occupancy(int D, int K, bool p2p, int* blocks_per_cu) {
#define CLV_CASE(DD, KK, PP) \
  if (D == DD && K == KK && p2p == PP) return hipOccupancyMaxActiveBlocksPerMultiprocessor(blocks_per_cu, persist_kernel<DD, KK, PP>, BLOCK, 0);
  CLV_FOR_K(CLV_CASE, 2, false)
  CLV_FOR_K(CLV_CASE, 3, false)
  CLV_FOR_K(CLV_CASE, 2, true)
  CLV_FOR_K(CLV_CASE, 3, true)
#undef CLV_CASE
  return hipErrorInvalidValue;
}

hipError_t persist_scratch_bytes(int D, int K, bool p2p, size_t* bytes) {
  hipFuncAttributes fa{};
#define CLV_CASE(DD, KK, PP)                                                                     \
  if (D == DD && K == KK && p2p == PP) {                                                         \
    const hipError_t e = hipFuncGetAttributes(&fa, reinterpret_cast<const void*>(&persist_kernel<DD, KK, PP>)); \
    *bytes = fa.localSizeBytes;                                                                  \
    return e;                                                                                    \
  }
  CLV_FOR_K(CLV_CASE, 2, false)
  CLV_FOR_K(CLV_CASE, 3, false)
  CLV_FOR_K(CLV_CASE, 2, true)
  CLV_FOR_K(CLV_CASE, 3, true)
#undef CLV_CASE
  return hipErrorInvalidValue;
}

hipError_t launch_group(const GroupArgs& a, hipStream_t st) {
  const int units_local = (a.g.nb_local + a.g.blocks_per_unit - 1) / a.g.blocks_per_unit;
  hipLaunchKernelGGL(group_kernel, dim3(units_local, a.g.n_chains), dim3(64), 0, st, a);
  return hipGetLastError();
}

hipError_t launch_hyper(const HyperArgs& a, bool replay, hipStream_t st) {
#define CLV_CASE(DD, KK, RR) \
  if (a.g.D == DD && a.g.K == KK && replay == RR) { hipLaunchKernelGGL((hyper_kernel<DD, KK, RR>), dim3(a.g.n_chains), dim3(256), 0, st, a); return hipGetLastError(); }
  CLV_FOR_K(CLV_CASE, 2, false)
  CLV_FOR_K(CLV_CASE, 3, false)
  CLV_FOR_K(CLV_CASE, 2, true)
  CLV_FOR_K(CLV_CASE, 3, true)
#undef CLV_CASE
  return hipErrorInvalidValue;
}

hipError_t launch_set_hyper(int D, int K, int n_chains, double* hyper, const double* bs, double omega2,
                            bool replay, hipStream_t st) {
#define CLV_CASE(DD, KK, RR) \
  if (D == DD && K == KK && replay == RR) { hipLaunchKernelGGL((set_hyper_kernel<DD, KK, !RR && CLV_L2_NR != 0>), dim3(1), dim3(64), 0, st, n_chains, hyper, bs, omega2); return hipGetLastError(); }
  CLV_FOR_K(CLV_CASE, 2, false)
  CLV_FOR_K(CLV_CASE, 3, false)
  CLV_FOR_K(CLV_CASE, 2, true)
  CLV_FOR_K(CLV_CASE, 3, true)
#undef CLV_CASE
  return hipErrorInvalidValue;
}

hipError_t launch_debug_philox(uint32_t k0, uint32_t k1, const uint32_t* ctr, int64_t n, uint32_t* out,
                               hipStream_t st) {
  hipLaunchKernelGGL(debug_philox_kernel, dim3((unsigned)((n + 255) / 256)), dim3(256), 0, st, k0, k1, ctr, n, out);
  return hipGetLastError();
}

hipError_t launch_debug_variates(uint64_t seed, int chain, uint32_t sweep, int64_t n, int S, float* tl,
                                 float* tm, float* ua, float* l2u, double* uz, double* ut, double* ea, double* ez,
// ... 130 lines not shown
```

mcmc_clv_model_amd/sampler.py:

```python
from __future__ import annotations

import ctypes
import weakref
import math
from dataclasses import dataclass, field
from typing import List, Optional, Sequence

import numpy as np

from . import _lib
from ._lib import check, dptr

BLOCK_SIZE = _lib.BLOCK


@dataclass
class Problem:
    D: int
    K: int
    x: np.ndarray
    t_x: np.ndarray
    T_cal: np.ndarray
    cov: np.ndarray
    log_s: Optional[np.ndarray]
# ... 130 lines not shown
        data.T_cal = p.T_cal.ctypes.data if p.N else None
        data.covariates = p.cov.ctypes.data if (p.K > 1 and p.N) else None
        data.log_s = p.log_s.ctypes.data if (p.D == 3 and p.N) else None
        self.prior = prior if prior is not None else make_prior(p, cfg.n_global)
        h = ctypes.c_void_p()
        check(L.clv_create(ctypes.byref(cfg), ctypes.byref(data), ctypes.byref(self.prior), ctypes.byref(h)))
        self.h = h
        self._L = L

    def close(self) -> None:
        for grp in list(getattr(self, "_groups", ())):
            grp.close()
        if getattr(self, "h", None):
            self._L.clv_destroy(self.h)
            self.h = None

    def __del__(self):
        try:
            self.close()
        except Exception:
            pass

    def __enter__(self):
        return self

    def __exit__(self, *exc):
        self.close()

    def run(self, n_sweeps: int) -> None:
        check(self._L.clv_run(self.h, int(n_sweeps)))

    def rollback(self) -> None:
        check(self._L.clv_rollback(self.h))

    def sweep(self) -> None:
        check(self._L.clv_sweep(self.h))

    def hyper(self, gathered_ptr: Optional[int] = None) -> None:
        check(self._L.clv_hyper(self.h, gathered_ptr))

    def partials(self):
        ptr = ctypes.c_void_p()
        nd = ctypes.c_int64()
        st = ctypes.c_int32()
        check(self._L.clv_partials(self.h, ctypes.byref(ptr), ctypes.byref(nd), ctypes.byref(st)))
        return ptr.value, nd.value, st.value

    def set_stream(self, stream: int) -> None:
        check(self._L.clv_set_stream(self.h, int(stream)))

    def note_sweeps(self, n: int) -> None:
        check(self._L.clv_note_sweeps(self.h, int(n)))

    def copy_partials(self, dst_ptr: int) -> None:
        check(self._L.clv_copy_partials(self.h, ctypes.c_void_p(dst_ptr)))

    def synchronize(self) -> None:
        check(self._L.clv_synchronize(self.h))

    def host_times(self) -> dict:
        hn = (ctypes.c_int64 * 8)()
        check(self._L.clv_debug_host_times(self.h, hn))
        h = [x / 1e3 for x in hn]
        if not h[0] or not h[6]:
            return {}
        names = ("set_device", "start_event", "launch_call", "end_event", "wait", "return")
        return {k: round(h[i + 1] - h[i], 3) for i, k in enumerate(names)}

    def clock_ghz(self) -> float:
        v = ctypes.c_double(0.0)
        check(self._L.clv_clock_ghz(self.h, ctypes.byref(v)))
        return float(v.value)

    def clock_probe(self, us: float = 50.0) -> float:
        v = ctypes.c_double(0.0)
        check(self._L.clv_clock_probe(self.h, float(us), ctypes.byref(v)))
        return float(v.value)

    def launch_info(self) -> dict:
        out = (ctypes.c_int64 * 6)()
        check(self._L.clv_launch_info(self.h, out))
        relay = ctypes.c_int32(0)
        check(self._L.clv_split_relay_steps(self.h, ctypes.byref(relay)))
        return dict(persistent=bool(out[0]), persist_blocks_per_cu=int(out[1]), n_cu=int(out[2]),
                    workgroups=int(out[3]), physical_workgroups=int(out[4]),
                    layout={1: "block", 2: "split", -1: "block (split aborted)"}.get(int(out[5])),
                    relay_steps=int(relay.value))

    IPC_HANDLE_BYTES = 64

    def p2p_info(self) -> dict:
        out = (ctypes.c_int64 * 6)()
        check(self._L.clv_p2p_info(self.h, out))
        return dict(capable=bool(out[0]), connected=bool(out[1]), mail_bytes=int(out[2]), mail_ptr=int(out[3]),
                    persistent=bool(out[4]), mail_memory={0: "uncached", 1: "fine-grained", 2: "device"}.get(int(out[5])))

    def p2p_export(self) -> bytes:
        buf = ctypes.create_string_buffer(self.IPC_HANDLE_BYTES)
        check(self._L.clv_p2p_export(self.h, buf))
        return buf.raw

    def p2p_connect(self, handles: Optional[Sequence[bytes]] = None, ptrs: Optional[Sequence[int]] = None) -> None:
        if handles is not None:
            blob = ctypes.create_string_buffer(b"".join(handles), self.IPC_HANDLE_BYTES * len(handles))
            check(self._L.clv_p2p_connect(self.h, blob, None))
        else:
            arr = (ctypes.c_uint64 * len(ptrs))(*[int(p) for p in ptrs])
            check(self._L.clv_p2p_connect(self.h, None, arr))

    def p2p_set_persistent(self, on: bool) -> None:
        check(self._L.clv_p2p_set_persistent(self.h, 1 if on else 0))

    def p2p_disconnect(self) -> None:
        check(self._L.clv_p2p_disconnect(self.h))

    def set_wait_timeout(self, ms: float) -> None:
        check(self._L.clv_set_wait_timeout(self.h, float(ms)))

    @property
    def sweeps_done(self) -> int:
        return int(self._L.clv_sweeps_done(self.h))

    def set_replay_tape(self, tape: np.ndarray, n_sweeps: int) -> None:
        tape = np.ascontiguousarray(tape, dtype=np.float64)
        stride = self.replay_sweep_stride
        if tape.size != self.chains * n_sweeps * stride:
            raise ValueError(f"tape has {tape.size} doubles, expected {self.chains * n_sweeps * stride}")
        check(self._L.clv_set_replay_tape(self.h, dptr(tape), int(n_sweeps)))

    @property
    def replay_sweep_stride(self) -> int:
        return int(self._L.clv_replay_sweep_stride(self.h))

    def level1_buffer(self) -> np.ndarray:
        return np.empty((self.chains, self.n_draws, self.n, self.D + 2))

    def stream_draws(self, level1: Optional[np.ndarray]) -> None:
        if level1 is not None:
            C, nd, n, D = self.chains, self.n_draws, self.n, self.D
            if (level1.shape != (C, nd, n, D + 2) or level1.dtype != np.float64 or not level1.flags.c_contiguous
                    or not level1.flags.writeable):
                raise ValueError("level1 must be a writeable C-contiguous float64 array of shape (chains, n_draws, n, D+2)")
        self._stream_buf = level1
        check(self._L.clv_stream_draws(self.h, dptr(level1)))

    def read_draws(self, level1: bool = True, out: Optional[np.ndarray] = None):
        C, nd, n, D, K = self.chains, self.n_draws, self.n, self.D, self.K
        l1 = None
        if level1 and self.draw_sink == "full":
            l1 = out if out is not None else self.level1_buffer()
        l2 = np.empty((C, nd, D * K + D * (D + 1) // 2))
        ll = np.empty((C, nd))
        check(self._L.clv_read_draws(self.h, dptr(l1), dptr(l2), dptr(ll)))
        return l1, l2, ll

    def flush(self) -> None:
        hyp = np.empty((self.chains, self.K * self.D + self.D * self.D))
        check(self._L.clv_get_state(self.h, None, None, dptr(hyp)))

    def read_summary(self):
        sums = np.empty((self.chains, _lib.N_SUM_STATS, self.n))
        k = ctypes.c_int64()
        check(self._L.clv_read_summary(self.h, dptr(sums), ctypes.byref(k)))
        return sums, int(k.value)

    def get_state(self):
        C, n, D, K = self.chains, self.n, self.D, self.K
        lam, mu = np.empty((C, n)), np.empty((C, n))
        hyp = np.empty((C, K * D + D * D))
        check(self._L.clv_get_state(self.h, dptr(lam), dptr(mu), dptr(hyp)))
# ... 523 lines not shown
```

Measured before the change: 11.49 billion.

## Add row-record partials layout for split relay persistent kernel

```diff
diff --git a/include/clvmcmc.h b/include/clvmcmc.h
--- a/include/clvmcmc.h
+++ b/include/clvmcmc.h
@@ -95,6 +95,7 @@
 int clv_clock_probe(clv_sampler* s, double us, double* ghz);
 int clv_launch_info(const clv_sampler* s, int64_t* out);
 int clv_split_relay_steps(const clv_sampler* s, int32_t* out);
+int clv_split_row_records(const clv_sampler* s, int32_t* out);
 #define CLV_IPC_HANDLE_BYTES 64
 int clv_p2p_info(const clv_sampler* s, int64_t* out);
 int clv_p2p_export(clv_sampler* s, void* handle);
@@ -147,6 +148,8 @@
 int clv_debug_split_draw_plan(int32_t R, int32_t share, int32_t* out);
 int clv_debug_split_stamps(clv_sampler* s, uint64_t* out);
 int clv_debug_sweep_plan(const int64_t* in, int32_t* out);
+int clv_debug_sweep_plan_rows(const int64_t* in, int32_t* out);
+int clv_debug_split_row_layout(int32_t nb, int32_t* out, int64_t* counts);
 
 enum { CLV_EXCHANGE_AUTO = 0, CLV_EXCHANGE_P2P = 1, CLV_EXCHANGE_COPY = 2 };
 typedef struct clv_group clv_group;
diff --git a/mcmc_clv_model_amd/_lib.py b/mcmc_clv_model_amd/_lib.py
--- a/mcmc_clv_model_amd/_lib.py
+++ b/mcmc_clv_model_amd/_lib.py
@@ -100,6 +100,7 @@
         "clv_clock_probe": (c_int32, [sp, c_double, POINTER(c_double)]),
         "clv_launch_info": (c_int32, [sp, POINTER(c_int64)]),
         "clv_split_relay_steps": (c_int32, [sp, POINTER(c_int32)]),
+        "clv_split_row_records": (c_int32, [sp, POINTER(c_int32)]),
         "clv_p2p_info": (c_int32, [sp, POINTER(c_int64)]),
         "clv_p2p_export": (c_int32, [sp, c_void_p]),
         "clv_p2p_connect": (c_int32, [sp, c_void_p, POINTER(c_uint64)]),
@@ -134,6 +135,8 @@
                                         POINTER(c_float), dp, POINTER(c_float), dp]),
         "clv_debug_wg_map": (c_int32, [c_int32, c_int32, c_int32, POINTER(c_int32)]),
         "clv_debug_sweep_plan": (c_int32, [POINTER(c_int64), POINTER(c_int32)]),
+        "clv_debug_sweep_plan_rows": (c_int32, [POINTER(c_int64), POINTER(c_int32)]),
+        "clv_debug_split_row_layout": (c_int32, [c_int32, POINTER(c_int32), POINTER(c_int64)]),
         "clv_debug_persist_choice": (c_int32, [c_int32, c_int32, c_int32, c_int64, c_int32, c_int32]),
         "clv_debug_persist_fits": (c_int32, [c_int64, c_int32, c_int32]),
         "clv_group_create": (c_int32, [POINTER(sp), c_int32, c_int32, POINTER(sp)]),
diff --git a/mcmc_clv_model_amd/csrc/capi.hip b/mcmc_clv_model_amd/csrc/capi.hip
--- a/mcmc_clv_model_amd/csrc/capi.hip
+++ b/mcmc_clv_model_amd/csrc/capi.hip
@@ -320,6 +320,10 @@
 #define CLV_SPLIT_RELAY_DEFAULT 1
 #endif
 constexpr bool SPLIT_RELAY_DEFAULT = CLV_SPLIT_RELAY_DEFAULT != 0;
+#ifndef CLV_SPLIT_ROWS_DEFAULT
+#define CLV_SPLIT_ROWS_DEFAULT 1
+#endif
+constexpr bool SPLIT_ROWS_DEFAULT = CLV_SPLIT_ROWS_DEFAULT != 0;
 
 namespace {
 
@@ -409,6 +413,7 @@
   int persistent = -1;
   int layout = 0;
   int relay = -1;
+  int rows = -1;
   bool defer = true;
   int mail_first = 0;
   double wait_ms = 0.0;
@@ -423,6 +428,8 @@
   e.layout = !v ? 0 : is(v, "block") ? LAYOUT_BLOCK : is(v, "split") ? LAYOUT_SPLIT : -1;
   v = std::getenv("CLV_SPLIT_RELAY");
   e.relay = !v ? -1 : is(v, "0") ? 0 : is(v, "1") ? 1 : 2;
+  v = std::getenv("CLV_SPLIT_ROWS");
+  e.rows = !v ? -1 : is(v, "0") ? 0 : is(v, "1") ? 1 : 2;
   e.defer = !is(std::getenv("CLV_DEFER"), "0");
   v = std::getenv("CLV_MAIL_ALLOC");
   e.mail_first = is(v, "fine") ? 1 : is(v, "default") ? 2 : 0;
@@ -436,11 +443,14 @@
 struct SweepResources {
   int n_cu = 0;
   Instance block, split, relay;
+  Instance rows;
 };
 struct SweepPlan {
   bool persistent = false, split = false, p2p_capable = false, p2p_persist_fits = false, fx_capable = false, defer = false;
   int relay_steps = 0;
+  bool rows = false;
   bool need_split = false, need_relay = false;
+  bool need_rows = false;
   const char* error = nullptr;
 };
 
@@ -473,6 +483,7 @@
   if (!(p.persistent && g.D == 2 && g.S <= PRE_STEPS && nb <= SPLIT_MAX_NB)) return p;
   if (e.layout < 0) p.error = "CLV_PERSIST_LAYOUT must be block or split";
   else if (e.relay > 1) p.error = "CLV_SPLIT_RELAY must be 0 or 1";
+  else if (e.rows > 1) p.error = "CLV_SPLIT_ROWS must be 0 or 1";
   if (p.error || e.layout == LAYOUT_BLOCK) return p;
   if (r.split.scratch == NOT_QUERIED) {
     p.need_split = true;
@@ -482,6 +493,10 @@
   if (p.split && SPLIT_RELAY_STEPS > 0 && g.S > SPLIT_RELAY_STEPS && (e.relay < 0 ? SPLIT_RELAY_DEFAULT : e.relay == 1)) {
     if (r.relay.scratch == NOT_QUERIED) p.need_relay = true;
     else if (r.relay.scratch == 0 && persist_split_fits(C, nb, r.relay.bpc, r.n_cu)) p.relay_steps = SPLIT_RELAY_STEPS;
+  }
+  if (p.relay_steps > 0 && (e.rows < 0 ? SPLIT_ROWS_DEFAULT : e.rows == 1)) {
+    if (r.rows.scratch == NOT_QUERIED) p.need_rows = true;
+    else p.rows = r.rows.scratch == 0 && persist_split_fits(C, nb, r.rows.bpc, r.n_cu);
   }
   return p;
 }
@@ -563,10 +578,10 @@
   return CLV_OK;
 }
 
-Instance query_split_instance(const Geometry& g, bool relay) {
+Instance query_split_instance(const Geometry& g, bool relay, bool rows = false) {
   Instance in;
   size_t scratch = 0;
-  const bool ok = persist_split_resources(g.D, g.K, &in.bpc, &scratch, relay) == hipSuccess;
+  const bool ok = persist_split_resources(g.D, g.K, &in.bpc, &scratch, relay, rows) == hipSuccess;
   if (!ok) (void)hipGetLastError();
   in.scratch = ok ? (int64_t)scratch : QUERY_FAILED;
   return in;
@@ -597,10 +612,15 @@
     r.relay = query_split_instance(g, true);
     p = plan_sweep(g, s->replay, r, env);
   }
+  if (p.need_rows) {
+    r.rows = query_split_instance(g, true, true);
+    p = plan_sweep(g, s->replay, r, env);
+  }
   if (p.error) return fail(CLV_EINVAL, p.error);
   s->persistent = p.persistent;
   s->split = p.split;
   s->relay_steps = p.relay_steps;
+  s->row_records = p.rows;
   s->p2p_capable = p.p2p_capable;
   s->p2p_persist_fits = p.p2p_persist_fits;
   s->fx_capable = p.fx_capable;
@@ -899,6 +919,12 @@
   return CLV_OK;
 }
 
+int clv_split_row_records(const clv_sampler* s, int32_t* out) {
+  if (!s || !out) return fail(CLV_EINVAL, "null argument");
+  *out = s->split && s->relay_steps > 0 && s->row_records ? 1 : 0;
+  return CLV_OK;
+}
+
 int clv_p2p_info(const clv_sampler* s, int64_t* out) {
   if (!s || !out) return fail(CLV_EINVAL, "null argument");
   out[0] = (s->p2p_capable || s->fx_capable) ? 1 : 0;
@@ -1035,7 +1061,8 @@
   s->host_ns[2] = host_now_ns();
   if (s->split) {
     a.wg_map = s->d_wgmap_split;
-    CLV_HIP(launch_persist_split(a, s->sweeps_done + 1, n_sweeps, s->stream, s->relay_steps > 0));
+    CLV_HIP(launch_persist_split(a, s->sweeps_done + 1, n_sweeps, s->stream, s->relay_steps > 0,
+                                 s->relay_steps > 0 && s->row_records));
   } else {
     CLV_HIP(launch_persist(a, s->sweeps_done + 1, n_sweeps, s->stream, nullptr, nullptr));
   }
@@ -1081,6 +1108,7 @@
     if (s->split) {
       s->split = false;
       s->relay_steps = 0;
+      s->row_records = false;
       s->split_reverted = true;
       diag += "; the split layout's launch aborted: this handle uses the block layout from now on";
     }
@@ -1584,7 +1612,7 @@
   return split_chosen(n_chains, nb, blocks_per_cu, n_cu, false) ? 1 : 0;
 }
 
-int clv_debug_sweep_plan(const int64_t* in, int32_t* out) {
+static int debug_sweep_plan(const int64_t* in, int32_t* out, bool with_rows) {
   if (!in || !out) return fail(CLV_EINVAL, "null argument");
   Geometry g{};
   g.D = (int)in[0];
@@ -1606,11 +1634,35 @@
   e.layout = (int)in[17];
   e.relay = (int)in[18];
   e.defer = in[19] != 0;
+  r.rows = with_rows ? Instance{(int)in[20], in[21]} : r.relay;
+  if (!with_rows && r.rows.scratch == NOT_QUERIED) r.rows.scratch = QUERY_FAILED;
+  e.rows = with_rows ? (int)in[22] : -1;
   const SweepPlan p = plan_sweep(g, in[8] != 0, r, e);
-  const int32_t o[8] = {p.persistent, p.split, p.relay_steps, p.p2p_capable, p.p2p_persist_fits, p.fx_capable,
-                        p.defer, (p.need_split ? 1 : 0) | (p.need_relay ? 2 : 0)};
-  std::copy(o, o + 8, out);
+  const int32_t o[9] = {p.persistent, p.split, p.relay_steps, p.p2p_capable, p.p2p_persist_fits, p.fx_capable,
+                        p.defer, (p.need_split ? 1 : 0) | (p.need_relay ? 2 : 0) | (p.need_rows ? 4 : 0), p.rows};
+  std::copy(o, o + (with_rows ? 9 : 8), out);
   return p.error ? fail(CLV_EINVAL, p.error) : CLV_OK;
+}
+
+int clv_debug_sweep_plan(const int64_t* in, int32_t* out) { return debug_sweep_plan(in, out, false); }
+int clv_debug_sweep_plan_rows(const int64_t* in, int32_t* out) { return debug_sweep_plan(in, out, true); }
+
+int clv_debug_split_row_layout(int32_t nb, int32_t* out, int64_t* counts) {
+  if (!out || !counts || nb < 1 || nb > SPLIT_MAX_NB) return fail(CLV_EINVAL, "bad arguments");
+  const int nwg = split_wgs(nb);
+  for (int p = 0; p < nwg; ++p)
+    for (int w = 0; w < SPLIT_CW; ++w) {
+      const int row = SPLIT_CW * p + w;
+      out[SPLIT_CW * p + w] = row < split_row_records(nb) ? row : -1;
+    }
+  Geometry g{};
+  g.n_chains = 1;
+  g.nb_local = nb;
+  g.stride = 1;
+  counts[0] = split_records(nb);
+  counts[1] = split_row_records(nb);
+  counts[2] = (int64_t)pblock_count(g);
+  return CLV_OK;
 }
 
 int clv_debug_split_relay_plan(int32_t S, int32_t R, int32_t* out) {
diff --git a/mcmc_clv_model_amd/csrc/internal.h b/mcmc_clv_model_amd/csrc/internal.h
--- a/mcmc_clv_model_amd/csrc/internal.h
+++ b/mcmc_clv_model_amd/csrc/internal.h
@@ -146,6 +146,7 @@
   int persist_bpc = 0, n_cu = 0;
   bool split = false;
   int relay_steps = 0;
+  bool row_records = false;
   bool split_reverted = false;
   clv::DevPtr<int32_t> d_wgmap_split;
   bool p2p_capable = false;
@@ -196,7 +197,10 @@
 inline size_t sums_count(const Geometry& g) { return (size_t)g.n_chains * CLV_N_SUM_STATS * g.n; }
 inline size_t arrive_count(const Geometry& g) { return (size_t)g.n_chains * (1 + g.units_per_rank); }
 inline size_t handoff_count(const Geometry& g) { return 2 * hyper_count(g); }
-inline size_t pblock_count(const Geometry& g) { return (size_t)g.n_chains * split_records(std::max(g.nb_local, 1)) * g.stride; }
+inline size_t pblock_count(const Geometry& g) {
+  const int nb = std::max(g.nb_local, 1);
+  return (size_t)g.n_chains * std::max(split_records(nb), split_row_records(nb)) * g.stride;
+}
 inline size_t unit_count(const Geometry& g) { return (size_t)g.n_chains * g.units_per_rank * g.stride; }
 inline size_t mail_count(const Geometry& g) { return mail_slots(g.world_size, g.n_chains, g.stride, g.units_per_rank) + MAIL_TAIL; }
 inline size_t loglik_count(const Geometry& g) { return (size_t)g.n_chains * g.n_draws; }
diff --git a/mcmc_clv_model_amd/csrc/kernels.h b/mcmc_clv_model_amd/csrc/kernels.h
--- a/mcmc_clv_model_amd/csrc/kernels.h
+++ b/mcmc_clv_model_amd/csrc/kernels.h
@@ -23,6 +23,10 @@
 enum : int { LAYOUT_NONE = 0, LAYOUT_BLOCK = 1, LAYOUT_SPLIT = 2 };
 __host__ __device__ inline int split_wgs(int nb) { return (2 * nb + 2) / 3; }
 __host__ __device__ inline int split_records(int nb) { return nb + 2 * ((nb + 1) / 3); }
+__host__ __device__ inline int split_row_records(int nb) { return 4 * nb; }
+__host__ __device__ inline int64_t split_row_slot(int nb, int rec, int stat) {
+  return ((int64_t)stat * 4 + (rec & 3)) * nb + (rec >> 2);
+}
 enum : int { WAIT_HYPER = 1, WAIT_BLOCKS = 2, WAIT_P2P_MAIL = 3, WAIT_FX_MAIL = 4, WAIT_RELAY = 5 };
 #ifndef CLV_SPLIT_RELAY_STEPS
 #define CLV_SPLIT_RELAY_STEPS 8
@@ -200,8 +204,9 @@
 hipError_t launch_persist(const SweepArgs& a, int64_t s_first, int64_t n_sweeps, hipStream_t st,
                           hipEvent_t e0 = nullptr, hipEvent_t e1 = nullptr);
 hipError_t launch_persist_split(const SweepArgs& a, int64_t s_first, int64_t n_sweeps, hipStream_t st,
-                                bool relay = false);
-hipError_t persist_split_resources(int D, int K, int* blocks_per_cu, size_t* scratch_bytes, bool relay = false);
+                                bool relay = false, bool rows = false);
+hipError_t persist_split_resources(int D, int K, int* blocks_per_cu, size_t* scratch_bytes, bool relay = false,
+                                   bool rows = false);
 hipError_t persist_occupancy(int D, int K, bool p2p, int* blocks_per_cu);
 hipError_t persist_scratch_bytes(int D, int K, bool p2p, size_t* bytes);
 hipError_t launch_persist_flush(const SweepArgs& a, int64_t s_first, hipStream_t st);
diff --git a/mcmc_clv_model_amd/csrc/kernels.hip b/mcmc_clv_model_amd/csrc/kernels.hip
--- a/mcmc_clv_model_amd/csrc/kernels.hip
+++ b/mcmc_clv_model_amd/csrc/kernels.hip
@@ -1922,7 +1922,7 @@
   return hipGetLastError();
 }
 
-template <int D, int K, bool P2P, bool SPLIT = false>
+template <int D, int K, bool P2P, bool SPLIT = false, bool ROWS = false>
 __device__ __forceinline__ void persist_level2(const SweepArgs& a, int64_t s_first, int64_t n_sweeps, int c, uint32_t k0,
                                             uint32_t k1, int64_t wgi, int64_t it_stamp, double* pool) {
   constexpr int NT = BLOCK;
@@ -1942,7 +1942,8 @@
   const int tid0 = threadIdx.x;
   (void)wgi;
   static_assert(!(SPLIT && P2P), "the split layout is world size 1 only");
-  double* parts0 = a.pblock + (int64_t)c * (SPLIT ? split_records(g.nb_local) : g.nb_local) * NS;
+  static_assert(SPLIT || !ROWS, "row records are the split layout's");
+  double* parts0 = a.pblock + (int64_t)c * (ROWS ? split_row_records(g.nb_local) : SPLIT ? split_records(g.nb_local) : g.nb_local) * NS;
   if (tid0 == 0) s_abort = 0;
   if constexpr (P2P) {
     if (tid0 < g.world_size) s_peers[tid0] = a.peers[tid0];
@@ -1977,6 +1978,69 @@
     if (!defer_now && tid == 0) bartlett_inverse<D>(var_iw, var_chi, l2.Ai);
     CLV_P_STAMP(a.stamps, wgi, 1, stp);
     if (!from_pend) {
+    if constexpr (ROWS) {
+    double v[4][NS];
+    const bool hb = tid < g.nb_local;
+    const int nbl = g.nb_local;
+    const uint32_t boff = hb ? (uint32_t)tid : 0u;
+    const uint64_t t0 = __builtin_amdgcn_s_memrealtime();
+    {
+      bool done = false;
+      for (uint32_t poll = 0;; ++poll) {
+        if (!done) {
+          bool ok = true;
+          int nbi = nbl;
+          asm volatile("" : "+s"(nbi));
+#pragma unroll
+          for (int r = 0; r < 4; ++r)
+#pragma unroll
+            for (int j = 0; j < NS; ++j) v[r][j] = ld_wt(parts + (int64_t)(j * 4 + r) * nbi + boff);
+#pragma unroll
+          for (int r = 0; r < 4; ++r)
+#pragma unroll
+            for (int j = 0; j < NS; ++j) ok = ok & (!hb | slot_full(v[r][j]));
+          done = ok;
+        }
+        if (__all(done)) break;
+        const int ws = wait_state(a, t0, poll, a.wait_ticks);
+        if (ws == WAIT_OBSERVED) {
+          s_abort = 1;
+          break;
+        }
+        if (ws == WAIT_EXPIRED) {
+          int mj = -1;
+          uint64_t mbits = 0;
+#pragma unroll
+          for (int r = 3; r >= 0; --r)
+#pragma unroll
+            for (int j = NS - 1; j >= 0; --j)
+              if (hb && !slot_full(v[r][j])) { mj = j; mbits = dbits(v[r][j]); }
+          report_wait(a, WAIT_BLOCKS, s, c, done, tid, mj, mbits, poll, t0);
+          raise_abort(a);
+          s_abort = 1;
+          break;
+        }
+        __builtin_amdgcn_s_sleep(1);
+      }
+    }
+    __syncthreads();
+    if (s_abort) return;
+    CLV_P_STAMP(a.stamps, wgi, 2, stp);
+    double acc[NS];
+#pragma unroll
+    for (int j = 0; j < NS; ++j) {
+      acc[j] = 0.0;
+      if (hb) acc[j] += ((v[0][j] + v[1][j]) + v[2][j]) + v[3][j];
+    }
+    block_reduce<NS, NT, P2P>(acc, red, tot);
+    CLV_P_STAMP(a.stamps, wgi, 6, stp);
+    const int rt = tid - 64;
+    if (rt >= 0) {
+      const int nrec = split_row_records(g.nb_local) * NS;
+      for (int e = rt; e < nrec; e += NT - 64) st_wt(parts + e, slot_empty());
+      if ((it > 0 || pin) && rt < HS) st_wt(a.hyp2 + ((int64_t)(s & 1) * g.n_chains + c) * HS + rt, slot_empty());
+    }
+    } else {
     double v0[NS], v1[NS];
     int eb = -1, er = 0, src = tid & 63;
     if constexpr (SPLIT) {
@@ -2184,6 +2248,7 @@
         const int q = e / nrun;
         if (q != a.rank) st_sys((double*)mb + (int64_t)q * per_rank + (e - q * nrun), slot_empty());
       }
+    }
     }
     }
     if (defer_now) {
@@ -2408,7 +2473,7 @@
 
 constexpr int RELAY_REC = 11;
 
-template <int D, int K, int R>
+template <int D, int K, int R, bool ROWS = false>
 __device__ __forceinline__ void split_relay_sweeps(const SweepArgs& a_launch, int64_t s_first, int64_t n_sweeps, int c,
                                                    int p, uint32_t k0, uint32_t k1, int64_t wgi, int64_t it_stamp,
                                                    double* parts, char* pool, double (*red)[K * D + D * (D + 1) / 2 + 1],
@@ -2435,13 +2500,13 @@
   if (tid == 2) relay_abort = 0;
   constexpr int DRAW = SPLIT_RELAY_DRAW;
   constexpr int HC1 = split_draw_gap1_chunks(DRAW);
-  constexpr bool GAP2 = split_draw_plan(R, DRAW, 4, QR).slot == DRAW_GAP2;
-  static_assert(HC1 <= QR, "gap 1 draws owner chunks only");
+  constexpr bool GAP2 = !ROWS && split_draw_plan(R, DRAW, 4, QR).slot == DRAW_GAP2;
+  static_assert(HC1 <= QR && HC1 <= 8, "gap 1 draws owner chunks only (relay_drawn: a byte of chunk bits)");
   static_assert(HC1 == 0 || (split_draw_plan(R, DRAW, 0, HC1 - 1).wave == SPLIT_CW && split_draw_plan(R, DRAW, 4, HC1 - 1).wave == SPLIT_CW &&
                              split_draw_plan(R, DRAW, 1, HC1 - 1).wave == SPLIT_CW + 1 && split_draw_plan(R, DRAW, 5, HC1 - 1).wave == SPLIT_CW + 1 &&
                              split_draw_plan(R, DRAW, 0, HC1).slot == DRAW_WINDOW && split_draw_plan(R, DRAW, 2, 0).slot == DRAW_WINDOW),
                 "gap 1: the first HC1 chunks of rows 0 and 4 by wavefront 6, of rows 1 and 5 by wavefront 7");
-  static_assert(GAP2 == (split_draw_plan(R, DRAW, 5, QR).slot == DRAW_GAP2) && split_draw_plan(R, DRAW, 4, QR - 1).slot != DRAW_GAP2,
+  static_assert(GAP2 == (!ROWS && split_draw_plan(R, DRAW, 5, QR).slot == DRAW_GAP2) && split_draw_plan(R, DRAW, 4, QR - 1).slot != DRAW_GAP2,
                 "gap 2: the relay wavefront's own chunks, the same of rows 4 and 5");
   constexpr int STAGE_STEPS = (HC1 > 0 ? HC1 : 1) * MC;
   float2* stage_t = nullptr;
@@ -2460,6 +2525,23 @@
     relay_arrive = &arrive;
     if (tid == 3) arrive = 0;
   }
+  uint32_t* relay_back = nullptr;
+  double* rowrec = nullptr;
+  constexpr uint32_t TAGM = 0xFFFFFFu;
+  if constexpr (ROWS) {
+    __shared__ uint32_t back[2];
+    relay_back = back;
+    if (tid >= 4 && tid < 6) back[tid - 4] = 0;
+    if constexpr (HC1 > 0) {
+      if (tid >= 8 && tid < 12) relay_drawn[tid - 8] = 0;
+    }
+    const int row = SPLIT_CW * p + (wave >= SPLIT_CW ? wave - 2 : wave);
+    if (row < split_row_records(a_launch.g.nb_local) && (tid & 63) < NS)
+      rowrec = parts + split_row_slot(a_launch.g.nb_local, row, tid & 63);
+  }
+  (void)TAGM;
+  (void)rowrec;
+  (void)relay_back;
 
   if (wave >= SPLIT_CW) {
     const int rw = wave - SPLIT_CW;
@@ -2486,6 +2568,9 @@
       if (it > 0 || first_wait) {
         __syncthreads();
         if (*s_abort) return;
+        if constexpr (ROWS) {
+          if (relay_abort) return;
+        }
       }
       const int64_t s = uniform64(s_first + it);
       const bool stored = is_stored(s, g);
@@ -2522,7 +2607,13 @@
               }
             }
           }
-          if ((tid & 63) == 0) {
+          if constexpr (ROWS) {
+            __builtin_amdgcn_fence(__ATOMIC_RELEASE, "workgroup", "local");
+            if ((tid & 63) == 0) {
+              __hip_atomic_store(&relay_drawn[rw], ((tag & TAGM) << 8) | have[0], __ATOMIC_RELAXED, __HIP_MEMORY_SCOPE_WORKGROUP);
+              __hip_atomic_store(&relay_drawn[2 + rw], ((tag & TAGM) << 8) | have[1], __ATOMIC_RELAXED, __HIP_MEMORY_SCOPE_WORKGROUP);
+            }
+          } else if ((tid & 63) == 0) {
             relay_drawn[rw] = have[0];
             relay_drawn[2 + rw] = have[1];
           }
@@ -2576,6 +2667,17 @@
         relay_ret[3][rl] = cu.lm;
       }
       wave_reduce_gen_row<NS, SWEEP_REDUCE_CHUNK>(st, red[4 + rw]);
+      if constexpr (ROWS) {
+        __builtin_amdgcn_fence(__ATOMIC_RELEASE, "wavefront");
+        if (seen && rowrec) st_wt(rowrec, red[4 + rw][tid & 63]);
+        CLV_R_STAMP(a, wgi, 2 * rw + 1, it == it_stamp);
+        __builtin_amdgcn_fence(__ATOMIC_RELEASE, "workgroup", "local");
+        if ((tid & 63) == 0) __hip_atomic_store(&relay_back[rw], tag, __ATOMIC_RELAXED, __HIP_MEMORY_SCOPE_WORKGROUP);
+        __builtin_amdgcn_s_setprio(0);
+        if (seen && cu.active && ahead)
+          mh_pre_variates_range<QR, NQ, SPLIT_NC>(SlotPhilox(k0, k1, cu.gi, (uint32_t)(s + 1)), g.S, pv);
+        continue;
+      }
       CLV_R_STAMP(a, wgi, 2 * rw + 1, it == it_stamp);
       if constexpr (GAP2) {
         uint32_t have = 0u;
@@ -2676,6 +2778,9 @@
       }
       __syncthreads();
       if (*s_abort) return;
+      if constexpr (ROWS) {
+        if (relay_abort) return;
+      }
     }
     CLV_P_STAMP(a.stamps, wgi, 1, stp);
     StatGen<D, K> st{};
@@ -2718,6 +2823,46 @@
     if constexpr (GAP2) {
       if ((tid & 63) == 0) __hip_atomic_fetch_add(relay_arrive, 1u, __ATOMIC_RELAXED, __HIP_MEMORY_SCOPE_WORKGROUP);
     }
+    bool back_ok = true;
+    if constexpr (ROWS) {
+      const uint32_t tag = (uint32_t)it + 1u;
+      if (!relayed) {
+        __builtin_amdgcn_fence(__ATOMIC_RELEASE, "wavefront");
+        if (rowrec) st_wt(rowrec, red[wave][tid & 63]);
+        if (wave == 2 || wave == 3) {
+          __builtin_amdgcn_s_setprio(0);
+          const uint64_t t0 = __builtin_amdgcn_s_memrealtime();
+          for (uint32_t poll = 0;; ++poll) {
+            const uint32_t f = (uint32_t)__builtin_amdgcn_readfirstlane(
+                (int)__hip_atomic_load(&relay_back[wave - 2], __ATOMIC_RELAXED, __HIP_MEMORY_SCOPE_WORKGROUP));
+            if (f == tag || wait_state(a, t0, poll, a.wait_ticks) != WAIT_GOING) break;
+            __builtin_amdgcn_s_sleep(2);
+          }
+        }
+      } else {
+        __builtin_amdgcn_s_setprio(0);
+        const uint64_t t0 = __builtin_amdgcn_s_memrealtime();
+        for (uint32_t poll = 0;; ++poll) {
+          const uint32_t f = (uint32_t)__builtin_amdgcn_readfirstlane(
+              (int)__hip_atomic_load(&relay_back[wave - 4], __ATOMIC_RELAXED, __HIP_MEMORY_SCOPE_WORKGROUP));
+          if (f == tag) break;
+          const int ws = wait_state(a, t0, poll, a.wait_ticks);
+          if (ws != WAIT_GOING) {
+            if (ws == WAIT_EXPIRED) {
+              report_wait(a, WAIT_RELAY, s, c, false, p, wave, f, poll, t0);
+              raise_abort(a);
+            }
+            if ((tid & 63) == 0) relay_abort = 1;
+            back_ok = false;
+            break;
+          }
+          __builtin_amdgcn_s_sleep(1);
+        }
+        __builtin_amdgcn_fence(__ATOMIC_ACQUIRE, "workgroup", "local");
+        if (relay_abort) back_ok = false;
+        CLV_R_STAMP(a, wgi, 14 + (wave - 4), it == it_stamp);
+      }
+    } else {
     __syncthreads();
     if (relay_abort) return;
     {
@@ -2744,6 +2889,7 @@
         }
       }
     }
+    }
     __builtin_amdgcn_s_setprio(0);
     CLV_P_STAMP(a.stamps, wgi, 5, stp);
     CLV_P_STAMP(a.stamps, wgi, 8, stp);
@@ -2751,7 +2897,7 @@
 #ifdef CLV_STAMPS
     if (stp && a.stamps) a.stamps[1024 * 8 + wgi * 12 + 11] = blockIdx.y * gridDim.x + blockIdx.x;
 #endif
-    if (cu.active) {
+    if (cu.active && back_ok) {
       if (relayed) {
         cu.lam = relay_ret[0][rl];
         cu.mu = relay_ret[1][rl];
@@ -2764,7 +2910,33 @@
         if constexpr (HC1 > 0) {
           const int w = __builtin_amdgcn_readfirstlane(tid >> 6);
           const int sr = 2 * (w >> 2) + (w & 1);
-          const uint32_t have = (w & 3) < 2 ? relay_drawn[sr] : 0u;
+          uint32_t have = 0u;
+          if constexpr (ROWS) {
+            if ((w & 3) < 2) {
+              const uint32_t tag = ((uint32_t)it + 1u) & TAGM;
+              const uint64_t t0 = __builtin_amdgcn_s_memrealtime();
+              for (uint32_t poll = 0;; ++poll) {
+                have = (uint32_t)__builtin_amdgcn_readfirstlane(
+                    (int)__hip_atomic_load(&relay_drawn[sr], __ATOMIC_RELAXED, __HIP_MEMORY_SCOPE_WORKGROUP));
+                if ((have >> 8) == tag) break;
+                const int ws = wait_state(a, t0, poll, a.wait_ticks);
+                if (ws != WAIT_GOING) {
+                  if (ws == WAIT_EXPIRED) {
+                    report_wait(a, WAIT_RELAY, s, c, false, p, w, have, poll, t0);
+                    raise_abort(a);
+                  }
+                  if ((tid & 63) == 0) relay_abort = 1;
+                  have = 0u;
+                  break;
+                }
+                __builtin_amdgcn_s_sleep(1);
+              }
+              __builtin_amdgcn_fence(__ATOMIC_ACQUIRE, "workgroup", "local");
+              have &= 0xFFu;
+            }
+          } else {
+            have = (w & 3) < 2 ? relay_drawn[sr] : 0u;
+          }
           const PreVariates sv{stage_t + sr * STAGE_STEPS * 64, stage_u + sr * STAGE_STEPS * 64, tid & 63};
           mh_pre_variates_window<0, HC1, SPLIT_NC, 64, true>(ph, g.S, pv, sv, have);
           mh_pre_variates_range<HC1, QR, SPLIT_NC>(ph, g.S, pv);
@@ -2783,7 +2955,7 @@
   }
 }
 
-template <int D, int K, int HC, int R = 0>
+template <int D, int K, int HC, int R = 0, bool ROWS = false>
 __global__ __launch_bounds__(SPLIT_NT, 1) void persist_kernel_split(SweepArgs a, int64_t s_first, int64_t n_sweeps) {
   static_assert(D == 2, "the split layout is bivariate");
   constexpr int NXY = K * D;
@@ -2813,12 +2985,13 @@
   (void)it_stamp;
   uint32_t k0, k1;
   chain_key(a.r.seed, (int64_t)a.r.chain_first + c, &k0, &k1);
-  double* parts = a.pblock + (int64_t)c * split_records(g.nb_local) * NS;
+  static_assert(!ROWS || R > 0, "row records: the relay instance");
+  double* parts = a.pblock + (int64_t)c * (ROWS ? split_row_records(g.nb_local) : split_records(g.nb_local)) * NS;
   if (tid == 0) s_abort = 0;
 
   if (p == nwg) {
     if (tid >= BLOCK) return;
-    persist_level2<D, K, false, true>(a, s_first, n_sweeps, c, k0, k1, wgi, it_stamp, (double*)pool);
+    persist_level2<D, K, false, true, ROWS>(a, s_first, n_sweeps, c, k0, k1, wgi, it_stamp, (double*)pool);
     return;
   }
 
@@ -2828,7 +3001,7 @@
   const bool first_wait = a.pend_in != nullptr;
   CLV_R_STAMP(a, wgi, 4 + wave, true);
   if constexpr (R > 0) {
-    split_relay_sweeps<D, K, R>(a, s_first, n_sweeps, c, p, k0, k1, wgi, it_stamp, parts, pool, red, exp_tab, Hs, &s_abort);
+    split_relay_sweeps<D, K, R, ROWS>(a, s_first, n_sweeps, c, p, k0, k1, wgi, it_stamp, parts, pool, red, exp_tab, Hs, &s_abort);
     return;
   }
 
@@ -3452,10 +3625,15 @@
   return hipErrorInvalidValue;
 }
 
-hipError_t launch_persist_split(const SweepArgs& a, int64_t s_first, int64_t n_sweeps, hipStream_t st, bool relay) {
+hipError_t launch_persist_split(const SweepArgs& a, int64_t s_first, int64_t n_sweeps, hipStream_t st, bool relay, bool rows) {
   const dim3 grid(split_wgs(a.g.nb_local) + 1, a.g.n_chains);
   if (relay && !(SPLIT_RELAY_STEPS > 0 && a.g.S > SPLIT_RELAY_STEPS)) return hipErrorInvalidValue;
+  if (rows && !relay) return hipErrorInvalidValue;
 #define CLV_CASE(DD, KK, PP)                                                                                        \
+  if (a.g.D == DD && a.g.K == KK && rows) {                                                                       \
+    hipLaunchKernelGGL((persist_kernel_split<DD, KK, CLV_SPLIT_HELP_CHUNKS, SPLIT_RELAY_STEPS, SPLIT_RELAY_STEPS != 0>), grid, dim3(SPLIT_NT), 0, st, a, s_first, n_sweeps); \
+    return hipGetLastError();                                                                                     \
+  }                                                                                                               \
   if (a.g.D == DD && a.g.K == KK && relay) {                                                                      \
     hipLaunchKernelGGL((persist_kernel_split<DD, KK, CLV_SPLIT_HELP_CHUNKS, SPLIT_RELAY_STEPS>), grid, dim3(SPLIT_NT), 0, st, a, s_first, n_sweeps); \
     return hipGetLastError();                                                                                     \
@@ -3469,10 +3647,18 @@
   return hipErrorInvalidValue;
 }
 
-hipError_t persist_split_resources(int D, int K, int* blocks_per_cu, size_t* scratch_bytes, bool relay) {
+hipError_t persist_split_resources(int D, int K, int* blocks_per_cu, size_t* scratch_bytes, bool relay, bool rows) {
   hipFuncAttributes fa{};
   if (relay && SPLIT_RELAY_STEPS <= 0) return hipErrorInvalidValue;
+  if (rows && !relay) return hipErrorInvalidValue;
 #define CLV_CASE(DD, KK, PP)                                                                                      \
+  if (D == DD && K == KK && rows) {                                                                               \
+    hipError_t e = hipOccupancyMaxActiveBlocksPerMultiprocessor(blocks_per_cu, persist_kernel_split<DD, KK, CLV_SPLIT_HELP_CHUNKS, SPLIT_RELAY_STEPS, SPLIT_RELAY_STEPS != 0>, SPLIT_NT, 0); \
+    if (e != hipSuccess) return e;                                                                                \
+    e = hipFuncGetAttributes(&fa, reinterpret_cast<const void*>(&persist_kernel_split<DD, KK, CLV_SPLIT_HELP_CHUNKS, SPLIT_RELAY_STEPS, SPLIT_RELAY_STEPS != 0>)); \
+    *scratch_bytes = fa.localSizeBytes;                                                                           \
+    return e;                                                                                                     \
+  }                                                                                                               \
   if (D == DD && K == KK && relay) {                                                                              \
     hipError_t e = hipOccupancyMaxActiveBlocksPerMultiprocessor(blocks_per_cu, persist_kernel_split<DD, KK, CLV_SPLIT_HELP_CHUNKS, SPLIT_RELAY_STEPS>, SPLIT_NT, 0); \
     if (e != hipSuccess) return e;                                                                                \
diff --git a/mcmc_clv_model_amd/sampler.py b/mcmc_clv_model_amd/sampler.py
--- a/mcmc_clv_model_amd/sampler.py
+++ b/mcmc_clv_model_amd/sampler.py
@@ -236,10 +236,12 @@
         check(self._L.clv_launch_info(self.h, out))
         relay = ctypes.c_int32(0)
         check(self._L.clv_split_relay_steps(self.h, ctypes.byref(relay)))
+        rows = ctypes.c_int32(0)
+        check(self._L.clv_split_row_records(self.h, ctypes.byref(rows)))
         return dict(persistent=bool(out[0]), persist_blocks_per_cu=int(out[1]), n_cu=int(out[2]),
                     workgroups=int(out[3]), physical_workgroups=int(out[4]),
                     layout={1: "block", 2: "split", -1: "block (split aborted)"}.get(int(out[5])),
-                    relay_steps=int(relay.value))
+                    relay_steps=int(relay.value), row_records=int(rows.value))
 
     IPC_HANDLE_BYTES = 64
 
```

New measurement: 11.35 billion. 0.989x the previous value.
